# unirestore/UniRestore

Measured on AMD Instinct MI355X. Metric: restored 512x512 images/sec @ 20 denoise steps (whole job), higher is better.
Workload: dtype bf16; 1 GPU; PIR 512x512 batch=8/GPU, 20 DDIM steps, bf16, hipGraph replay (BASELINE.json configs[1]; configs[2] shape for N=8); global_batch=8, per_gpu_batch=8, image=512, denoise_steps=20, parallelism=image-parallel dp1, weights=seeded random init (no checkpoints reachable)

## Files before the change

### include/unirestore_hip.h

```cpp
#ifndef UNIRESTORE_HIP_H
#define UNIRESTORE_HIP_H

#include <stddef.h>
#include <stdint.h>

#ifdef __cplusplus
extern "C" {
#endif

typedef void* ur_stream_t;

enum { UR_OK = 0, UR_E_INVALID = -1, UR_E_UNSUPPORTED = -2, UR_E_LAUNCH = -3, UR_E_WORKSPACE = -4 };

enum { UR_DT_BF16 = 0, UR_DT_F16 = 1 };

enum {
  UR_ACT_NONE = 0,
  UR_ACT_SILU = 1,
  UR_ACT_GELU = 2,
  UR_ACT_GEGLU = 3,
  UR_ACT_GATE = 4,
  UR_ACT_TANH = 5,
  UR_ACT_RELU = 6
};

int ur_version(void);
const char* ur_last_error(void);

typedef struct ur_conv_desc {
  const void* x;
  const void* x2;
  const void* w;
  const float* bias;
  const void* residual;
  void* y;
  void* yt;
  float* gn_part;
  const float* gn_ab;
  int gn_silu;
  float* row_stats;
  const float* ln_stats;
  const float* ln_colsum;
  float ln_eps;
  int ln_dim;
  int ln_parts;
  float* workspace;
  size_t workspace_bytes;
  int N, H, W;
  int C1, ldx, C2, ldx2;
  int Cout, ldw, ldy, ldr;
  int KH, KW, stride, pad_t, pad_l;
  int OH, OW;
  int upsample2x;
  int act;
  int out_f32;
  int n_split, t_rows, t_ld;
  float out_scale;
  int nbatch;
  long long bs_x, bs_x2, bs_w, bs_bias, bs_y, bs_r;
  int k_chunk_major;
  long long bias_img_stride;
  int dtype;
  const void* w_frag;
} ur_conv_desc;

int ur_conv2d_nhwc(const ur_conv_desc* d, ur_stream_t stream);

typedef struct ur_conv_plan {
  int row_stat_parts;
  int gn_parts;
  int gn_fused;
  int prologue_ok;
} ur_conv_plan;
int ur_conv2d_plan(const ur_conv_desc* d, ur_conv_plan* plan);

typedef struct ur_conv_launch_info {
  int launcher;
  int splitk;
  int nk_per_split;
  int reduce;
  int reduce_ri;
  int gn_pass;
  int group_loop;
} ur_conv_launch_info;
int ur_conv2d_plan_launch(const ur_conv_desc* d, ur_conv_launch_info* info);
int ur_conv_launcher_count(void);
const char* ur_conv_launcher_name(int i);

int ur_gemm_bias_act(const void* x, const void* w, const float* bias, const void* residual, void* y, long long M, int N, int K,
                     int ldx, int ldw, int ldy, int ldr, int act, float* workspace, size_t workspace_bytes, int dtype,
                     ur_stream_t stream);
int ur_groupconv3x3_nhwc(const void* x, const void* w, const float* bias, void* y, int N, int H, int W, int Cg, int Cog,
                         int groups, int act, float* workspace, size_t workspace_bytes, int dtype, ur_stream_t stream);

int ur_groupnorm_stats_parts(int N, int HW, int C);
size_t ur_groupnorm_ws_bytes(int N, int HW, int C);
size_t ur_groupnorm_ab_bytes(int N, int C);
int ur_groupnorm_stats(const void* x, float* part, int N, int HW, int C, int dtype, ur_stream_t stream);
int ur_instnorm_stats(const void* x, float* part, int N, int HW, int C, int dtype, ur_stream_t stream);
int ur_groupnorm_finalize(const float* part1, int parts1, int C1, const float* part2, int parts2, int C2, const float* gamma,
                          const float* beta, int N, int HW, int G, float eps, float* ab, float* mean_out, ur_stream_t stream);
int ur_groupnorm_apply_act(const void* x, const void* x2, void* y, const float* ab, int N, int HW, int C1, int C2, int silu,
                           int dtype, ur_stream_t stream);
int ur_groupnorm_nhwc(const void* x, const void* x2, void* y, const float* gamma, const float* beta, int N, int HW,
                      int C1, int C2, int G, float eps, int silu, float* ws, float* ab, const float* pre1, int parts1,
                      const float* pre2, int parts2, int dtype, ur_stream_t stream);
int ur_layernorm_rows(const void* x, void* y, const float* gamma, const float* beta, long long rows, int C,
                      float eps, int dtype, ur_stream_t stream);
int ur_softmax_rows_f32(const float* s, void* p, long long rows, int cols, int ldp, int dtype, ur_stream_t stream);

int ur_attention_fwd(const void* q, const void* k, const void* vt, void* o, int B, int H, int Tq, int Tk,
                     int D, int ldq, int ldk, int ldvt, int ldo, long long bs_q, long long bs_k,
                     long long bs_vt, long long bs_o, float scale, int dtype, ur_stream_t stream);
size_t ur_attention_workspace_bytes(int B, int H, int Tq, int Tk, int D);
int ur_attention_fwd_ws(const void* q, const void* k, const void* vt, void* o, int B, int H, int Tq, int Tk,
                        int D, int ldq, int ldk, int ldvt, int ldo, long long bs_q, long long bs_k, long long bs_vt,
                        long long bs_o, float scale, void* ws, size_t ws_bytes, int dtype, ur_stream_t stream);
typedef struct ur_attention_plan {
  int kernel;
  int workgroups;
  int n_full;
  int n_split;
} ur_attention_plan;
int ur_attention_plan_launch(const void* q, const void* k, const void* vt, void* o, int B, int H, int Tq, int Tk,
                             int D, int ldq, int ldk, int ldvt, int ldo, long long bs_q, long long bs_k, long long bs_vt,
                             long long bs_o, void* ws, size_t ws_bytes, ur_attention_plan* plan);
int ur_attention_kernel_count(void);
const char* ur_attention_kernel_name(int i);

size_t ur_chain_tile_bytes(void);
int ur_ff_geglu_fused(const void* x, const void* stream_w, size_t stream_bytes, void* y, long long T, int C, int hidden, int ldx,
                      int ldy, float ln_eps, int dtype, ur_stream_t stream);

int ur_transformer_head_fused(const void* x, const float* gn_ab, const void* stream_w, size_t stream_bytes, void* h0, void* q, void* k,
                              void* vt, long long T, int tokens_per_image, int C, float ln_eps, int dtype, ur_stream_t stream);
int ur_transformer_tail_fused(const void* o1, const void* h0, const void* xres, const void* stream_w, size_t stream_bytes, void* y,
                              float* gn_part, long long T, int tokens_per_image, int C, int hidden, int heads, int tk, float ln_eps,
                              float attn_scale, int dtype, ur_stream_t stream);

int ur_csce_fused(const void* x, const void* cond, const void* stream_w, size_t stream_bytes, void* y, float* gn_part, long long T,
                  int tokens_per_image, int C, int Ccond, int dtype, ur_stream_t stream);

int ur_dwconv3x3_nhwc(const void* x, const float* w9c, const float* bias, void* y, int N, int H, int W, int C,
                      int gate, int dtype, ur_stream_t stream);
int ur_avgpool_hw(const void* x, float* out, int N, int HW, int C, float* ws, int dtype, ur_stream_t stream);
int ur_scale_channels(const void* x, const float* s, const void* residual, void* y, int N, int HW, int C,
                      int dtype, ur_stream_t stream);
int ur_axpy_channels(const void* a, const void* b, const float* s, void* y, long long rows, int C, int dtype, ur_stream_t stream);
int ur_spade_modulate(const void* n, const void* gb, int ldgb, const void* residual, void* y, long long rows, int C,
                      int dtype, ur_stream_t stream);
int ur_linear_f32(const float* x, const float* w, const float* bias, float* y, int M, int N, int K, int groups,
                  int act, ur_stream_t stream);
int ur_tfa_prompt_update(const float* pooled, const float* cond, float* upd, int B, int T, int D, ur_stream_t stream);
int ur_scale_channels_fanout(const void* x, const float* s, void* y, int B, int K, int HW, int C, int dtype, ur_stream_t stream);
int ur_tfa_prompt_update_fanout(const float* pooled, const float* cond, float* upd, int B, int K, int T, int D, int cond_per_row,
                                ur_stream_t stream);
int ur_vec_mul_group(const float* a, const float* b, float* out, int N, int C, int G, ur_stream_t stream);

int ur_image_to_nhwc(const float* img, void* y, int N, int C, int H, int W, int Cpad, int dtype, ur_stream_t stream);
int ur_nhwc_to_nchw_f32(const void* x, int x_is_f32, float* out, int N, int C, int H, int W, int ld, float mul,
                        float add, int dtype, ur_stream_t stream);
int ur_nchw_f32_to_nhwc(const float* x, void* y, int N, int C, int H, int W, int Cpad, int dtype, ur_stream_t stream);
int ur_image_resize_pad_nhwc(const float* img, void* y, int N, int C, int H, int W, int RH, int RW, int PH, int PW, int Cpad,
                             float mul, float add, int dtype, ur_stream_t stream);
int ur_image_unpad_resize_nchw(const void* x, int x_is_f32, float* out, int N, int C, int XH, int XW, int ld, int CH, int CW,
                               int OH, int OW, float mul, float add, int quantize, int dtype, ur_stream_t stream);
int ur_image_u8_ingest(const uint8_t* src, long long slot_bytes, const int* geom, void* y, int N, int CH, int CW, int Cpad, float mul,
                       float add, int dtype, ur_stream_t stream);
int ur_image_u8_egress(const void* x, int x_is_f32, uint8_t* dst, long long slot_bytes, const int* geom, int* nonfinite, int N, int C,
                       int XH, int XW, int ld, float mul, float add, int dtype, ur_stream_t stream);
int ur_vae_sample(const float* moments, int ld, const float* noise_nchw, float* z_nhwc, void* z_16, int N,
                  int HW, int Clat, int Cpad, float scale, int dtype, ur_stream_t stream);
int ur_add_noise(const float* z0, const float* noise_nchw, float* zt, void* zt_16, int N, int HW, int Clat,
                 int Cpad, float sa, float sb, int dtype, ur_stream_t stream);
int ur_ddim_step(float* zt, const float* eps, int ld_eps, void* zt_16, long long M, int Clat, int Cpad,
                 float c_x, float c_e, int dtype, ur_stream_t stream);
int ur_latent_tiles_gather(const float* z, void* tiles_16, int N, int LH, int LW, int Cpad, int T, int th, int tw,
                           const int* origins, int dtype, ur_stream_t stream);
int ur_latent_tiles_blend_ddim(float* zt, const float* eps_tiles, int ld_eps, void* zt_tiles_16, const float* wn, int N, int LH,
                               int LW, int Clat, int Cpad, int T, int th, int tw, const int* origins, float c_x, float c_e,
                               int dtype, ur_stream_t stream);
int ur_f32_to_bf16_scaled(const float* x, int ld, void* y, long long M, int C, int Cpad, float mul, int dtype, ur_stream_t stream);

int ur_image_metrics(const float* pred, const float* target, int N, int C, int H, int W, int win, double data_range,
                     double* psnr, double* ssim, void* ws, long long ws_bytes, ur_stream_t stream);
long long ur_image_metrics_ws_size(int N, int C, int H, int W, int win);

int ur_profile_enable(int on);
int ur_profile_report(char* buf, size_t buf_bytes);

#ifdef __cplusplus
}
#endif
#endif
```

### unirestore_amd/capi.py

```python
import ctypes as C
import os

import torch

_HERE = os.path.dirname(os.path.abspath(__file__))
LIB_PATH = os.environ.get("UR_LIB") or os.path.join(_HERE, "libunirestore_hip.so")

UR_ACT_NONE, UR_ACT_SILU, UR_ACT_GELU, UR_ACT_GEGLU, UR_ACT_GATE, UR_ACT_TANH, UR_ACT_RELU = range(7)
UR_DT_BF16, UR_DT_F16 = 0, 1
UR_E_INVALID, UR_E_UNSUPPORTED = -1, -2


class ConvDesc(C.Structure):
    _fields_ = [
        ("x", C.c_void_p), ("x2", C.c_void_p), ("w", C.c_void_p), ("bias", C.c_void_p), ("residual", C.c_void_p),
        ("y", C.c_void_p), ("yt", C.c_void_p), ("gn_part", C.c_void_p), ("gn_ab", C.c_void_p), ("gn_silu", C.c_int),
        ("row_stats", C.c_void_p), ("ln_stats", C.c_void_p), ("ln_colsum", C.c_void_p), ("ln_eps", C.c_float), ("ln_dim", C.c_int), ("ln_parts", C.c_int),
        ("workspace", C.c_void_p),
        ("workspace_bytes", C.c_size_t),
        ("N", C.c_int), ("H", C.c_int), ("W", C.c_int),
        ("C1", C.c_int), ("ldx", C.c_int), ("C2", C.c_int), ("ldx2", C.c_int),
        ("Cout", C.c_int), ("ldw", C.c_int), ("ldy", C.c_int), ("ldr", C.c_int),
        ("KH", C.c_int), ("KW", C.c_int), ("stride", C.c_int), ("pad_t", C.c_int), ("pad_l", C.c_int),
        ("OH", C.c_int), ("OW", C.c_int),
        ("upsample2x", C.c_int), ("act", C.c_int), ("out_f32", C.c_int),
        ("n_split", C.c_int), ("t_rows", C.c_int), ("t_ld", C.c_int),
        ("out_scale", C.c_float),
        ("nbatch", C.c_int),
        ("bs_x", C.c_longlong), ("bs_x2", C.c_longlong), ("bs_w", C.c_longlong), ("bs_bias", C.c_longlong),
        ("bs_y", C.c_longlong), ("bs_r", C.c_longlong), ("k_chunk_major", C.c_int), ("bias_img_stride", C.c_longlong),
        ("dtype", C.c_int), ("w_frag", C.c_void_p),
    ]


class ConvPlan(C.Structure):
    _fields_ = [("row_stat_parts", C.c_int), ("gn_parts", C.c_int), ("gn_fused", C.c_int), ("prologue_ok", C.c_int)]


class ConvLaunchInfo(C.Structure):
    _fields_ = [("launcher", C.c_int), ("splitk", C.c_int), ("nk_per_split", C.c_int), ("reduce", C.c_int), ("reduce_ri", C.c_int),
                ("gn_pass", C.c_int), ("group_loop", C.c_int)]


class AttentionPlan(C.Structure):
    _fields_ = [("kernel", C.c_int), ("workgroups", C.c_int), ("n_full", C.c_int), ("n_split", C.c_int)]


_P, _I, _F, _LL, _SZ = C.c_void_p, C.c_int, C.c_float, C.c_longlong, C.c_size_t

SIGNATURES = {
    "ur_version": (_I, []),
    "ur_last_error": (C.c_char_p, []),
    "ur_conv2d_nhwc": (_I, [C.POINTER(ConvDesc), _P]),
    "ur_conv2d_plan": (_I, [C.POINTER(ConvDesc), C.POINTER(ConvPlan)]),
    "ur_conv2d_plan_launch": (_I, [C.POINTER(ConvDesc), C.POINTER(ConvLaunchInfo)]),
    "ur_conv_launcher_count": (_I, []),
    "ur_conv_launcher_name": (C.c_char_p, [_I]),
    "ur_gemm_bias_act": (_I, [_P, _P, _P, _P, _P, _LL, _I, _I, _I, _I, _I, _I, _I, _P, _SZ, _I, _P]),
    "ur_groupconv3x3_nhwc": (_I, [_P, _P, _P, _P, _I, _I, _I, _I, _I, _I, _I, _P, _SZ, _I, _P]),
    "ur_groupnorm_stats_parts": (_I, [_I, _I, _I]),
    "ur_groupnorm_ws_bytes": (_SZ, [_I, _I, _I]),
    "ur_groupnorm_ab_bytes": (_SZ, [_I, _I]),
    "ur_groupnorm_stats": (_I, [_P, _P, _I, _I, _I, _I, _P]),
    "ur_instnorm_stats": (_I, [_P, _P, _I, _I, _I, _I, _P]),
    "ur_groupnorm_finalize": (_I, [_P, _I, _I, _P, _I, _I, _P, _P, _I, _I, _I, _F, _P, _P, _P]),
    "ur_groupnorm_apply_act": (_I, [_P, _P, _P, _P, _I, _I, _I, _I, _I, _I, _P]),
    "ur_groupnorm_nhwc": (_I, [_P, _P, _P, _P, _P, _I, _I, _I, _I, _I, _F, _I, _P, _P, _P, _I, _P, _I, _I, _P]),
    "ur_layernorm_rows": (_I, [_P, _P, _P, _P, _LL, _I, _F, _I, _P]),
    "ur_softmax_rows_f32": (_I, [_P, _P, _LL, _I, _I, _I, _P]),
    "ur_attention_fwd": (_I, [_P, _P, _P, _P, _I, _I, _I, _I, _I, _I, _I, _I, _I, _LL, _LL, _LL, _LL, _F, _I, _P]),
    "ur_attention_workspace_bytes": (_SZ, [_I, _I, _I, _I, _I]),
    "ur_attention_fwd_ws": (_I, [_P, _P, _P, _P, _I, _I, _I, _I, _I, _I, _I, _I, _I, _LL, _LL, _LL, _LL, _F, _P, _SZ, _I, _P]),
    "ur_attention_plan_launch": (_I, [_P, _P, _P, _P, _I, _I, _I, _I, _I, _I, _I, _I, _I, _LL, _LL, _LL, _LL, _P, _SZ, C.POINTER(AttentionPlan)]),
    "ur_attention_kernel_count": (_I, []),
    "ur_attention_kernel_name": (C.c_char_p, [_I]),
    "ur_chain_tile_bytes": (_SZ, []),
    "ur_ff_geglu_fused": (_I, [_P, _P, _SZ, _P, _LL, _I, _I, _I, _I, _F, _I, _P]),
    "ur_transformer_head_fused": (_I, [_P, _P, _P, _SZ, _P, _P, _P, _P, _LL, _I, _I, _F, _I, _P]),
    "ur_transformer_tail_fused": (_I, [_P, _P, _P, _P, _SZ, _P, _P, _LL, _I, _I, _I, _I, _I, _F, _F, _I, _P]),
    "ur_csce_fused": (_I, [_P, _P, _P, _SZ, _P, _P, _LL, _I, _I, _I, _I, _P]),
    "ur_dwconv3x3_nhwc": (_I, [_P, _P, _P, _P, _I, _I, _I, _I, _I, _I, _P]),
    "ur_avgpool_hw": (_I, [_P, _P, _I, _I, _I, _P, _I, _P]),
    "ur_scale_channels": (_I, [_P, _P, _P, _P, _I, _I, _I, _I, _P]),
    "ur_scale_channels_fanout": (_I, [_P, _P, _P, _I, _I, _I, _I, _I, _P]),
    "ur_axpy_channels": (_I, [_P, _P, _P, _P, _LL, _I, _I, _P]),
    "ur_spade_modulate": (_I, [_P, _P, _I, _P, _P, _LL, _I, _I, _P]),
    "ur_linear_f32": (_I, [_P, _P, _P, _P, _I, _I, _I, _I, _I, _P]),
    "ur_tfa_prompt_update": (_I, [_P, _P, _P, _I, _I, _I, _P]),
    "ur_tfa_prompt_update_fanout": (_I, [_P, _P, _P, _I, _I, _I, _I, _I, _P]),
    "ur_vec_mul_group": (_I, [_P, _P, _P, _I, _I, _I, _P]),
    "ur_image_to_nhwc": (_I, [_P, _P, _I, _I, _I, _I, _I, _I, _P]),
    "ur_nhwc_to_nchw_f32": (_I, [_P, _I, _P, _I, _I, _I, _I, _I, _F, _F, _I, _P]),
    "ur_nchw_f32_to_nhwc": (_I, [_P, _P, _I, _I, _I, _I, _I, _I, _P]),
    "ur_image_resize_pad_nhwc": (_I, [_P, _P] + [_I] * 9 + [_F, _F, _I, _P]),
    "ur_image_unpad_resize_nchw": (_I, [_P, _I, _P] + [_I] * 9 + [_F, _F, _I, _I, _P]),
    "ur_image_u8_ingest": (_I, [_P, _LL, _P, _P, _I, _I, _I, _I, _F, _F, _I, _P]),
    "ur_image_u8_egress": (_I, [_P, _I, _P, _LL, _P, _P, _I, _I, _I, _I, _I, _F, _F, _I, _P]),
    "ur_vae_sample": (_I, [_P, _I, _P, _P, _P, _I, _I, _I, _I, _F, _I, _P]),
    "ur_add_noise": (_I, [_P, _P, _P, _P, _I, _I, _I, _I, _F, _F, _I, _P]),
    "ur_ddim_step": (_I, [_P, _P, _I, _P, _LL, _I, _I, _F, _F, _I, _P]),
    "ur_latent_tiles_gather": (_I, [_P, _P, _I, _I, _I, _I, _I, _I, _I, _P, _I, _P]),
    "ur_latent_tiles_blend_ddim": (_I, [_P, _P, _I, _P, _P, _I, _I, _I, _I, _I, _I, _I, _I, _P, _F, _F, _I, _P]),
    "ur_f32_to_bf16_scaled": (_I, [_P, _I, _P, _LL, _I, _I, _F, _I, _P]),
    "ur_image_metrics": (_I, [_P, _P, _I, _I, _I, _I, _I, C.c_double, _P, _P, _P, _LL, _P]),
    "ur_image_metrics_ws_size": (_LL, [_I, _I, _I, _I, _I]),
    "ur_profile_enable": (_I, [_I]),
    "ur_profile_report": (_I, [C.c_char_p, _SZ]),
}


def _load():
    if not os.path.exists(LIB_PATH):
        raise ImportError(
            f"{LIB_PATH} not found: build it with `python -m unirestore_amd.build` (or __graft_entry__.build()). "
            "There is no CPU / eager fallback in the product path.")
    lib = C.CDLL(LIB_PATH)
    for name, (res, args) in SIGNATURES.items():
        fn = getattr(lib, name)
        fn.restype, fn.argtypes = res, args
    return lib


lib = _load()


def launcher_names() -> list:
    return [lib.ur_conv_launcher_name(i).decode() for i in range(lib.ur_conv_launcher_count())]


def plan_launch(d: ConvDesc) -> ConvLaunchInfo:
    info = ConvLaunchInfo()
    check(lib.ur_conv2d_plan_launch(d, info))
    return info


def attention_kernel_names() -> list:
    return [lib.ur_attention_kernel_name(i).decode() for i in range(lib.ur_attention_kernel_count())]


def attention_plan(q, k, vt, o, B, H, Tq, Tk, D, ldq, ldk, ldvt, ldo, bs_q, bs_k, bs_vt, bs_o, ws, ws_bytes) -> AttentionPlan:
    plan = AttentionPlan()
    check(lib.ur_attention_plan_launch(q, k, vt, o, B, H, Tq, Tk, D, ldq, ldk, ldvt, ldo, bs_q, bs_k, bs_vt, bs_o, ws, ws_bytes, plan))
    return plan


class URError(RuntimeError):
    pass


def check(rc: int):
    if rc != 0:
        msg = lib.ur_last_error().decode("utf-8", "replace")
        if rc == UR_E_INVALID:
            raise ValueError(f"unirestore_hip: {msg}")
        if rc == UR_E_UNSUPPORTED:
            raise NotImplementedError(f"unirestore_hip (UR_E_UNSUPPORTED): {msg}")
        raise URError(f"unirestore_hip error {rc}: {msg}")
```

### unirestore_amd/csrc/igemm.hip

```cpp
#include "igemm_impl.h"

namespace urk {
#define UR_DECLARE(name)                                                                                             \
  ConvLaunch name##_bf16(void* k, size_t ws_bytes);                                                                 \
  ConvLaunch name##_f16(void* k, size_t ws_bytes);                                                                  \
  static ConvLaunch name(ConvK& k, size_t ws_bytes) { return (k.f16 ? name##_f16 : name##_bf16)(&k, ws_bytes); }
UR_CONV_LAUNCHERS(UR_DECLARE)
#undef UR_DECLARE
}

namespace {

ConvLaunch dispatch_conv(ConvK& k, bool pair, size_t ws_bytes) {
  if (k.KH == 3 && k.stride == 1 && k.pad_t == 1 && k.pad_l == 1 && k.kcm && k.staged_ok_ && !pair && k.nbatch == 1 &&
      k.OW % 32 == 0 && k.OH % 8 == 0 && k.OH == (k.ups ? 2 * k.H : k.H) && k.OW == (k.ups ? 2 * k.W : k.W) && !k.yt) {
    const bool ok128 = k.Cout % 128 == 0, ok160 = k.Cout % 160 == 0;
    const long long tm8 = (long long)k.N * (k.OH / 8) * (k.OW / 32);
    auto eff = [](long long t) { return t <= 128 ? (double)(t * (256 / t)) / 256.0 : (double)t / (double)(((t + 255) / 256) * 256); };
    const bool use160 = ok160 && (!ok128 || eff(tm8 * (k.Cout / 160)) >= eff(tm8 * (k.Cout / 128)));
    const long long tiles8 = tm8 * (use160 ? k.Cout / 160 : k.Cout / 128);
    if ((ok128 || ok160) && tiles8 >= 64) {
      if (use160) return urk::halo_8x32_160(k, ws_bytes);
      return urk::halo_8x32_128(k, ws_bytes);
    }
  }
  if (k.KH == 3 && k.stride == 1 && k.pad_t == 1 && k.pad_l == 1 && k.kcm && !pair && k.nbatch == 1 && !k.ups && k.C2 == 0 &&
      k.Cout <= 32 && k.OW % 32 == 0 && k.OH % 8 == 0 && k.OH == k.H && k.OW == k.W && !k.yt && !k.gn_part && !k.gn_ab && !k.row_stats && !k.ln_stats &&
      !k.bias_img && (long long)k.N * (k.OH / 8) * (k.OW / 32) >= 128)
    return urk::halo_thin_32(k, ws_bytes);
  const bool himg_ups = k.ups && k.OH == 16 && k.OW == 16 && k.H == 8 && k.W == 8;
  if (k.KH == 3 && k.stride == 1 && k.pad_t == 1 && k.pad_l == 1 && k.kcm && k.staged_ok_ && !pair && k.nbatch == 1 &&
      ((!k.ups && k.OH == k.H && k.OW == k.W) || himg_ups) && !k.yt && k.Cout % 128 == 0 && k.nk >= 36) {
    if (k.wf && k.OH == 8 && k.OW == 8 && k.N <= 16 && k.Cin % 256 == 0 && k.nk >= 72 && k.y && k.ws && !k.gn_ab && !k.row_stats && !k.ln_stats &&
        (long long)(k.nk / 36) * k.M * k.Cout * 4 <= (long long)ws_bytes)
      return urk::wstream_8x8(k, ws_bytes);
    if (k.OH == 16 && k.OW == 16) return urk::himg_16x16(k, ws_bytes);
    if (k.OH == 8 && k.OW == 8 && k.N % 4 == 0) {
      return urk::himg_8x8x4(k, ws_bytes);
    }
  }
  if (k.KH == 1 && k.stride == 1 && !k.ups && k.C2 == 0 && k.staged_ok_ && k.Cout % 256 == 0 && !k.yt && (k.act == UR_ACT_GEGLU || k.act == UR_ACT_GATE) &&
      (long long)((k.M + 255) / 256) * (k.Cout / 256) * k.nbatch >= 200 && (long long)k.M * k.ldx < (1ll << 31) - 256)
  {
    auto fill = [](long long t) { return (double)t / (double)(((t + 255) / 256) * 256); };
    const long long tm = (k.M + 255) / 256;
    if (k.Cout % 320 == 0 && k.nbatch == 1 && !k.bias_img && fill(tm * (k.Cout / 320)) > fill(tm * (k.Cout / 256)))
      return urk::gemm_256x320_pair(k, ws_bytes);
    return urk::gemm_256x256(k, ws_bytes);
  }
  const bool use_v1 = k.KH == 1 && k.nk <= 10;
  const long long blocks128 = (long long)((k.M + 127) / 128) * ((k.Cout + 127) / 128) * k.nbatch;
  const bool g1 = k.KH == 1 && k.stride == 1 && !k.ups && k.C2 == 0 && k.pad_t == 0 && k.pad_l == 0 && k.OH == k.H && k.OW == k.W &&
                  (long long)k.M * k.ldx + k.Ktot < (1ll << 31) - 256;
  auto nosplit = [&](int bm, int bn) { return (long long)((k.M + bm - 1) / bm) * ((k.Cout + bn - 1) / bn) * k.nbatch >= 200 || k.nk < 8 || !k.ws; };
  if (k.KH == 1 && !pair && k.Cout > 64) {
    const long long blocks64 = (long long)((k.M + 63) / 64) * ((k.Cout + 63) / 64) * k.nbatch;
    if (blocks128 < 200 && g1 && blocks64 >= 128 && blocks64 <= 256 && k.nk >= 8 && k.nk <= 48) return urk::g1_64x64_deep(k, ws_bytes);
    if (g1 && blocks128 < 200 && k.nk > 24 && k.nk <= 96 && (long long)((k.M + 127) / 128) * ((k.Cout + 63) / 64) * k.nbatch >= 256)
      return urk::g1_128x64_deep(k, ws_bytes);
    if (blocks128 < 200 && g1 && ((blocks64 >= 128 && k.nk <= 24) || (blocks64 >= 256 && k.nk <= 48))) return urk::g1_64x64(k, ws_bytes);
    if (blocks128 < 200 && k.nk <= 24) return g1 && nosplit(64, 64) ? urk::g1_64x64(k, ws_bytes) : urk::v1_64x64(k, ws_bytes);
    if (use_v1 && blocks128 > 256 && blocks128 < 400 && k.Cout % 128 == 0) return g1 && nosplit(128, 64) ? urk::g1_128x64(k, ws_bytes) : urk::v1_128x64(k, ws_bytes);
  }
  if (use_v1) {
    if (pair) return urk::v1_128x128(k, ws_bytes);
    if (k.Cout <= 32) return urk::v1_256x32(k, ws_bytes);
    if (k.Cout <= 64) return urk::v1_128x64(k, ws_bytes);
    if (k.Cout % 160 == 0 && k.Cout % 128 != 0) return g1 && nosplit(128, 160) ? urk::g1_128x160(k, ws_bytes) : urk::v1_128x160(k, ws_bytes);
    return g1 && nosplit(128, 128) ? urk::g1_128x128(k, ws_bytes) : urk::v1_128x128(k, ws_bytes);
  }
  if (k.Cout <= 32) return urk::v2_256x32(k, ws_bytes);
  if (k.Cout <= 64 && !pair) return urk::v2_128x64(k, ws_bytes);
  const bool n160 = !pair && k.Cout % 160 == 0 && k.Cout % 128 != 0;
  const long long big_tiles = (long long)((k.M + 255) / 256) * ((k.Cout + (n160 ? 159 : 127)) / (n160 ? 160 : 128)) * k.nbatch;
  if (g1 && !pair && big_tiles < 256) {
    const long long t160 = k.Cout % 160 == 0 ? (long long)((k.M + 127) / 128) * (k.Cout / 160) : 0;
    const long long t128 = (long long)((k.M + 127) / 128) * ((k.Cout + 127) / 128);
    auto fill = [](long long t) { return t <= 0 ? 0.0 : (double)t / (double)(((t + 255) / 256) * 256); };
    if (t160 >= 200 && fill(t160) >= fill(t128)) return urk::g1_128x160(k, ws_bytes);
    if (t128 >= 200) return urk::g1_128x128(k, ws_bytes);
  }
  if (big_tiles >= 160) {
    if (n160 && g1) return urk::g1_128x160(k, ws_bytes);
    if (n160) return urk::v2_256x160(k, ws_bytes);
    return urk::v2_256x128(k, ws_bytes);
  }
  if (k.Cout % 160 == 0 && k.Cout % 128 != 0 && !pair) return urk::v1_128x160(k, ws_bytes);
  return urk::v1_128x128(k, ws_bytes);
}

}

static int conv_impl(const ur_conv_desc* d, ur_stream_t stream, ur_conv_plan* plan, ur_conv_launch_info* info = nullptr) {
  UR_REQUIRE(d && d->x && d->w, "null x/w");
  UR_REQUIRE(d->KH == d->KW && (d->KH == 1 || d->KH == 3), "only 1x1 and 3x3 kernels");
  UR_REQUIRE(d->C1 > 0 && d->C1 % 8 == 0 && d->C2 % 8 == 0 && d->ldx % 8 == 0, "Cin/ldx must be multiples of 8");
  UR_REQUIRE(d->C2 == 0 || (d->x2 && d->ldx2 % 8 == 0), "virtual concat needs x2");
  UR_REQUIRE(d->Cout > 0 && d->Cout % 4 == 0 && d->ldw % 8 == 0, "Cout%4, ldw%8");
  UR_REQUIRE(d->nbatch >= 1 && d->stride >= 1 && d->OH > 0 && d->OW > 0, "bad dims");
  UR_REQUIRE(d->y || d->yt || d->gn_part, "no output requested");
  UR_REQUIRE_DT(d->dtype);
  const bool pair = d->act == UR_ACT_GEGLU || d->act == UR_ACT_GATE;
  if (pair && d->Cout % 64 != 0)
    return ur::fail(UR_E_UNSUPPORTED, "ur_conv2d_nhwc: pair activations (GEGLU / SimpleGate) need Cout % 64 == 0 (32-row a|g interleave)");
  UR_REQUIRE(!d->y || (d->out_f32 ? d->ldy % 4 == 0 : d->ldy % 4 == 0), "ldy%4");
  UR_REQUIRE(!d->residual || d->ldr % 4 == 0, "ldr%4");
  UR_REQUIRE(!d->yt || (d->t_rows > 0 && d->n_split % 4 == 0 && !pair), "bad transposed-output spec");

  ConvK k;
  k.x = (const uint16_t*)d->x; k.x2 = (const uint16_t*)d->x2; k.w = (const uint16_t*)d->w; k.bias = d->bias;
  k.res = (const uint16_t*)d->residual; k.y = d->y; k.yt = (uint16_t*)d->yt;
  k.ws = d->workspace;
  k.N = d->N; k.H = d->H; k.W = d->W; k.C1 = d->C1; k.ldx = d->ldx; k.C2 = d->C2; k.ldx2 = d->ldx2;
  k.Cin = d->C1 + d->C2; k.Cout = d->Cout; k.ldw = d->ldw; k.ldy = d->ldy; k.ldr = d->ldr;
  k.KH = d->KH; k.KW = d->KW; k.stride = d->stride; k.pad_t = d->pad_t; k.pad_l = d->pad_l;
  k.OH = d->OH; k.OW = d->OW; k.OHW = d->OH * d->OW; k.ups = d->upsample2x; k.act = d->act; k.out_f32 = d->out_f32;
  k.n_split = d->yt ? d->n_split : d->Cout; k.t_rows = d->t_rows; k.t_ld = d->t_ld;
  k.out_scale = d->out_scale;
  k.M = d->N * d->OH * d->OW; k.Ktot = d->KH * d->KW * k.Cin; k.nk = (k.Ktot + 63) / 64; k.nbatch = d->nbatch;
  k.bs_x = d->bs_x; k.bs_x2 = d->bs_x2; k.bs_w = d->bs_w; k.bs_bias = d->bs_bias; k.bs_y = d->bs_y; k.bs_r = d->bs_r; k.bias_img = d->bias_img_stride;
  UR_REQUIRE(k.M > 0, "empty problem");
  UR_REQUIRE((long long)d->N * d->H * d->W * (long long)std::max(d->ldx, d->ldx2) < (1ll << 31) &&
                 (long long)d->Cout * d->ldw < (1ll << 31), "tensor too large for 32-bit element offsets");

  k.kcm = d->k_chunk_major; k.wf = (const uint16_t*)d->w_frag; k.wmajor = 0; k.xgm = 0; k.xbn = 0; k.patch_tw = 0;
  UR_REQUIRE(!k.kcm || (k.Cin % 64 == 0 && d->C1 % 64 == 0), "k_chunk_major needs C1 and C1+C2 to be multiples of 64");
  k.gn_part = d->gn_part; k.gn_ab = d->gn_ab; k.gn_silu = d->gn_silu; k.f16 = d->dtype == UR_DT_F16; k.gn_fused = 0; k.gn_parts = 0;
  k.ln_parts = d->ln_parts;
  k.row_stats = d->row_stats; k.ln_stats = d->ln_stats; k.ln_colsum = d->ln_colsum; k.ln_eps = d->ln_eps; k.ln_dim = d->ln_dim;
  UR_REQUIRE(!d->ln_stats || (d->ln_colsum && d->ln_dim > 0), "ln_stats needs ln_colsum / ln_dim");
  UR_REQUIRE(!(d->bias_img_stride && (pair || d->ln_stats || d->yt)), "per-image bias rows do not combine with pair activations / LayerNorm folding / transposed columns");
  k.staged_ok_ = (d->y ? (!d->out_f32 && ((d->ldy | d->bs_y) & 7) == 0) : d->gn_part != nullptr) &&
                 (!d->residual || ((d->ldr | d->bs_r) & 7) == 0);
  UR_REQUIRE(!d->gn_part || (!d->out_f32 && !d->yt), "gn_part needs a plain 16-bit output (or none)");
  hipStream_t s = (hipStream_t)stream;
  const double flops = 2.0 * k.M * (double)k.Cout * k.Ktot * k.nbatch;
  const double bytes = 2.0 * ((double)k.M * k.Cin + (double)k.Cout * k.Ktot + (double)k.M * k.Cout) * k.nbatch;
  const char* fam = d->KH == 3 ? "conv3x3_igemm" : "gemm1x1_igemm";
  static const bool prof_shapes = getenv("UR_PROF_SHAPES") != nullptr;
  if (prof_shapes) {
    static std::map<std::string, int> interned;
    char buf[128];
    snprintf(buf, sizeof buf, "%s M%d N%d K%d s%d u%d b%d a%d", d->KH == 3 ? "c3" : "g1", k.M, k.Cout, k.Ktot, d->stride, d->upsample2x,
             k.nbatch, d->act);
    fam = interned.emplace(buf, 0).first->first.c_str();
  }
  const ConvLaunch launch = dispatch_conv(k, pair, d->workspace_bytes);
  const bool group_loop = k.nbatch > 1 && d->KH == 3 && k.kcm && k.stride == 1 && !pair && !k.gn_part && !k.row_stats && !k.ln_stats &&
                          !k.yt && !k.gn_ab && !k.out_f32 && k.staged_ok_ && k.Cout % 128 == 0 && !k.bias_img && k.C2 == 0;
  auto group_k = [&](int b) {
    ConvK kb = k;
    kb.nbatch = 1;
    kb.x = k.x + b * k.bs_x; kb.w = k.w + b * k.bs_w; kb.bias = k.bias ? k.bias + b * k.bs_bias : nullptr;
    kb.res = k.res ? k.res + b * k.bs_r : nullptr;
    kb.y = reinterpret_cast<uint16_t*>(k.y) + b * k.bs_y;
    kb.bs_x = kb.bs_w = kb.bs_bias = kb.bs_y = kb.bs_r = 0;
    return kb;
  };
  if (plan) {
    plan->row_stat_parts = d->row_stats ? (k.splitk > 1 ? 1 : k.tiles_n) : 0;
    plan->gn_parts = k.gn_parts; plan->gn_fused = k.gn_fused; plan->prologue_ok = launch.prologue_ok;
  }
  if (info) {
    ConvK kb = group_loop ? group_k(0) : k;
    const ConvLaunch l = group_loop ? dispatch_conv(kb, pair, d->workspace_bytes) : launch;
    info->launcher = l.id; info->splitk = kb.splitk; info->nk_per_split = kb.nk_per_split;
    const ReducePlan r = kb.splitk > 1 ? plan_splitk_reduce(kb) : ReducePlan{-1, 0};
    info->reduce = r.kind; info->reduce_ri = r.ri;
    info->gn_pass = k.gn_part && !k.gn_fused && !group_loop;
    info->group_loop = group_loop;
  }
  if (plan || info) return UR_OK;
  if (!d->y && d->gn_part && (!k.gn_fused || k.splitk > 1))
    return ur::fail(UR_E_UNSUPPORTED, "ur_conv2d_nhwc: y == NULL needs a launch whose epilogue writes gn_part (see ur_conv2d_plan)");
  if (d->gn_ab && !launch.prologue_ok)
    return ur::fail(UR_E_UNSUPPORTED, "ur_conv2d_nhwc: gn_ab is not supported by this launch (see ur_conv2d_plan.prologue_ok)");
  ur::ProfScope prof(fam, flops, bytes, s);
  UR_REQUIRE(!(d->row_stats || d->ln_stats) || (k.staged_ok_ && k.nbatch == 1 && !d->yt == !d->yt), "row_stats / ln fusion need a bf16 staged output");
  if (group_loop) {
    for (int b = 0; b < d->nbatch; ++b) {
      ConvK kb = group_k(b);
      const int rcb = dispatch_conv(kb, pair, d->workspace_bytes).launch(&kb, s);
      if (rcb != UR_OK) return rcb;
    }
    return UR_OK;
  }
  const int rc = launch.launch(&k, s);
  if (rc != UR_OK) return rc;
  if (k.gn_part && !k.gn_fused) {
    const int ctot = (pair ? k.Cout / 2 : k.Cout) * k.nbatch;
    UR_REQUIRE(k.y && k.ldy == ctot, "gn_part fallback needs a dense output (ldy == channels)");
    return ur::gn_stats_launch(k.y, k.gn_part, k.N, k.OHW, ctot, d->dtype, s);
  }
  return UR_OK;
}

extern "C" int ur_conv2d_nhwc(const ur_conv_desc* d, ur_stream_t stream) { return conv_impl(d, stream, nullptr); }

extern "C" int ur_conv2d_plan(const ur_conv_desc* d, ur_conv_plan* plan) {
  UR_REQUIRE(d && plan, "null pointer");
  ur_conv_desc t = *d;
  if (!t.y && !t.yt && !t.gn_part) t.y = reinterpret_cast<void*>(16);
  return conv_impl(&t, nullptr, plan);
}

extern "C" int ur_conv2d_plan_launch(const ur_conv_desc* d, ur_conv_launch_info* info) {
  UR_REQUIRE(d && info, "null pointer");
  ur_conv_desc t = *d;
  if (!t.y && !t.yt && !t.gn_part) t.y = reinterpret_cast<void*>(16);
  return conv_impl(&t, nullptr, nullptr, info);
}

#define UR_LAUNCHER_NAME(name) #name,
static const char* const kLauncherNames[] = {UR_CONV_LAUNCHERS(UR_LAUNCHER_NAME)};
#undef UR_LAUNCHER_NAME
static_assert(sizeof(kLauncherNames) / sizeof(kLauncherNames[0]) == UR_CONV_LAUNCHER_COUNT, "one name per launcher");

extern "C" int ur_conv_launcher_count(void) { return UR_CONV_LAUNCHER_COUNT; }
extern "C" const char* ur_conv_launcher_name(int i) { return i >= 0 && i < UR_CONV_LAUNCHER_COUNT ? kLauncherNames[i] : nullptr; }

extern "C" int ur_gemm_bias_act(const void* x, const void* w, const float* bias, const void* residual, void* y, long long M, int N, int K,
                                int ldx, int ldw, int ldy, int ldr, int act, float* workspace, size_t workspace_bytes, int dtype,
                                ur_stream_t stream) {
  UR_REQUIRE(M > 0 && M < (1ll << 31), "M out of range");
  ur_conv_desc d = {};
  d.x = x; d.w = w; d.bias = bias; d.residual = residual; d.y = y;
  d.workspace = workspace; d.workspace_bytes = workspace_bytes;
  d.N = 1; d.H = 1; d.W = (int)M; d.C1 = K; d.ldx = ldx; d.Cout = N; d.ldw = ldw; d.ldy = ldy; d.ldr = ldr;
  d.KH = d.KW = 1; d.stride = 1; d.OH = 1; d.OW = (int)M; d.act = act; d.out_scale = 1.f; d.nbatch = 1; d.dtype = dtype;
  return conv_impl(&d, stream, nullptr);
}

extern "C" int ur_groupconv3x3_nhwc(const void* x, const void* w, const float* bias, void* y, int N, int H, int W, int Cg, int Cog,
                                    int groups, int act, float* workspace, size_t workspace_bytes, int dtype, ur_stream_t stream) {
  UR_REQUIRE(groups >= 1 && Cg % 8 == 0 && Cog % 4 == 0, "groups >= 1, Cg % 8 == 0, Cog % 4 == 0");
  ur_conv_desc d = {};
  d.x = x; d.w = w; d.bias = bias; d.y = y;
  d.workspace = workspace; d.workspace_bytes = workspace_bytes;
  d.N = N; d.H = H; d.W = W; d.C1 = Cg; d.ldx = Cg * groups; d.Cout = Cog; d.ldw = 9 * Cg; d.ldy = Cog * groups;
  d.KH = d.KW = 3; d.stride = 1; d.pad_t = d.pad_l = 1; d.OH = H; d.OW = W; d.act = act; d.out_scale = 1.f; d.nbatch = groups;
  d.bs_x = Cg; d.bs_w = (long long)Cog * 9 * Cg; d.bs_bias = Cog; d.bs_y = Cog; d.dtype = dtype;
  return conv_impl(&d, stream, nullptr);
}
```

### unirestore_amd/csrc/igemm_impl.h

```cpp
#pragma once
#include <cstdio>
#include <cstdlib>
#include <map>
#include <string>

#include "common.h"

static __device__ uint4 g_zero_page[8];
typedef uint32_t ig_u32x4 __attribute__((ext_vector_type(4)));

struct ConvLaunch {
  int (*launch)(void* k, hipStream_t s);
  int prologue_ok;
  int id;
};

namespace {

struct ConvK {
  const uint16_t* x; const uint16_t* x2; const uint16_t* w; const float* bias; const uint16_t* res;
  void* y; uint16_t* yt; float* ws; float* gn_part; const float* gn_ab;
  float* row_stats; const float* ln_stats; const float* ln_colsum; float ln_eps; int ln_dim, ln_parts;
  int N, H, W, C1, ldx, C2, ldx2, Cin, Cout, ldw, ldy, ldr, KH, KW, stride, pad_t, pad_l, OH, OW, OHW;
  int ups, act, out_f32, n_split, t_rows, t_ld;
  float out_scale;
  int M, Ktot, nk, tiles_m, tiles_n, splitk, nk_per_split, nbatch;
  long long bs_x, bs_x2, bs_w, bs_bias, bs_y, bs_r, bias_img;
  int gn_fused, gn_parts, gn_silu, f16, staged_ok_;
  int patch_tw;
  int kcm;
  const uint16_t* wf;
  int wmajor;
  int xgm, xbn;
};

__device__ __forceinline__ void xcd_tile_map(const ConvK& p, int id, int& tm, int& tn) {
  const int xcd = id & 7, idx = id >> 3;
  if (p.xgm) {
    const int lm = idx / p.xbn, ln = idx - lm * p.xbn;
    tm = (xcd % p.xgm) * (p.tiles_m / p.xgm) + lm;
    tn = (xcd / p.xgm) * p.xbn + ln;
    return;
  }
  const int nt = p.tiles_m * p.tiles_n, q = nt >> 3, r = nt & 7;
  id = (xcd < r ? xcd * (q + 1) : r * (q + 1) + (xcd - r) * q) + idx;
  if (p.wmajor) { tn = id / p.tiles_m; tm = id - tn * p.tiles_m; }
  else { tm = id / p.tiles_n; tn = id - tm * p.tiles_n; }
}

static inline void pick_xcd_grid(ConvK& k, double W, double A) {
  k.xgm = 0; k.xbn = 0; k.wmajor = 0;
  static const bool off = getenv("UR_NOXCDGRID") != nullptr;
  if (off || k.nbatch != 1) return;
  const long long nt = (long long)k.tiles_m * k.tiles_n;
  double best = 0.9 * (8.0 * W + A);
  if (nt % 8 == 0)
    for (int gm = 4; gm >= 1; gm >>= 1) {
      const int gn = 8 / gm;
      if (k.tiles_m % gm || k.tiles_n % gn) continue;
      const double c = gm * W + gn * A;
      if (c < best) { best = c; k.xgm = gm; k.xbn = k.tiles_n / gn; }
    }
  if (!k.xgm && k.tiles_n >= 8 && W + 8.0 * A < best) k.wmajor = 1;
}

__device__ __forceinline__ bool is_pair_act(int act) { return act == UR_ACT_GEGLU || act == UR_ACT_GATE; }

__device__ __forceinline__ int tile_row_to_m(const ConvK& p, int m0, int r) {
  return p.patch_tw ? m0 + (r / p.patch_tw) * p.OW + (r % p.patch_tw) : m0 + r;
}

template <bool F16>
__device__ __forceinline__ void epi_store(const ConvK& p, int gb, int m, int co, float v[4]) {
  if (p.res) {
    const uint16_t* r = p.res + gb * p.bs_r + (long long)m * p.ldr + co;
    uint2 rv = *reinterpret_cast<const uint2*>(r);
    v[0] += Act<F16>::lo(rv.x); v[1] += Act<F16>::hi(rv.x);
    v[2] += Act<F16>::lo(rv.y); v[3] += Act<F16>::hi(rv.y);
  }
  if (p.yt && co >= p.n_split) {
    int b = m / p.t_rows, t = m - b * p.t_rows;
    int cw = p.Cout - p.n_split;
    uint16_t* o = p.yt + ((long long)b * cw + (co - p.n_split)) * p.t_ld + t;
#pragma unroll
    for (int e = 0; e < 4; ++e) o[(long long)e * p.t_ld] = f2h16<F16>(v[e]);
    return;
  }
  if (!p.y) return;
  if (p.out_f32) {
    float* o = reinterpret_cast<float*>(p.y) + gb * p.bs_y + (long long)m * p.ldy + co;
    *reinterpret_cast<float4*>(o) = make_float4(v[0], v[1], v[2], v[3]);
  } else {
    uint16_t* o = reinterpret_cast<uint16_t*>(p.y) + gb * p.bs_y + (long long)m * p.ldy + co;
    *reinterpret_cast<uint2*>(o) = make_uint2(Act<F16>::pack2(v[0], v[1]), Act<F16>::pack2(v[2], v[3]));
  }
}

__device__ __forceinline__ int epi_act(const ConvK& p, int gb, int m, int co_in, float a[4], const float g[4]) {
  const long long boff = gb * p.bs_bias + (p.bias_img ? (long long)(m / p.OHW) * p.bias_img : 0);
  if (p.bias) {
    const float* b = p.bias + boff + co_in;
    float4 bv = *reinterpret_cast<const float4*>(b);
    a[0] += bv.x; a[1] += bv.y; a[2] += bv.z; a[3] += bv.w;
  }
  int co = co_in;
  if (is_pair_act(p.act)) {
    float gg[4] = {g[0], g[1], g[2], g[3]};
    if (p.bias) {
      float4 bv = *reinterpret_cast<const float4*>(p.bias + boff + co_in + 32);
      gg[0] += bv.x; gg[1] += bv.y; gg[2] += bv.z; gg[3] += bv.w;
    }
#pragma unroll
    for (int e = 0; e < 4; ++e) a[e] *= (p.act == UR_ACT_GEGLU) ? gelu_f(gg[e]) : gg[e];
    co = (co_in >> 6) * 32 + (co_in & 31);
  } else if (p.act != UR_ACT_NONE) {
#pragma unroll
    for (int e = 0; e < 4; ++e) a[e] = apply_act(a[e], p.act);
  }
#pragma unroll
  for (int e = 0; e < 4; ++e) a[e] *= p.out_scale;
  return co;
}

template <int BM, int NC, int NT, int SROW, bool LOAD>
__device__ __forceinline__ void tile_copy(const ConvK& p, uint16_t* g, long long ld, unsigned char* smem, int m0, int M, int c0,
                                          int cmax) {
  constexpr int Q = NC / 8;
  constexpr int TOT = BM * Q, U = 5;
  for (int i0 = threadIdx.x; i0 < TOT; i0 += NT * U) {
    uint4 v[U];
    uint16_t* gp[U];
    uint2* lp[U];
    bool ok[U];
#pragma unroll
    for (int u = 0; u < U; ++u) {
      const int i = i0 + u * NT;
      const int r = i / Q, c = (i - r * Q) * 8;
      const int m = tile_row_to_m(p, m0, i < TOT ? r : 0);
      ok[u] = i < TOT && m < M && c < cmax;
      gp[u] = g + (long long)(ok[u] ? m : m0) * ld + c0 + (ok[u] ? c : 0);
      lp[u] = reinterpret_cast<uint2*>(smem + (ok[u] ? r * SROW + c * 2 : 0));
      if (LOAD) v[u] = *reinterpret_cast<const uint4*>(gp[u]);
      else { const uint2 a = lp[u][0], b = lp[u][1]; v[u] = make_uint4(a.x, a.y, b.x, b.y); }
    }
#pragma unroll
    for (int u = 0; u < U; ++u) {
      if (!ok[u]) continue;
      if (LOAD) { lp[u][0] = make_uint2(v[u].x, v[u].y); lp[u][1] = make_uint2(v[u].z, v[u].w); }
      else {
store16_wt(gp[u], v[u]);
      }
    }
  }
}

template <int FM, int FN, int WTM, int WTN, bool F16>
__device__ __forceinline__ void igemm_epilogue_direct(const ConvK& p, f32x16 (&acc)[FN][FM], int m0, int n0, int wm, int wn,
                                                      int lane, int gb) {
  const int fhalf = lane >> 5, mrow = lane & 31;
  const bool pair = is_pair_act(p.act);
#pragma unroll
  for (int a = 0; a < FN; ++a) {
    if (pair && (a & 1)) continue;
#pragma unroll
    for (int b = 0; b < FM; ++b) {
      int m = tile_row_to_m(p, m0, wm * WTM + b * 32 + mrow);
#pragma unroll
      for (int rg = 0; rg < 4; ++rg) {
        int co_in = n0 + wn * WTN + a * 32 + rg * 8 + fhalf * 4;
        bool ok = m < p.M && co_in < p.Cout;
        float v[4], g[4] = {0.f, 0.f, 0.f, 0.f};
#pragma unroll
        for (int e = 0; e < 4; ++e) v[e] = acc[a][b][rg * 4 + e];
        if (pair) {
          constexpr int a1 = (FN > 1) ? 1 : 0;
#pragma unroll
          for (int e = 0; e < 4; ++e) g[e] = acc[(a + a1) % FN][b][rg * 4 + e];
        }
        int co = co_in;
        if (ok) co = epi_act(p, gb, m, co_in, v, g);
        if (ok) epi_store<F16>(p, gb, m, co, v);
      }
    }
  }
}

template <int FM, int FN, int WTM, int WTN, int BM, int BN, int SROW, int PAIR, int LN, int MULTI, int YT, int ACT, bool F16>
__device__ __forceinline__ void epi_frag_pass(const ConvK& p, f32x16 (&acc)[FN][FM], int m0, int n0, int c0, int wm, int wn, int lane,
                                              int gb, unsigned char* smem, const float* sbias, const float* scol, const float* srow) {
  const int fhalf = lane >> 5, mrow = lane & 31;
  const bool pair_ = PAIR == 2 ? is_pair_act(p.act) : PAIR != 0;
  const bool ln_ = LN == 2 ? p.ln_stats != nullptr : LN != 0;
  const bool multi_ = MULTI == 2 ? (p.bias_img && !p.patch_tw && p.OHW < BM) : MULTI != 0;
  const bool yt_ = YT == 2 ? p.yt != nullptr : YT != 0;
  const bool act_ = ACT == 2 ? p.act != UR_ACT_NONE : ACT != 0;
  const bool has_res = p.res != nullptr;
#pragma unroll
  for (int a = 0; a < FN; ++a) {
    if (pair_ && (a & 1)) continue;
#pragma unroll
    for (int rg = 0; rg < 4; ++rg) {
      const int ln = wn * WTN + a * 32 + rg * 8 + fhalf * 4;
      const int co_in = n0 + ln;
      float4 bv = *reinterpret_cast<const float4*>(sbias + ln);
      float4 gv = make_float4(0.f, 0.f, 0.f, 0.f);
      if (pair_) gv = *reinterpret_cast<const float4*>(sbias + ln + 32);
      const int lco = pair_ ? ((ln >> 6) * 32 + (ln & 31)) : ln;
      const int co = c0 + lco;
      const bool col_ok = co_in < p.Cout;
      float4 sv = make_float4(0.f, 0.f, 0.f, 0.f), sg = make_float4(0.f, 0.f, 0.f, 0.f);
      if (ln_) {
        sv = *reinterpret_cast<const float4*>(scol + ln);
        if (pair_) sg = *reinterpret_cast<const float4*>(scol + ln + 32);
      }
#pragma unroll
      for (int b = 0; b < FM; ++b) {
        const int lm = wm * WTM + b * 32 + mrow;
        if (multi_) {
          const int il = lm / p.OHW;
          bv = *reinterpret_cast<const float4*>(sbias + il * BN + ln);
          if (pair_) gv = *reinterpret_cast<const float4*>(sbias + il * BN + ln + 32);
        }
        float v[4], gq[4] = {0.f, 0.f, 0.f, 0.f};
        constexpr int a1 = (FN > 1) ? 1 : 0;
        if (ln_) {
          const float mean = srow[2 * lm], rstd = srow[2 * lm + 1];
          v[0] = rstd * (acc[a][b][rg * 4] - mean * sv.x) + bv.x;     v[1] = rstd * (acc[a][b][rg * 4 + 1] - mean * sv.y) + bv.y;
          v[2] = rstd * (acc[a][b][rg * 4 + 2] - mean * sv.z) + bv.z; v[3] = rstd * (acc[a][b][rg * 4 + 3] - mean * sv.w) + bv.w;
          if (pair_) {
            gq[0] = rstd * (acc[(a + a1) % FN][b][rg * 4] - mean * sg.x) + gv.x;     gq[1] = rstd * (acc[(a + a1) % FN][b][rg * 4 + 1] - mean * sg.y) + gv.y;
            gq[2] = rstd * (acc[(a + a1) % FN][b][rg * 4 + 2] - mean * sg.z) + gv.z; gq[3] = rstd * (acc[(a + a1) % FN][b][rg * 4 + 3] - mean * sg.w) + gv.w;
          }
        } else {
          v[0] = acc[a][b][rg * 4] + bv.x; v[1] = acc[a][b][rg * 4 + 1] + bv.y;
          v[2] = acc[a][b][rg * 4 + 2] + bv.z; v[3] = acc[a][b][rg * 4 + 3] + bv.w;
          if (pair_) {
            gq[0] = acc[(a + a1) % FN][b][rg * 4] + gv.x; gq[1] = acc[(a + a1) % FN][b][rg * 4 + 1] + gv.y;
            gq[2] = acc[(a + a1) % FN][b][rg * 4 + 2] + gv.z; gq[3] = acc[(a + a1) % FN][b][rg * 4 + 3] + gv.w;
          }
        }
        if (pair_) {
          const float g0 = gq[0], g1 = gq[1], g2 = gq[2], g3 = gq[3];
          if (p.act == UR_ACT_GEGLU) { v[0] *= gelu_f(g0); v[1] *= gelu_f(g1); v[2] *= gelu_f(g2); v[3] *= gelu_f(g3); }
          else { v[0] *= g0; v[1] *= g1; v[2] *= g2; v[3] *= g3; }
        } else if (act_) {
#pragma unroll
          for (int e = 0; e < 4; ++e) v[e] = apply_act(v[e], p.act);
        }
#pragma unroll
        for (int e = 0; e < 4; ++e) v[e] *= p.out_scale;
        const int mg = tile_row_to_m(p, m0, lm);
        const bool ok = col_ok && mg < p.M;
        if (yt_ && co >= p.n_split) {
          if (ok) epi_store<F16>(p, gb, mg, co, v);
          continue;
        }
        uint2* sp = reinterpret_cast<uint2*>(smem + lm * SROW + lco * 2);
        if (has_res) {
          const uint2 rv = *sp;
          v[0] += Act<F16>::lo(rv.x); v[1] += Act<F16>::hi(rv.x);
          v[2] += Act<F16>::lo(rv.y); v[3] += Act<F16>::hi(rv.y);
        }
        if (ok) *sp = make_uint2(Act<F16>::pack2(v[0], v[1]), Act<F16>::pack2(v[2], v[3]));
      }
    }
  }
}

template <int FM, int FN, int WTM, int WTN, int BM, int BN, int NT, int CLS, bool PAIRC, bool F16>
__device__ __forceinline__ void staged_epilogue(const ConvK& p, f32x16 (&acc)[FN][FM], int m0, int n0, int wm, int wn, int lane,
                                                int gb, unsigned char* smem, bool owner, int nimg_tile_in) {
  constexpr int SROW = (PAIRC ? BN : BN * 2) + 8;
  const bool pair = CLS ? is_pair_act(p.act) : false;
  const bool ln = CLS ? p.ln_stats != nullptr : false;
  const bool yt = CLS ? p.yt != nullptr : false;
  const int nimg_tile = CLS ? nimg_tile_in : 1;
  const int c0 = pair ? (n0 >> 1) : n0;
  const int ncols = pair ? BN / 2 : BN;
  const int cmax = min(yt ? p.n_split : (pair ? p.Cout / 2 : p.Cout), c0 + ncols) - c0;
  float* sbias = reinterpret_cast<float*>(smem + BM * SROW);
  float* scol = sbias + 4 * BN;
  float* srow = scol + BN;
  const int img0 = m0 / p.OHW;
  for (int i = threadIdx.x; i < BN * nimg_tile; i += NT) {
    const int il = i / BN, col = i - il * BN;
    const long long boff = gb * p.bs_bias + (p.bias_img ? (long long)min(img0 + il, p.N - 1) * p.bias_img : 0);
    sbias[i] = (p.bias && n0 + col < p.Cout) ? p.bias[boff + n0 + col] : 0.f;
  }
  if (ln) {
    for (int i = threadIdx.x; i < BN; i += NT) scol[i] = n0 + i < p.Cout ? p.ln_colsum[n0 + i] : 0.f;
    for (int r = threadIdx.x; r < BM; r += NT) {
      const int m = min(tile_row_to_m(p, m0, r), p.M - 1);
      float sx = 0.f, sq = 0.f;
      for (int q = 0; q < p.ln_parts; ++q) {
        const float2 t2 = *reinterpret_cast<const float2*>(p.ln_stats + 2 * ((long long)q * p.M + m));
        sx += t2.x; sq += t2.y;
      }
      const float mean = sx / p.ln_dim;
      const float var = fmaxf(sq / p.ln_dim - mean * mean, 0.f);
      srow[2 * r] = mean;
      srow[2 * r + 1] = rsqrtf(var + p.ln_eps);
    }
  }
  if (p.res) {
    uint16_t* rb = const_cast<uint16_t*>(p.res) + gb * p.bs_r;
    if (pair) tile_copy<BM, (BN >= 16 ? BN / 2 : 8), NT, SROW, true>(p, rb, p.ldr, smem, m0, p.M, c0, cmax);
    else tile_copy<BM, BN, NT, SROW, true>(p, rb, p.ldr, smem, m0, p.M, c0, cmax);
  }
  __syncthreads();
  if (owner) {
    const bool multi = nimg_tile > 1, hasact = p.act != UR_ACT_NONE;
#define UR_EPI_PASS(PAIR, LN, MULTI, YT, ACT) \
    epi_frag_pass<FM, FN, WTM, WTN, BM, BN, SROW, PAIR, LN, MULTI, YT, ACT, F16>(p, acc, m0, n0, c0, wm, wn, lane, gb, smem, sbias, scol, srow)
    if constexpr (CLS == 0) { if (hasact) UR_EPI_PASS(0, 0, 0, 0, 1); else UR_EPI_PASS(0, 0, 0, 0, 0); }
    else if constexpr (PAIRC) {
      if (ln) UR_EPI_PASS(1, 1, 0, 0, 0); else UR_EPI_PASS(1, 0, 0, 0, 0);
    } else {
      if (pair) { if (ln) UR_EPI_PASS(1, 1, 0, 0, 0); else UR_EPI_PASS(1, 0, 0, 0, 0); }
      else if (yt) {
        if (hasact) UR_EPI_PASS(0, 2, 0, 1, 2);
        else if (ln) UR_EPI_PASS(0, 1, 0, 1, 0);
        else UR_EPI_PASS(0, 0, 0, 1, 0);
      }
      else if (multi) { if (hasact) UR_EPI_PASS(0, 0, 1, 0, 2); else UR_EPI_PASS(0, 0, 1, 0, 0); }
      else if (hasact) UR_EPI_PASS(0, 1, 0, 0, 2);
      else UR_EPI_PASS(0, 1, 0, 0, 0);
    }
#undef UR_EPI_PASS
  }
  __syncthreads();
  if (p.gn_fused) {
    float* red = sbias;
    const int CP = ncols >> 1, NG = NT / CP, RGN = (BM + NG - 1) / NG;
    const int cp = threadIdx.x % CP, g = threadIdx.x / CP;
    if (g < NG) {
      float s0 = 0.f, s1 = 0.f, q0 = 0.f, q1 = 0.f;
      if (cp * 2 < cmax) {
        const int r0 = g * RGN, r1 = p.patch_tw ? min(BM, r0 + RGN) : min(min(BM, r0 + RGN), p.M - m0);
        for (int r = r0; r < r1; ++r) {
          const uint32_t w = *reinterpret_cast<const uint32_t*>(smem + r * SROW + cp * 4);
          const float a = Act<F16>::lo(w), b = Act<F16>::hi(w);
          s0 += a; q0 += a * a; s1 += b; q1 += b * b;
        }
      }
      red[(g * 4 + 0) * CP + cp] = s0; red[(g * 4 + 1) * CP + cp] = s1;
      red[(g * 4 + 2) * CP + cp] = q0; red[(g * 4 + 3) * CP + cp] = q1;
    }
    __syncthreads();
    const int ctot = pair ? p.Cout / 2 : p.Cout;
    const int img = m0 / p.OHW, rem = m0 - img * p.OHW;
    const int pm = p.patch_tw ? ((rem / p.OW) / (BM / p.patch_tw)) * (p.OW / p.patch_tw) + (rem % p.OW) / p.patch_tw : rem / BM;
    float* st = p.gn_part + ((((long long)img * p.gn_parts + pm) * p.nbatch + gb) * ctot + c0) * 2;
    for (int i = threadIdx.x; i < cmax; i += NT) {
      const int c2 = i >> 1, odd = i & 1;
      float a = 0.f, b = 0.f;
      for (int gg = 0; gg < NG; ++gg) { a += red[(gg * 4 + odd) * CP + c2]; b += red[(gg * 4 + 2 + odd) * CP + c2]; }
      *reinterpret_cast<float2*>(st + 2 * i) = make_float2(a, b);
    }
  }
  if (p.row_stats) {
    constexpr int TPR = NT / BM >= 1 ? NT / BM : 1;
    const int r = threadIdx.x / TPR, part = threadIdx.x % TPR;
    if (r < BM) {
      const int m = tile_row_to_m(p, m0, r);
      const int npair = cmax >> 1, per = (npair + TPR - 1) / TPR;
      float sx = 0.f, sq = 0.f;
      for (int j = part * per; j < min(npair, (part + 1) * per); ++j) {
        const uint32_t w = *reinterpret_cast<const uint32_t*>(smem + r * SROW + j * 4);
        const float a = Act<F16>::lo(w), b = Act<F16>::hi(w);
        sx += a + b; sq += a * a + b * b;
      }
      if (TPR >= 2) { sx += __shfl_xor(sx, 1, 64); sq += __shfl_xor(sq, 1, 64); }
      if (TPR >= 4) { sx += __shfl_xor(sx, 2, 64); sq += __shfl_xor(sq, 2, 64); }
      static_assert(TPR == 1 || TPR == 2 || TPR == 4, "row-stat reduction: 1, 2 or 4 threads per row (same wave)");
      const int tn_idx = n0 / BN;
      if (m < p.M && part == 0)
        *reinterpret_cast<float2*>(p.row_stats + 2 * ((long long)tn_idx * p.M + m)) = make_float2(sx, sq);
    }
  }
  if (!p.y) return;
  uint16_t* yb = reinterpret_cast<uint16_t*>(p.y) + gb * p.bs_y;
  if (pair) tile_copy<BM, (BN >= 16 ? BN / 2 : 8), NT, SROW, false>(p, yb, p.ldy, smem, m0, p.M, c0, cmax);
  else tile_copy<BM, BN, NT, SROW, false>(p, yb, p.ldy, smem, m0, p.M, c0, cmax);
}

template <int BM, int BN, int NT, bool PAIRC = false>
constexpr int epi_lds_bytes() {
  constexpr int tile = BM * ((PAIRC ? BN : BN * 2) + 8);
  constexpr int aux1 = 5 * BN * 4 + BM * 8, aux2 = 4 * NT * 4;
  return tile + (aux1 > aux2 ? aux1 : aux2);
}

template <int FM, int FN, int WTM, int WTN, int BM, int BN, int NT, bool F16, bool DIRECT_OK = true, bool PAIRC = false>
__device__ __forceinline__ void igemm_epilogue(const ConvK& p, f32x16 (&acc)[FN][FM], int m0, int n0, int wm, int wn, int lane,
                                               int gb, int sz, unsigned char* smem, bool owner = true) {
  const int fhalf = lane >> 5, mrow = lane & 31;
  if (p.splitk > 1) {
    if (!owner) return;
    float* ws = p.ws + ((long long)(sz * p.nbatch + gb) * p.M) * p.Cout;
#pragma unroll
    for (int a = 0; a < FN; ++a)
#pragma unroll
      for (int b = 0; b < FM; ++b) {
        int m = tile_row_to_m(p, m0, wm * WTM + b * 32 + mrow);
#pragma unroll
        for (int rg = 0; rg < 4; ++rg) {
          int co = n0 + wn * WTN + a * 32 + rg * 8 + fhalf * 4;
          if (m < p.M && co < p.Cout)
            *reinterpret_cast<float4*>(ws + (long long)m * p.Cout + co) =
                make_float4(acc[a][b][rg * 4], acc[a][b][rg * 4 + 1], acc[a][b][rg * 4 + 2], acc[a][b][rg * 4 + 3]);
        }
      }
    return;
  }
  const bool pair = is_pair_act(p.act);
  constexpr int SROW = BN * 2 + 8;
  const int nimg_tile = (p.bias_img && !p.patch_tw && p.OHW < BM) ? BM / p.OHW : 1;
  const bool bias_geom_ok = !p.bias_img || p.patch_tw || (p.OHW % BM) == 0 || ((BM % p.OHW) == 0 && nimg_tile <= 4);
  const bool staged = p.staged_ok_ && BN >= 32 && bias_geom_ok;
  if (!staged) {
    if (DIRECT_OK && owner) igemm_epilogue_direct<FM, FN, WTM, WTN, F16>(p, acc, m0, n0, wm, wn, lane, gb);
    return;
  }
  const bool plain = !pair && !p.ln_stats && nimg_tile == 1 && !p.yt;
  if (PAIRC) { if (!plain) staged_epilogue<FM, FN, WTM, WTN, BM, BN, NT, 1, true, F16>(p, acc, m0, n0, wm, wn, lane, gb, smem, owner, nimg_tile); }
  else if (plain) staged_epilogue<FM, FN, WTM, WTN, BM, BN, NT, 0, false, F16>(p, acc, m0, n0, wm, wn, lane, gb, smem, owner, nimg_tile);
  else staged_epilogue<FM, FN, WTM, WTN, BM, BN, NT, 1, false, F16>(p, acc, m0, n0, wm, wn, lane, gb, smem, owner, nimg_tile);
}

#include "igemm_asm.inc"
#define IG_MN(ASM, ...)                                                                      \
  do {                                                                                       \
    if constexpr (F16) asm volatile(ASM("v_mfma_f32_32x32x16_f16") __VA_ARGS__);             \
    else asm volatile(ASM("v_mfma_f32_32x32x16_bf16") __VA_ARGS__);                          \
  } while (0)
template <int FM, int FN, bool F16>
__device__ __forceinline__ void ktile_mma(f32x16 (&acc)[FN][FM], const unsigned (&ab)[FM], unsigned aw) {
  ig_u32x4 t0, t1, t2, t3, t4, t5, t6, t7, t8, t9;
  unsigned x0, x1, xw;
#define KT_POOL6 "=&v"(t0), "=&v"(t1), "=&v"(t2), "=&v"(t3), "=&v"(t4), "=&v"(t5)
#define KT_POOL8 KT_POOL6, "=&v"(t6), "=&v"(t7)
#define KT_POOL10 KT_POOL8, "=&v"(t8), "=&v"(t9)
  if constexpr (FM == 1 && FN == 5) {
    IG_MN(IG_ASM_KT_1x5, : "+v"(acc[0][0]), "+v"(acc[1][0]), "+v"(acc[2][0]), "+v"(acc[3][0]), "+v"(acc[4][0]), KT_POOL10, "=&v"(x0), "=&v"(xw)
          : "v"(ab[0]), "v"(aw) : "memory");
  } else if constexpr (FM == 2 && FN == 2) {
    IG_MN(IG_ASM_KT_2x2, : "+v"(acc[0][0]), "+v"(acc[0][1]), "+v"(acc[1][0]), "+v"(acc[1][1]), KT_POOL8, "=&v"(x0), "=&v"(x1), "=&v"(xw)
          : "v"(ab[0]), "v"(ab[1]), "v"(aw) : "memory");
  } else if constexpr (FM == 1 && FN == 1) {
    IG_MN(IG_ASM_KT_1x1, : "+v"(acc[0][0]), KT_POOL6, "=&v"(x0), "=&v"(xw) : "v"(ab[0]), "v"(aw) : "memory");
  } else if constexpr (FM == 2 && FN == 1) {
    IG_MN(IG_ASM_KT_2x1, : "+v"(acc[0][0]), "+v"(acc[0][1]), KT_POOL6, "=&v"(x0), "=&v"(x1), "=&v"(xw) : "v"(ab[0]), "v"(ab[1]), "v"(aw) : "memory");
  } else if constexpr (FM == 2 && FN == 4) {
    IG_MN(IG_ASM_KT_2x4, : "+v"(acc[0][0]), "+v"(acc[0][1]), "+v"(acc[1][0]), "+v"(acc[1][1]), "+v"(acc[2][0]), "+v"(acc[2][1]), "+v"(acc[3][0]), "+v"(acc[3][1]),
          KT_POOL6, "=&v"(x0), "=&v"(x1), "=&v"(xw) : "v"(ab[0]), "v"(ab[1]), "v"(aw) : "memory");
  } else if constexpr (FM == 1 && FN == 10) {
    IG_MN(IG_ASM_KT_1x10, : "+v"(acc[0][0]), "+v"(acc[1][0]), "+v"(acc[2][0]), "+v"(acc[3][0]), "+v"(acc[4][0]), "+v"(acc[5][0]), "+v"(acc[6][0]), "+v"(acc[7][0]),
          "+v"(acc[8][0]), "+v"(acc[9][0]), KT_POOL6, "=&v"(x0), "=&v"(xw) : "v"(ab[0]), "v"(aw) : "memory");
  } else {
    static_assert(FM == 0, "no hand-scheduled K tile for this fragment shape");
  }
#undef KT_POOL6
#undef KT_POOL8
#undef KT_POOL10
}
template <int FM, int FN> constexpr bool ktile_gemm_ok() {
#if defined(UR_IGEMM_NOASM) || defined(UR_GEMM_NOASM)
  return false;
#else
  return (FM == 1 && (FN == 1 || FN == 5 || FN == 10)) || (FM == 2 && (FN == 1 || FN == 2 || FN == 4));
#endif
}
template <int FM, int FN> constexpr bool ktile_asm_ok() {
#ifdef UR_IGEMM_NOASM
  return false;
#else
  return (FM == 1 && FN == 5) || (FM == 2 && FN == 2);
#endif
}


template <int BM, int BN, int WM, int WN, bool G1, bool F16>
__global__ __launch_bounds__(256) void igemm_kernel(const ConvK p) {
  constexpr int WTM = BM / WM, WTN = BN / WN, FM = WTM / 32, FN = WTN / 32, XP = BM / 32, WP = BN / 32;
  constexpr int STAGE = (BM + BN) * 128;
  static_assert(WM * WN == 4 && WTM % 32 == 0 && WTN % 32 == 0, "tile/wave shape");
  extern __shared__ __attribute__((aligned(16))) unsigned char smem[];

  const int tid = threadIdx.x, lane = tid & 63, wid = tid >> 6;
  const int wm = wid % WM, wn = wid / WM;
  const int gb = blockIdx.y, sz = blockIdx.z;

  int tm, tn;
  xcd_tile_map(p, blockIdx.x, tm, tn);
  const int m0 = tm * BM, n0 = tn * BN;

  const uint16_t* __restrict__ X1 = p.x + gb * p.bs_x;
  const uint16_t* __restrict__ X2 = p.x2 ? p.x2 + gb * p.bs_x2 : nullptr;
  const uint16_t* __restrict__ Wt = p.w + gb * p.bs_w;

  const int chunk = tid & 7, lrow = tid >> 3;
  int ih0[XP], iw0[XP], nb[XP];
  bool xok[XP];
#pragma unroll
  for (int i = 0; i < XP; ++i) {
    int m = m0 + i * 32 + lrow;
    xok[i] = m < p.M;
    if (G1) { nb[i] = xok[i] ? m * p.ldx : 0; ih0[i] = iw0[i] = 0; continue; }
    int mm = xok[i] ? m : 0;
    int n = mm / p.OHW, rem = mm - n * p.OHW;
    int oh = rem / p.OW, ow = rem - oh * p.OW;
    ih0[i] = oh * p.stride - p.pad_t;
    iw0[i] = ow * p.stride - p.pad_l;
    nb[i] = n * p.H;
  }
  long long woff[WP];
  bool wok[WP];
#pragma unroll
  for (int j = 0; j < WP; ++j) {
    int row = n0 + j * 32 + lrow;
    wok[j] = row < p.Cout;
    woff[j] = (long long)(wok[j] ? row : 0) * p.ldw;
  }
  const int Hlim = p.ups ? p.H * 2 : p.H, Wlim = p.ups ? p.W * 2 : p.W;

  const int kt_begin = sz * p.nk_per_split;
  const int kt_end = min(p.nk, kt_begin + p.nk_per_split);
  int kcur = kt_begin * 64 + chunk * 8;
  int tap = 0, cch = kcur;
  const int ntap = p.KH * p.KW;
  if (!G1) {
    tap = kcur / p.Cin; cch = kcur - tap * p.Cin;
    if (p.kcm) { tap = kt_begin % ntap; cch = (kt_begin / ntap) * 64 + chunk * 8; }
  }

  uint4 xr[XP], wr[WP];
  auto load_tile = [&]() {
    const bool kval = kcur < p.Ktot;
    if (G1) {
#pragma unroll
      for (int i = 0; i < XP; ++i) {
        const bool v = kval && xok[i];
        const uint4 val = *reinterpret_cast<const uint4*>(v ? X1 + nb[i] + kcur : X1);
        xr[i] = v ? val : make_uint4(0, 0, 0, 0);
      }
#pragma unroll
      for (int j = 0; j < WP; ++j) {
        const bool v = kval && wok[j];
        const uint4 val = *reinterpret_cast<const uint4*>(v ? Wt + woff[j] + kcur : Wt);
        wr[j] = v ? val : make_uint4(0, 0, 0, 0);
      }
      kcur += 64;
      return;
    }
    const int dy = (p.KW == 1) ? 0 : (tap * 11) >> 5;
    const int dx = tap - dy * p.KW;
    const uint16_t* src = X1;
    int ld = p.ldx, cc = cch;
    if (cch >= p.C1) { src = X2; ld = p.ldx2; cc = cch - p.C1; }
#pragma unroll
    for (int i = 0; i < XP; ++i) {
      int ih = ih0[i] + dy, iw = iw0[i] + dx;
      bool v = kval && xok[i] && (unsigned)ih < (unsigned)Hlim && (unsigned)iw < (unsigned)Wlim;
      if (p.ups) { ih >>= 1; iw >>= 1; }
      long long off = ((long long)(nb[i] + ih) * p.W + iw) * ld + cc;
      const uint4* ptr = reinterpret_cast<const uint4*>(v ? src + off : src);
      uint4 val = *ptr;
      xr[i] = v ? val : make_uint4(0, 0, 0, 0);
    }
#pragma unroll
    for (int j = 0; j < WP; ++j) {
      bool v = kval && wok[j];
      const uint4* ptr = reinterpret_cast<const uint4*>(v ? Wt + woff[j] + kcur : Wt);
      uint4 val = *ptr;
      wr[j] = v ? val : make_uint4(0, 0, 0, 0);
    }
    kcur += 64;
    if (p.kcm) { if (++tap == ntap) { tap = 0; cch += 64; } }
    else { cch += 64; while (cch >= p.Cin) { cch -= p.Cin; ++tap; } }
  };
  auto store_tile = [&](int stage) {
    unsigned char* xs = smem + stage * STAGE;
    unsigned char* wsm = xs + BM * 128;
#pragma unroll
    for (int i = 0; i < XP; ++i) {
      int row = i * 32 + lrow;
      *reinterpret_cast<uint4*>(xs + row * 128 + ((chunk ^ ((row >> 1) & 7)) << 4)) = xr[i];
    }
#pragma unroll
    for (int j = 0; j < WP; ++j) {
      int row = j * 32 + lrow;
      *reinterpret_cast<uint4*>(wsm + row * 128 + ((chunk ^ ((row >> 1) & 7)) << 4)) = wr[j];
    }
  };

  f32x16 acc[FN][FM];
#pragma unroll
  for (int a = 0; a < FN; ++a)
#pragma unroll
    for (int b = 0; b < FM; ++b)
#pragma unroll
      for (int e = 0; e < 16; ++e) acc[a][b][e] = 0.f;

  const int frow = lane & 31, fhalf = lane >> 5;
  typedef __attribute__((address_space(3))) void* lptr_t;
  const unsigned kt_x0 = (unsigned)(uintptr_t)(lptr_t)smem + (wm * WTM + frow) * 128 + ((fhalf ^ ((frow >> 1) & 7)) << 4);
  const unsigned kt_w0 = (unsigned)(uintptr_t)(lptr_t)smem + (BM + wn * WTN + frow) * 128 + ((fhalf ^ ((frow >> 1) & 7)) << 4);
  static_assert(WTM % 32 == 0 && ((WTN >> 1) & 7) == 0, "fragment rows must keep the swizzle phase of row 0");
  auto compute = [&](int stage) {
    if constexpr (ktile_gemm_ok<FM, FN>()) {
      unsigned ab[FM];
#pragma unroll
      for (int b = 0; b < FM; ++b) ab[b] = kt_x0 + stage * STAGE + b * 4096;
      ktile_mma<FM, FN, F16>(acc, ab, kt_w0 + stage * STAGE);
      return;
    }
    const unsigned char* xs = smem + stage * STAGE;
    const unsigned char* wsm = xs + BM * 128;
#pragma unroll
    for (int ks = 0; ks < 4; ++ks) {
      const int slot = ks * 2 + fhalf;
      typename Frag<F16>::type bfr[FM], afr[FN];
#pragma unroll
      for (int b = 0; b < FM; ++b) {
        int row = wm * WTM + b * 32 + frow;
        bfr[b] = *reinterpret_cast<const typename Frag<F16>::type*>(xs + row * 128 + ((slot ^ ((row >> 1) & 7)) << 4));
      }
#pragma unroll
      for (int a = 0; a < FN; ++a) {
        int row = wn * WTN + a * 32 + frow;
        afr[a] = *reinterpret_cast<const typename Frag<F16>::type*>(wsm + row * 128 + ((slot ^ ((row >> 1) & 7)) << 4));
      }
#pragma unroll
      for (int a = 0; a < FN; ++a)
#pragma unroll
        for (int b = 0; b < FM; ++b)
          acc[a][b] = mfma16t(afr[a], bfr[b], acc[a][b]);
    }
  };

  if (kt_begin < kt_end) {
    load_tile();
    store_tile(0);
    __syncthreads();
    int stage = 0;
    for (int kt = kt_begin; kt < kt_end; ++kt) {
      const bool more = kt + 1 < kt_end;
      if (more) load_tile();
      compute(stage);
      if (more) store_tile(stage ^ 1);
      __syncthreads();
      stage ^= 1;
    }
  }
// ... 611 lines not shown

struct GnAB { float4 a0, a1, b0, b1; };
__device__ __forceinline__ GnAB gn_load_ab(const unsigned char* abuf, int chunk) {
  GnAB r;
  r.a0 = *reinterpret_cast<const float4*>(abuf + chunk * 32); r.a1 = *reinterpret_cast<const float4*>(abuf + chunk * 32 + 16);
  r.b0 = *reinterpret_cast<const float4*>(abuf + 256 + chunk * 32); r.b1 = *reinterpret_cast<const float4*>(abuf + 256 + chunk * 32 + 16);
  return r;
}
template <bool F16>
__device__ __forceinline__ void gn_piece_inplace(unsigned char* piece, const GnAB& ab, bool silu) {
  const float4 a0 = ab.a0, a1 = ab.a1, b0 = ab.b0, b1 = ab.b1;
  const uint4 v = *reinterpret_cast<const uint4*>(piece);
  float f[8];
  unpack8t<F16>(v, f);
  f[0] = fmaf(f[0], a0.x, b0.x); f[1] = fmaf(f[1], a0.y, b0.y); f[2] = fmaf(f[2], a0.z, b0.z); f[3] = fmaf(f[3], a0.w, b0.w);
  f[4] = fmaf(f[4], a1.x, b1.x); f[5] = fmaf(f[5], a1.y, b1.y); f[6] = fmaf(f[6], a1.z, b1.z); f[7] = fmaf(f[7], a1.w, b1.w);
  if (silu) {
#pragma unroll
    for (int e = 0; e < 8; ++e) f[e] = silu_f(f[e]);
  }
  *reinterpret_cast<uint4*>(piece) = pack8t<F16>(f);
}

template <int FM, int FN> struct KPipeRings { ig_u32x4 ra[FN == 5 ? 10 : 4], rb[4]; };
template <int FM, int FN, bool F16, int PHASE>
__device__ __forceinline__ void kpipe(f32x16 (&acc)[FN][FM], KPipeRings<FM, FN>& r, const unsigned (&ab)[FM], unsigned aw, const unsigned (&abn)[FM],
                                      unsigned awn) {
  unsigned x0, x1, xw;
#define KP_OPS_1x5 : "+v"(acc[0][0]), "+v"(acc[1][0]), "+v"(acc[2][0]), "+v"(acc[3][0]), "+v"(acc[4][0]),                                        \
      "+v"(r.ra[0]), "+v"(r.ra[1]), "+v"(r.ra[2]), "+v"(r.ra[3]), "+v"(r.ra[4]), "+v"(r.ra[5]), "+v"(r.ra[6]), "+v"(r.ra[7]), "+v"(r.ra[8]), "+v"(r.ra[9]), \
      "+v"(r.rb[0]), "+v"(r.rb[1]), "+v"(r.rb[2]), "+v"(r.rb[3]), "=&v"(x0), "=&v"(xw) : "v"(ab[0]), "v"(aw), "v"(abn[0]), "v"(awn) : "memory"
#define KP_OPS_2x2 : "+v"(acc[0][0]), "+v"(acc[0][1]), "+v"(acc[1][0]), "+v"(acc[1][1]),                                                          \
      "+v"(r.ra[0]), "+v"(r.ra[1]), "+v"(r.ra[2]), "+v"(r.ra[3]),                                                                                 \
      "+v"(r.rb[0]), "+v"(r.rb[1]), "+v"(r.rb[2]), "+v"(r.rb[3]), "=&v"(x0), "=&v"(x1), "=&v"(xw)                                                   \
      : "v"(ab[0]), "v"(ab[1]), "v"(aw), "v"(abn[0]), "v"(abn[1]), "v"(awn) : "memory"
  if constexpr (FM == 1 && FN == 5) {
    if constexpr (PHASE == 0) IG_MN(IG_ASM_KP_1x5_PRE, KP_OPS_1x5);
    else if constexpr (PHASE == 1) IG_MN(IG_ASM_KP_1x5_H1, KP_OPS_1x5);
    else if constexpr (PHASE == 2) IG_MN(IG_ASM_KP_1x5_H2, KP_OPS_1x5);
    else IG_MN(IG_ASM_KP_1x5_H2L, KP_OPS_1x5);
  } else if constexpr (FM == 2 && FN == 2) {
    if constexpr (PHASE == 0) IG_MN(IG_ASM_KP_2x2_PRE, KP_OPS_2x2);
    else if constexpr (PHASE == 1) IG_MN(IG_ASM_KP_2x2_H1, KP_OPS_2x2);
    else if constexpr (PHASE == 2) IG_MN(IG_ASM_KP_2x2_H2, KP_OPS_2x2);
    else IG_MN(IG_ASM_KP_2x2_H2L, KP_OPS_2x2);
  } else {
    static_assert(FM == 0, "no pipelined K tile for this fragment shape");
  }
#undef KP_OPS_1x5
#undef KP_OPS_2x2
}
template <int FM, int FN> __device__ __forceinline__ void kpipe_drain(KPipeRings<FM, FN>& r) {
  if constexpr (FN == 5)
    asm volatile("s_waitcnt lgkmcnt(0)" : "+v"(r.ra[0]), "+v"(r.ra[1]), "+v"(r.ra[2]), "+v"(r.ra[3]), "+v"(r.ra[4]), "+v"(r.ra[5]), "+v"(r.ra[6]), "+v"(r.ra[7]),
                 "+v"(r.ra[8]), "+v"(r.ra[9]), "+v"(r.rb[0]), "+v"(r.rb[1]), "+v"(r.rb[2]), "+v"(r.rb[3]) : : "memory");
  else
    asm volatile("s_waitcnt lgkmcnt(0)" : "+v"(r.ra[0]), "+v"(r.ra[1]), "+v"(r.ra[2]), "+v"(r.ra[3]), "+v"(r.rb[0]), "+v"(r.rb[1]), "+v"(r.rb[2]), "+v"(r.rb[3]) : : "memory");
}
template <int FM, int FN> __device__ __forceinline__ void kpipe_init(KPipeRings<FM, FN>& r) {
#pragma unroll
  for (int i = 0; i < (FN == 5 ? 10 : 4); ++i) r.ra[i] = ig_u32x4{0u, 0u, 0u, 0u};
#pragma unroll
  for (int i = 0; i < 4; ++i) r.rb[i] = ig_u32x4{0u, 0u, 0u, 0u};
}

template <int TH, int BN, int WM, int WN, bool F16, bool GNP>
__global__ __launch_bounds__(WM* WN * 64) void igemm_halo_kernel(const ConvK p) {
  constexpr int NW = WM * WN, TW = 32, BM = TH * TW, PW = TW + 2, HPIX = (TH + 2) * PW;
  constexpr int HSLOTS = (HPIX + 8 * NW - 1) / (8 * NW);
  constexpr int HPIECES = HSLOTS * NW, HBYTES = HPIECES * 1024;
  constexpr int WBYTES = BN * 128 > NW * 1024 ? BN * 128 : NW * 1024, WPIECES = BN / 8, WPW = (WPIECES + NW - 1) / NW;
  constexpr int WTM = BM / WM, WTN = BN / WN, FM = WTM / 32, FN = WTN / 32, NT = NW * 64;
  static_assert((NW == 8 || NW == 4) && WTM % 32 == 0 && WTN % 32 == 0 && HSLOTS <= 8, "wave layout");
  extern __shared__ __attribute__((aligned(16))) unsigned char smem[];
  unsigned char* const hbuf = smem;
  unsigned char* const wring = smem + 2 * HBYTES;
  unsigned char* const abuf = wring + 3 * WBYTES;
  constexpr bool gnp = GNP;
  static_assert(HSLOTS <= 7, "the in-LDS GroupNorm pass needs taps 2 .. HSLOTS+1 <= 8");

  const int tid = threadIdx.x, lane = tid & 63, wid = tid >> 6;
  const int wm = wid % WM, wn = wid / WM;
  const int sz = blockIdx.y;
  int id = blockIdx.x;
  {
    const int nt = p.tiles_m * p.tiles_n, q = nt >> 3, r = nt & 7, xcd = id & 7, idx = id >> 3;
    id = (xcd < r ? xcd * (q + 1) : r * (q + 1) + (xcd - r) * q) + idx;
  }
  const int tn = id % p.tiles_n, tmi = id / p.tiles_n;
  const int tiles_x = p.OW / TW, tiles_y = p.OH / TH;
  const int tx = tmi % tiles_x, ty = (tmi / tiles_x) % tiles_y, img = tmi / (tiles_x * tiles_y);
  const int n0 = tn * BN;
  const int m0 = img * p.OHW + ty * TH * p.OW + tx * TW;

  typedef __attribute__((address_space(1))) const void* gptr_t;
  typedef __attribute__((address_space(3))) void* lptr_t;
  const uint16_t* __restrict__ X1 = p.x;
  const uint16_t* __restrict__ X2 = p.x2;
  const uint16_t* __restrict__ Wt = p.w;
  const uint16_t* zero = reinterpret_cast<const uint16_t*>(g_zero_page);
  const int lr = lane >> 3, ps = lane & 7;
  const int chunk = ps ^ ((((wid & 1) << 2) + (lr >> 1)) & 7);

  int hpix[HSLOTS];
#pragma unroll
  for (int t = 0; t < HSLOTS; ++t) {
    const int hr = (t * NW + wid) * 8 + lr;
    const int hy = hr / PW, hx = hr - hy * PW;
    int iy = ty * TH - 1 + hy, ix = tx * TW - 1 + hx;
    const bool v = hr < HPIX && (unsigned)iy < (unsigned)p.OH && (unsigned)ix < (unsigned)p.OW;
    if (p.ups) { iy >>= 1; ix >>= 1; }
    hpix[t] = v ? (img * p.H + iy) * p.W + ix : -1;
  }
  int woff[WPW];
#pragma unroll
  for (int i = 0; i < WPW; ++i) {
    const int qq = (wid + NW * i < WPIECES) ? wid + NW * i : wid;
    const int row = n0 + qq * 8 + lr;
    woff[i] = row < p.Cout ? row * p.ldw : -1;
  }
  const int cps = p.nk_per_split / 9, c_begin = sz * cps, nchunk = min(p.nk / 9, c_begin + cps) - c_begin;
  const int nk = nchunk * 9, kt0 = c_begin * 9;

#ifdef UR_HALO_DMA_BUILTIN
  auto issue_w = [&](int kt, int ring) {
    unsigned char* st = wring + ring * WBYTES;
#pragma unroll
    for (int i = 0; i < WPW; ++i) {
      const int qq = (wid + NW * i < WPIECES) ? wid + NW * i : wid;
      const uint16_t* g = woff[i] >= 0 ? Wt + woff[i] + (kt0 + kt) * 64 + chunk * 8 : zero;
      __builtin_amdgcn_global_load_lds((gptr_t)g, (lptr_t)(st + qq * 1024), 16, 0, 0);
    }
  };
  auto issue_h = [&](int c, int t) {
    const int q = t * NW + wid;
    int cc = (c_begin + c) * 64 + chunk * 8;
    const uint16_t* src = X1;
    int ld = p.ldx;
    if (cc >= p.C1) { src = X2; ld = p.ldx2; cc -= p.C1; }
    const uint16_t* g = hpix[t] >= 0 ? src + hpix[t] * ld + cc : zero;
    __builtin_amdgcn_global_load_lds((gptr_t)g, (lptr_t)(hbuf + (c & 1) * HBYTES + q * 1024), 16, 0, 0);
  };
#else
  const int wid_s = __builtin_amdgcn_readfirstlane(wid);
  const ig_u32x4 rs_w = ig_make_rsrc(Wt, (unsigned long long)p.Cout * p.ldw * 2);
  const ig_u32x4 rs_x1 = ig_make_rsrc(X1, (unsigned long long)p.N * p.H * p.W * p.ldx * 2);
  const ig_u32x4 rs_x2 = ig_make_rsrc(X2 ? X2 : X1, (unsigned long long)p.N * p.H * p.W * (X2 ? p.ldx2 : p.ldx) * 2);
  const unsigned wring_lds = (unsigned)(uintptr_t)(lptr_t)wring, hbuf_lds = (unsigned)(uintptr_t)(lptr_t)hbuf;
  unsigned wvo[WPW];
#pragma unroll
  for (int i = 0; i < WPW; ++i) wvo[i] = woff[i] >= 0 ? (unsigned)woff[i] * 2u + chunk * 16u : IG_OOB;
  auto issue_w = [&](int kt, int ring) {
#pragma unroll
    for (int i = 0; i < WPW; ++i) {
      const int qq = (wid_s + NW * i < WPIECES) ? wid_s + NW * i : wid_s;
      ig_lds_dma16(wring_lds + ring * WBYTES + qq * 1024, wvo[i], rs_w, (unsigned)(kt0 + kt) * 128u);
    }
  };
  auto issue_h = [&](int c, int t) {
    const int cb = (c_begin + c) * 64;
    const bool second = cb >= p.C1;
    const unsigned ld2 = (unsigned)(second ? p.ldx2 : p.ldx) * 2u;
    const unsigned vo = hpix[t] >= 0 ? (unsigned)hpix[t] * ld2 + chunk * 16u : IG_OOB;
    const unsigned m0v = hbuf_lds + (c & 1) * HBYTES + (t * NW + wid_s) * 1024;
    if (second) ig_lds_dma16(m0v, vo, rs_x2, (unsigned)(cb - p.C1) * 2u);
    else ig_lds_dma16(m0v, vo, rs_x1, (unsigned)cb * 2u);
  };
#endif
  auto issue_ab = [&](int c) {
    const float* t = p.gn_ab + ((long long)img * 2 + (lane >> 4 & 1)) * p.Cin + (c_begin + c) * 64 + (lane & 15) * 4;
    const void* g = lane < 32 ? (const void*)t : (const void*)zero;
    __builtin_amdgcn_global_load_lds((gptr_t)g, (lptr_t)(abuf + (c & 1) * 1024), 16, 0, 0);
  };
  auto gn_slot = [&](int c, int t) {
    if (hpix[t] >= 0)
      gn_piece_inplace<F16>(hbuf + (c & 1) * HBYTES + (t * NW + wid) * 1024 + lane * 16, gn_load_ab(abuf + (c & 1) * 1024, chunk), p.gn_silu != 0);
  };

  f32x16 acc[FN][FM];
#pragma unroll
  for (int a = 0; a < FN; ++a)
#pragma unroll
    for (int b = 0; b < FM; ++b)
#pragma unroll
      for (int e = 0; e < 16; ++e) acc[a][b][e] = 0.f;
  const int frow = lane & 31, fhalf = lane >> 5;
  const unsigned hb_lds = (unsigned)(uintptr_t)(lptr_t)hbuf;
  const unsigned aw_lds = (unsigned)(uintptr_t)(lptr_t)wring + (wn * WTN + frow) * 128 + ((fhalf ^ ((frow >> 1) & 7)) << 4);
  static_assert(((WTN >> 1) & 7) == 0, "the wave's weight rows must keep the swizzle phase of fragment row 0");

  if (gnp) issue_ab(0);
#pragma unroll
  for (int t = 0; t < HSLOTS; ++t) issue_h(0, t);
  issue_w(0, 0);
  if (nk > 1) {
    issue_w(1, 1);
    asm volatile("s_waitcnt vmcnt(%0)" ::"n"(WPW) : "memory");
  } else {
    asm volatile("s_waitcnt vmcnt(0)" ::: "memory");
  }
  if (gnp) {
#pragma unroll
    for (int t = 0; t < HSLOTS; ++t) gn_slot(0, t);
    asm volatile("s_waitcnt lgkmcnt(0)" ::: "memory");
  }
  __builtin_amdgcn_s_barrier();

  auto tap_addr = [&](int cc, int tp, unsigned (&ab)[FM]) -> unsigned {
    const int dy = tp / 3, dx = tp % 3;
#pragma unroll
    for (int b = 0; b < FM; ++b) {
      const int hrow = (wm * FM + b + dy) * PW + dx + frow;
      ab[b] = hb_lds + (cc & 1) * HBYTES + hrow * 128 + ((fhalf ^ ((hrow >> 1) & 7)) << 4);
    }
    return aw_lds + (tp % 3) * WBYTES;
  };
#if defined(UR_HALO_DMA_BUILTIN) || !defined(UR_HALO_STAGGER)
  constexpr bool stagger = false;
  const bool early_grp = true;
#else
  constexpr bool stagger = ktile_asm_ok<FM, FN>();
  const bool early_grp = wid_s < NW / 2;
#endif
  KPipeRings<FM, FN> rings;
  if constexpr (ktile_asm_ok<FM, FN>()) {
    kpipe_init(rings);
    unsigned ab0[FM];
    const unsigned aw0 = tap_addr(0, 0, ab0);
    kpipe<FM, FN, F16, 0>(acc, rings, ab0, aw0, ab0, aw0);
  }

  for (int c = 0; c < nchunk; ++c) {
    const unsigned char* hb = hbuf + (c & 1) * HBYTES;
    const bool next_chunk = c + 1 < nchunk;
#pragma unroll
    for (int tap = 0; tap < 9; ++tap) {
      const int kt = c * 9 + tap;
      const bool more_w = kt + 2 < nk;
      const bool more_h = tap < HSLOTS && next_chunk;
      auto issue_tap = [&]() {
        if (more_w) issue_w(kt + 2, (tap + 2) % 3);
        if (tap < HSLOTS) { if (next_chunk) issue_h(c + 1, tap < HSLOTS ? tap : 0); }
      };
      if (!stagger || early_grp) issue_tap();
      const bool ab_now = gnp && tap == 0 && next_chunk;
      if (ab_now) issue_ab(c + 1);
      if (gnp && tap >= 2 && tap - 2 < HSLOTS && next_chunk) gn_slot(c + 1, (tap >= 2 && tap - 2 < HSLOTS) ? tap - 2 : 0);
      auto dma_wait = [&]() {
        if (ab_now) {
          if (more_w) asm volatile("s_waitcnt vmcnt(%0)" ::"n"(WPW + 2) : "memory");
          else asm volatile("s_waitcnt vmcnt(2)" ::: "memory");
        } else if (more_w && more_h) asm volatile("s_waitcnt vmcnt(%0)" ::"n"(WPW + 1) : "memory");
        else if (more_w) asm volatile("s_waitcnt vmcnt(%0)" ::"n"(WPW) : "memory");
        else if (more_h) asm volatile("s_waitcnt vmcnt(1)" ::: "memory");
        else asm volatile("s_waitcnt vmcnt(0)" ::: "memory");
      };
      if constexpr (ktile_asm_ok<FM, FN>()) {
        unsigned ab[FM], abn[FM];
        const unsigned aw = tap_addr(c, tap, ab), awn = tap_addr(c + (tap == 8 ? 1 : 0), (tap + 1) % 9, abn);
        kpipe<FM, FN, F16, 1>(acc, rings, ab, aw, abn, awn);
        if (stagger && !early_grp) issue_tap();
        dma_wait();
        __builtin_amdgcn_s_barrier();
        kpipe<FM, FN, F16, 2>(acc, rings, ab, aw, abn, awn);
        __builtin_amdgcn_s_barrier();
      } else {
        const int dy = tap / 3, dx = tap % 3;
        const unsigned char* wsm = wring + (tap % 3) * WBYTES;
        typedef typename Frag<F16>::type frag_t;
        auto load_frags = [&](int ks, frag_t (&bfr)[FM], frag_t (&afr)[FN]) {
          const int slot = ks * 2 + fhalf;
#pragma unroll
          for (int b = 0; b < FM; ++b) {
            const int hrow = (wm * FM + b + dy) * PW + dx + frow;
            bfr[b] = *reinterpret_cast<const frag_t*>(hb + hrow * 128 + ((slot ^ ((hrow >> 1) & 7)) << 4));
          }
#pragma unroll
          for (int a = 0; a < FN; ++a) {
            const int row = wn * WTN + a * 32 + frow;
            afr[a] = *reinterpret_cast<const frag_t*>(wsm + row * 128 + ((slot ^ ((row >> 1) & 7)) << 4));
          }
        };
#pragma unroll
        for (int ks = 0; ks < 4; ++ks) {
          frag_t bfr[FM], afr[FN];
          load_frags(ks, bfr, afr);
#pragma unroll
          for (int a = 0; a < FN; ++a)
#pragma unroll
            for (int b = 0; b < FM; ++b)
              acc[a][b] = mfma16t(afr[a], bfr[b], acc[a][b]);
        }
        dma_wait();
        asm volatile("s_waitcnt lgkmcnt(0)" ::: "memory");
        __builtin_amdgcn_s_barrier();
      }
    }
  }
  if constexpr (ktile_asm_ok<FM, FN>()) kpipe_drain(rings);
  asm volatile("s_waitcnt vmcnt(0)\n\ts_nop 15\n\ts_nop 7" ::: "memory");
  igemm_epilogue<FM, FN, WTM, WTN, BM, BN, NT, F16, BN == 32>(p, acc, m0, n0, wm, wn, lane, 0, sz, smem);
}

template <int TH, int BN, int WM, int WN, bool F16, bool GNP>
__global__ __launch_bounds__((WM * WN + 2) * 64) void igemm_halo_ws_kernel(const ConvK p) {
  constexpr int NW = WM * WN, TW = 32, BM = TH * TW, PW = TW + 2, HPIX = (TH + 2) * PW;
  constexpr int HSLOTS = (HPIX + 8 * NW - 1) / (8 * NW), HNEED = (HPIX + 7) / 8;
  constexpr int HPIECES = HSLOTS * NW, HBYTES = HPIECES * 1024;
  constexpr int HPER = (HNEED + 15) / 16, HTAP = 2 * HPER;
  constexpr int WBYTES = BN * 128, WPIECES = BN / 8, WH = WPIECES / 2;
  constexpr int WTM = BM / WM, WTN = BN / WN, FM = WTM / 32, FN = WTN / 32, NT = NW * 64;
  static_assert(NW == 8 && WTM % 32 == 0 && WTN % 32 == 0 && HTAP <= NW && ktile_asm_ok<FM, FN>(), "wave layout");
  extern __shared__ __attribute__((aligned(16))) unsigned char smem[];
  unsigned char* const hbuf = smem;
  unsigned char* const wring = smem + 2 * HBYTES;
  unsigned char* const abuf = wring + 3 * WBYTES;
  constexpr bool gnp = GNP;
  typedef __attribute__((address_space(3))) void* lptr_t;

  const int tid = threadIdx.x, lane = tid & 63, wid = tid >> 6;
  const int wid_s = __builtin_amdgcn_readfirstlane(wid);
  const int sz = blockIdx.y;
  int id = blockIdx.x;
  {
    const int nt = p.tiles_m * p.tiles_n, q = nt >> 3, r = nt & 7, xcd = id & 7, idx = id >> 3;
    id = (xcd < r ? xcd * (q + 1) : r * (q + 1) + (xcd - r) * q) + idx;
  }
  const int tn = id % p.tiles_n, tmi = id / p.tiles_n;
  const int tiles_x = p.OW / TW, tiles_y = p.OH / TH;
  const int tx = tmi % tiles_x, ty = (tmi / tiles_x) % tiles_y, img = tmi / (tiles_x * tiles_y);
  const int n0 = tn * BN;
  const int m0 = img * p.OHW + ty * TH * p.OW + tx * TW;
  const int cps = p.nk_per_split / 9, c_begin = sz * cps, nchunk = min(p.nk / 9, c_begin + cps) - c_begin;
  const int nk = nchunk * 9, kt0 = c_begin * 9;
  const unsigned wring_lds = (unsigned)(uintptr_t)(lptr_t)wring, hbuf_lds = (unsigned)(uintptr_t)(lptr_t)hbuf;
  const unsigned abuf_lds = (unsigned)(uintptr_t)(lptr_t)abuf;
  const int lr = lane >> 3, ps = lane & 7;
  auto halo_pixel = [&](int hr) -> int {
    const int hy = hr / PW, hx = hr - hy * PW;
    int iy = ty * TH - 1 + hy, ix = tx * TW - 1 + hx;
    const bool v = hr < HPIX && (unsigned)iy < (unsigned)p.OH && (unsigned)ix < (unsigned)p.OW;
    if (p.ups) { iy >>= 1; ix >>= 1; }
    return v ? (img * p.H + iy) * p.W + ix : -1;
  };

  if (wid_s >= NW) {
    const bool two = blockDim.x > (NW + 1) * 64;
    const bool do_w = wid_s == NW, do_h = two ? wid_s == NW + 1 : true;
    const unsigned ck0 = (ps ^ ((lr >> 1) & 7)) * 16u, ck1 = (ps ^ ((4 + (lr >> 1)) & 7)) * 16u;
    const ig_u32x4 rs_w = ig_make_rsrc(p.w, (unsigned long long)p.Cout * p.ldw * 2);
    const ig_u32x4 rs_x1 = ig_make_rsrc(p.x, (unsigned long long)p.N * p.H * p.W * p.ldx * 2);
    const ig_u32x4 rs_x2 = ig_make_rsrc(p.x2 ? p.x2 : p.x, (unsigned long long)p.N * p.H * p.W * (p.x2 ? p.ldx2 : p.ldx) * 2);
    const ig_u32x4 rs_ab = ig_make_rsrc(gnp ? (const void*)p.gn_ab : (const void*)p.w, gnp ? (unsigned long long)p.N * 2 * p.Cin * 4 : 16ull);
    unsigned wvo[WPIECES];
#pragma unroll
    for (int q = 0; q < WPIECES; ++q) {
      const int row = n0 + q * 8 + lr;
      wvo[q] = row < p.Cout ? (unsigned)row * (unsigned)p.ldw * 2u + ((q & 1) ? ck1 : ck0) : IG_OOB;
    }
    int hpx[HNEED];
    auto dma_w = [&](int kt, int ring, int q0, int q1) {
      const unsigned so = (unsigned)(kt0 + min(kt, nk - 1)) * 128u;
#pragma unroll
      for (int q = q0; q < q1; ++q) ig_lds_dma16(wring_lds + ring * WBYTES + q * 1024, wvo[q], rs_w, so);
    };
    auto dma_h = [&](int c, int h) {
      const int cb = (c_begin + min(c, nchunk - 1)) * 64;
      const bool second = cb >= p.C1;
      const unsigned ld2 = (unsigned)(second ? p.ldx2 : p.ldx) * 2u;
      const unsigned so = (unsigned)(second ? cb - p.C1 : cb) * 2u;
#pragma unroll
      for (int j = 0; j < HPER; ++j) {
        const int q = h * HPER + j;
        if (h < 16 && q < HNEED) {
          const unsigned vo = hpx[q] >= 0 ? (unsigned)hpx[q] * ld2 + ((q & 1) ? ck1 : ck0) : IG_OOB;
          const unsigned m0v = hbuf_lds + (c & 1) * HBYTES + q * 1024;
          if (second) ig_lds_dma16(m0v, vo, rs_x2, so);
          else ig_lds_dma16(m0v, vo, rs_x1, so);
        }
      }
    };
    auto halo_count = [](int h) -> int { return (h >= 16 || h * HPER >= HNEED) ? 0 : (HNEED - h * HPER < HPER ? HNEED - h * HPER : HPER); };
    auto dma_ab = [&](int c) {
      const unsigned vo = lane < 32 ? (unsigned)((img * 2 + (lane >> 4 & 1)) * p.Cin + (lane & 15) * 4) * 4u : IG_OOB;
      ig_lds_dma16(abuf_lds + (c & 1) * 1024, vo, rs_ab, (unsigned)((c_begin + min(c, nchunk - 1)) * 64) * 4u);
    };
    if (gnp && do_h) dma_ab(0);
    if (do_w) dma_w(1, 1, 0, WPIECES);
    if (do_h) {
#pragma unroll
      for (int q = 0; q < HNEED; ++q) hpx[q] = halo_pixel(q * 8 + lr);
    }
    if (gnp && do_h) {
      if (do_w) asm volatile("s_waitcnt vmcnt(%0)" ::"n"(WPIECES) : "memory");
      else asm volatile("s_waitcnt vmcnt(0)" ::: "memory");
    }
    __builtin_amdgcn_s_barrier();
    if (gnp) __builtin_amdgcn_s_barrier();
    for (int c = 0; c < nchunk; ++c) {
#pragma unroll
      for (int tap = 0; tap < 9; ++tap) {
        const int kt = c * 9 + tap;
        if (do_w) dma_w(kt + 2, (tap + 2) % 3, 0, WH);
        if (do_h) {
          dma_h(c + 1, 2 * tap);
          if (gnp && tap == 0) dma_ab(c + 1);
        }
        if (kt + 1 == nk) asm volatile("s_waitcnt vmcnt(0)" ::: "memory");
        else if (do_w && do_h) asm volatile("s_waitcnt vmcnt(%0)" ::"n"(WH + halo_count(2 * tap) + ((gnp && tap == 0) ? 1 : 0)) : "memory");
        else if (do_w) asm volatile("s_waitcnt vmcnt(%0)" ::"n"(WH) : "memory");
        else asm volatile("s_waitcnt vmcnt(%0)" ::"n"(halo_count(2 * tap) + ((gnp && tap == 0) ? 1 : 0)) : "memory");
        __builtin_amdgcn_s_barrier();
        if (kt + 1 < nk) {
          if (do_w) dma_w(kt + 2, (tap + 2) % 3, WH, WPIECES);
          if (do_h) dma_h(c + 1, 2 * tap + 1);
        }
        __builtin_amdgcn_s_barrier();
      }
    }
    return;
  }

  const int wm = wid % WM, wn = wid / WM;
  const int chunk = ps ^ ((((wid & 1) << 2) + (lr >> 1)) & 7);
  static_assert(HTAP % 2 == 0, "piece parity");
  int hpix[8];
#pragma unroll
  for (int t = 0; t < 8; ++t) hpix[t] = (wid < HTAP && t * HTAP + wid < HNEED) ? halo_pixel((t * HTAP + wid) * 8 + lr) : -1;
  {
    const ig_u32x4 rs_w = ig_make_rsrc(p.w, (unsigned long long)p.Cout * p.ldw * 2);
    const int cb = c_begin * 64;
    const bool second = cb >= p.C1;
    const ig_u32x4 rs_x = second ? ig_make_rsrc(p.x2, (unsigned long long)p.N * p.H * p.W * p.ldx2 * 2) : ig_make_rsrc(p.x, (unsigned long long)p.N * p.H * p.W * p.ldx * 2);
    const unsigned ld2 = (unsigned)(second ? p.ldx2 : p.ldx) * 2u, so = (unsigned)(second ? cb - p.C1 : cb) * 2u;
    if (wid_s < HTAP) {
#pragma unroll
      for (int t = 0; t < 8; ++t)
        if (t * HTAP + wid_s < HNEED)
          ig_lds_dma16(hbuf_lds + (t * HTAP + wid_s) * 1024, hpix[t] >= 0 ? (unsigned)hpix[t] * ld2 + chunk * 16u : IG_OOB, rs_x, so);
    }
#pragma unroll
    for (int j = 0; j < (WPIECES + NW - 1) / NW; ++j) {
      const int q = wid_s + NW * j;
      if (q < WPIECES) {
        const int row = n0 + q * 8 + lr;
        ig_lds_dma16(wring_lds + q * 1024, row < p.Cout ? (unsigned)row * (unsigned)p.ldw * 2u + chunk * 16u : IG_OOB, rs_w, (unsigned)kt0 * 128u);
      }
    }
  }
  auto gn_slot = [&](int c, int t) {
    if (hpix[t] >= 0)
      gn_piece_inplace<F16>(hbuf + (c & 1) * HBYTES + (t * HTAP + wid) * 1024 + lane * 16, gn_load_ab(abuf + (c & 1) * 1024, chunk), p.gn_silu != 0);
  };
  f32x16 acc[FN][FM];
#pragma unroll
  for (int a = 0; a < FN; ++a)
#pragma unroll
    for (int b = 0; b < FM; ++b)
#pragma unroll
      for (int e = 0; e < 16; ++e) acc[a][b][e] = 0.f;
  const int frow = lane & 31, fhalf = lane >> 5;
  const unsigned aw_lds = wring_lds + (wn * WTN + frow) * 128 + ((fhalf ^ ((frow >> 1) & 7)) << 4);
  static_assert(((WTN >> 1) & 7) == 0, "the wave's weight rows must keep the swizzle phase of fragment row 0");
  auto tap_addr = [&](int cc, int tp, unsigned (&ab)[FM]) -> unsigned {
    const int dy = tp / 3, dx = tp % 3;
#pragma unroll
    for (int b = 0; b < FM; ++b) {
      const int hrow = (wm * FM + b + dy) * PW + dx + frow;
      ab[b] = hbuf_lds + (cc & 1) * HBYTES + hrow * 128 + ((fhalf ^ ((hrow >> 1) & 7)) << 4);
    }
    return aw_lds + (tp % 3) * WBYTES;
  };
  KPipeRings<FM, FN> rings;
  kpipe_init(rings);
  asm volatile("s_waitcnt vmcnt(0)" ::: "memory");
  __builtin_amdgcn_s_barrier();
  if (gnp) {
#pragma unroll
    for (int t = 0; t < 8; ++t) gn_slot(0, t);
    asm volatile("s_waitcnt lgkmcnt(0)" ::: "memory");
    __builtin_amdgcn_s_barrier();
  }
  {
    unsigned ab0[FM];
    const unsigned aw0 = tap_addr(0, 0, ab0);
    kpipe<FM, FN, F16, 0>(acc, rings, ab0, aw0, ab0, aw0);
  }
  for (int c = 0; c < nchunk; ++c) {
    const bool next_chunk = c + 1 < nchunk;
#pragma unroll
    for (int tap = 0; tap < 9; ++tap) {
      if (gnp && tap >= 2 && next_chunk) gn_slot(c + 1, tap >= 2 ? tap - 2 : 0);
      if (gnp && tap == 0 && c > 0) gn_slot(c, 7);
      unsigned ab[FM], abn[FM];
      const unsigned aw = tap_addr(c, tap, ab), awn = tap_addr(c + (tap == 8 ? 1 : 0), (tap + 1) % 9, abn);
      kpipe<FM, FN, F16, 1>(acc, rings, ab, aw, abn, awn);
      __builtin_amdgcn_s_barrier();
      kpipe<FM, FN, F16, 2>(acc, rings, ab, aw, abn, awn);
      __builtin_amdgcn_s_barrier();
    }
  }
  kpipe_drain(rings);
  asm volatile("s_nop 15\n\ts_nop 7" ::: "memory");
  igemm_epilogue<FM, FN, WTM, WTN, BM, BN, NT, F16, false>(p, acc, m0, n0, wm, wn, lane, 0, sz, smem);
}

template <int TH, int BN, int WM, int WN>
struct HaloThin {
  static constexpr int NW = WM * WN, HPIX = (TH + 2) * 34, HSLOTS = (HPIX + 8 * NW - 1) / (8 * NW);
  static constexpr int HBYTES = HSLOTS * NW * 1024;
  static constexpr int lds = 2 * HBYTES + 3 * (BN * 128 > NW * 1024 ? BN * 128 : NW * 1024) + 2048;
  static_assert(lds <= 160 * 1024, "LDS budget");
  static int plan(ConvK& k, size_t) {
    k.tiles_m = k.N * (k.OH / TH) * (k.OW / 32);
    k.tiles_n = (k.Cout + BN - 1) / BN;
    k.splitk = 1;
    k.nk_per_split = k.nk;
    set_gn_plan(k, false, 0);
    return 0;
  }
  static int launch(ConvK& k, hipStream_t s) {
    k.patch_tw = 32;
    static ur::DeviceOnce attr_once;
    if (auto once_guard = attr_once.first()) {
      hipFuncSetAttribute(reinterpret_cast<const void*>(&igemm_halo_kernel<TH, BN, WM, WN, UR_TU_F16 != 0, false>), hipFuncAttributeMaxDynamicSharedMemorySize, lds);
    }
    UR_F16_SWITCH(k, hipLaunchKernelGGL((igemm_halo_kernel<TH, BN, WM, WN, F16, false>), dim3(k.tiles_m * k.tiles_n, 1), dim3(NW * 64), lds, s, k));
    return ur::check_launch("ur_conv2d_nhwc");
  }
};

template <int TH, int BN, int WM, int WN>
struct Halo {
  static constexpr int NW = WM * WN, BM = TH * 32, HPIX = (TH + 2) * 34, HSLOTS = (HPIX + 8 * NW - 1) / (8 * NW);
  static constexpr int HBYTES = HSLOTS * NW * 1024;
  static constexpr int lds_loop = 2 * HBYTES + 3 * BN * 128 + 2048, lds_epi = epi_lds_bytes<BM, BN, NW * 64>();
  static constexpr int lds = lds_loop > lds_epi ? lds_loop : lds_epi;
  static_assert(lds <= 160 * 1024, "LDS budget");
  static constexpr bool GN_OK = BN <= 128;
  static int plan(ConvK& k, size_t ws_bytes) {
    k.tiles_m = k.N * (k.OH / TH) * (k.OW / 32);
    k.tiles_n = (k.Cout + BN - 1) / BN;
    const int nchunk = k.nk / 9;
    const long long tiles = (long long)k.tiles_m * k.tiles_n;
    plan_splitk(k, ws_bytes, tiles <= 128 && k.ws && k.y ? std::min<long long>(256 / tiles, std::max(1, nchunk / 2)) : 1, 9);
    set_gn_plan(k, true, (k.OH / TH) * (k.OW / 32));
    return GN_OK;
  }
  static int launch(ConvK& k, hipStream_t s) {
    k.patch_tw = 32;
    static ur::DeviceOnce attr_once;
    if (auto once_guard = attr_once.first()) {
      hipFuncSetAttribute(reinterpret_cast<const void*>(&igemm_halo_kernel<TH, BN, WM, WN, UR_TU_F16 != 0, false>), hipFuncAttributeMaxDynamicSharedMemorySize, lds);
      hipFuncSetAttribute(reinterpret_cast<const void*>(&igemm_halo_kernel<TH, BN, WM, WN, UR_TU_F16 != 0, GN_OK>), hipFuncAttributeMaxDynamicSharedMemorySize, lds);
      hipFuncSetAttribute(reinterpret_cast<const void*>(&igemm_halo_ws_kernel<TH, BN, WM, WN, UR_TU_F16 != 0, false>), hipFuncAttributeMaxDynamicSharedMemorySize, lds);
      hipFuncSetAttribute(reinterpret_cast<const void*>(&igemm_halo_ws_kernel<TH, BN, WM, WN, UR_TU_F16 != 0, GN_OK>), hipFuncAttributeMaxDynamicSharedMemorySize, lds);
    }
    static const bool no_ws = getenv("UR_HALO_NOWS") != nullptr;
    if (no_ws) {
      if (GN_OK && k.gn_ab) UR_F16_SWITCH(k, hipLaunchKernelGGL((igemm_halo_kernel<TH, BN, WM, WN, F16, GN_OK>), dim3(k.tiles_m * k.tiles_n, k.splitk), dim3(NW * 64), lds, s, k));
      else UR_F16_SWITCH(k, hipLaunchKernelGGL((igemm_halo_kernel<TH, BN, WM, WN, F16, false>), dim3(k.tiles_m * k.tiles_n, k.splitk), dim3(NW * 64), lds, s, k));
    } else {
      static const bool ld1 = getenv("UR_HALO_LD1") != nullptr;
      const dim3 blk((NW + (ld1 ? 1 : 2)) * 64);
      if (GN_OK && k.gn_ab) UR_F16_SWITCH(k, hipLaunchKernelGGL((igemm_halo_ws_kernel<TH, BN, WM, WN, F16, GN_OK>), dim3(k.tiles_m * k.tiles_n, k.splitk), blk, lds, s, k));
      else UR_F16_SWITCH(k, hipLaunchKernelGGL((igemm_halo_ws_kernel<TH, BN, WM, WN, F16, false>), dim3(k.tiles_m * k.tiles_n, k.splitk), blk, lds, s, k));
    }
    if (k.splitk > 1) {
      k.patch_tw = 0;
      launch_splitk_reduce(k, s);
    }
    return ur::check_launch("ur_conv2d_nhwc");
  }
};

template <int TH, int TW, int NIMG, int BN, int WM, int WN, bool F16, bool GNP>
__global__ __launch_bounds__(WM* WN * 64) void igemm_halo_img_kernel(const ConvK p) {
  constexpr int NW = WM * WN, BM = TH * TW * NIMG, PW = TW + 2, HP = (TH + 2) * PW, HPIX = HP * NIMG;
  constexpr int HSLOTS = (HPIX + 8 * NW - 1) / (8 * NW);
  constexpr int HPIECES = HSLOTS * NW, HBYTES = HPIECES * 1024;
  constexpr int WBYTES = BN * 128, WPIECES = BN / 8, WPW = (WPIECES + NW - 1) / NW;
  constexpr int WTM = BM / WM, WTN = BN / WN, FM = WTM / 32, FN = WTN / 32, NT = NW * 64;
  static_assert(BM == 256 && NW == 8 && WTM % 32 == 0 && WTN % 32 == 0 && HSLOTS <= 8, "tile shape");
  extern __shared__ __attribute__((aligned(16))) unsigned char smem[];
  unsigned char* const hbuf = smem;
  unsigned char* const wring = smem + 2 * HBYTES;
  unsigned char* const abuf = wring + 3 * WBYTES;
  constexpr bool GN_OK = NIMG == 1 && HSLOTS <= 7;
  constexpr bool gnp = GN_OK && GNP;

  const int tid = threadIdx.x, lane = tid & 63, wid = tid >> 6;
  const int wm = wid % WM, wn = wid / WM;
  int sz = blockIdx.y, tn, tmi;
  if (p.wmajor) {
    const int L = blockIdx.x, xcd = L & 7, j = L >> 3;
    const int g = (j / p.tiles_m) * 8 + xcd;
    if (g >= p.tiles_n * p.splitk) return;
    tn = g % p.tiles_n; sz = g / p.tiles_n; tmi = j % p.tiles_m;
  } else {
    int id = blockIdx.x;
    const int nt = p.tiles_m * p.tiles_n, q = nt >> 3, r = nt & 7, xcd = id & 7, idx = id >> 3;
    id = (xcd < r ? xcd * (q + 1) : r * (q + 1) + (xcd - r) * q) + idx;
    tn = id % p.tiles_n; tmi = id / p.tiles_n;
  }
  const int n0 = tn * BN, img0 = tmi * NIMG, m0 = tmi * BM;

  typedef __attribute__((address_space(1))) const void* gptr_t;
  typedef __attribute__((address_space(3))) void* lptr_t;
  const uint16_t* __restrict__ X1 = p.x;
  const uint16_t* __restrict__ X2 = p.x2;
  const uint16_t* __restrict__ Wt = p.w;
  const uint16_t* zero = reinterpret_cast<const uint16_t*>(g_zero_page);
  const int lr = lane >> 3, ps = lane & 7;

  int hpix[HSLOTS], hchk[HSLOTS];
#pragma unroll
  for (int t = 0; t < HSLOTS; ++t) {
    const int hr = (t * NW + wid) * 8 + lr;
    const int im = hr / HP, rin = hr - im * HP, hy = rin / PW, hx = rin - hy * PW;
    const int iy = hy - 1, ix = hx - 1;
    const bool v = hr < HPIX && img0 + im < p.N && (unsigned)iy < (unsigned)TH && (unsigned)ix < (unsigned)TW;
    const int sy = p.ups ? iy >> 1 : iy, sx = p.ups ? ix >> 1 : ix;
    hpix[t] = v ? ((img0 + im) * p.H + sy) * p.W + sx : -1;
    hchk[t] = ps ^ (((rin >> 1) - hy) & 7);
  }
  const int wchunk = ps ^ ((((wid & 1) << 2) + (lr >> 1)) & 7);
  int woff[WPW];
#pragma unroll
  for (int i = 0; i < WPW; ++i) {
    const int qq = (wid + NW * i < WPIECES) ? wid + NW * i : wid;
    const int row = n0 + qq * 8 + lr;
    woff[i] = row < p.Cout ? row * p.ldw : -1;
  }
  const int nchunk_all = p.nk / 9, cps = p.nk_per_split / 9;
  const int c_begin = sz * cps, c_end = min(nchunk_all, c_begin + cps);
  const int nchunk = c_end - c_begin, nk = nchunk * 9, kt0 = c_begin * 9;

  const int wid_s = __builtin_amdgcn_readfirstlane(wid);
  const ig_u32x4 rs_w = ig_make_rsrc(Wt, (unsigned long long)p.Cout * p.ldw * 2);
  const ig_u32x4 rs_x1 = ig_make_rsrc(X1, (unsigned long long)p.N * p.H * p.W * p.ldx * 2);
  const ig_u32x4 rs_x2 = ig_make_rsrc(X2 ? X2 : X1, (unsigned long long)p.N * p.H * p.W * (X2 ? p.ldx2 : p.ldx) * 2);
  const unsigned wring_lds = (unsigned)(uintptr_t)(lptr_t)wring, hbuf_lds = (unsigned)(uintptr_t)(lptr_t)hbuf;
  unsigned wvo[WPW];
#pragma unroll
  for (int i = 0; i < WPW; ++i) wvo[i] = woff[i] >= 0 ? (unsigned)woff[i] * 2u + wchunk * 16u : IG_OOB;
  auto issue_w = [&](int kt, int ring) {
#pragma unroll
    for (int i = 0; i < WPW; ++i) {
      const int qq = (wid_s + NW * i < WPIECES) ? wid_s + NW * i : wid_s;
      ig_lds_dma16(wring_lds + ring * WBYTES + qq * 1024, wvo[i], rs_w, (unsigned)(kt0 + kt) * 128u);
    }
  };
  auto issue_h = [&](int c, int t) {
    const int cb = (c_begin + c) * 64;
    const bool second = cb >= p.C1;
    const unsigned ld2 = (unsigned)(second ? p.ldx2 : p.ldx) * 2u;
    const unsigned vo = hpix[t] >= 0 ? (unsigned)hpix[t] * ld2 + hchk[t] * 16u : IG_OOB;
    const unsigned m0v = hbuf_lds + (c & 1) * HBYTES + (t * NW + wid_s) * 1024;
    if (second) ig_lds_dma16(m0v, vo, rs_x2, (unsigned)(cb - p.C1) * 2u);
    else ig_lds_dma16(m0v, vo, rs_x1, (unsigned)cb * 2u);
  };
  auto issue_ab = [&](int c) {
    const float* t = p.gn_ab + ((long long)img0 * 2 + (lane >> 4 & 1)) * p.Cin + (c_begin + c) * 64 + (lane & 15) * 4;
    const void* g = lane < 32 ? (const void*)t : (const void*)zero;
    __builtin_amdgcn_global_load_lds((gptr_t)g, (lptr_t)(abuf + (c & 1) * 1024), 16, 0, 0);
  };
  auto gn_slot = [&](int c, int t) {
    if (hpix[t] >= 0)
      gn_piece_inplace<F16>(hbuf + (c & 1) * HBYTES + (t * NW + wid) * 1024 + lane * 16, gn_load_ab(abuf + (c & 1) * 1024, hchk[t]), p.gn_silu != 0);
  };

  f32x16 acc[FN][FM];
#pragma unroll
  for (int a = 0; a < FN; ++a)
#pragma unroll
    for (int b = 0; b < FM; ++b)
#pragma unroll
      for (int e = 0; e < 16; ++e) acc[a][b][e] = 0.f;
  const int frow = lane & 31, fhalf = lane >> 5;
  int hrow0[FM], hin0[FM], hy0[FM];
#pragma unroll
  for (int b = 0; b < FM; ++b) {
    const int pix = wm * WTM + b * 32 + frow;
    const int im = pix / (TH * TW), r = pix - im * (TH * TW), y = r / TW, x = r - y * TW;
    hin0[b] = y * PW + x;
    hrow0[b] = im * HP + hin0[b];
    hy0[b] = y;
  }
  const unsigned hb_lds = (unsigned)(uintptr_t)(lptr_t)hbuf;
  const unsigned aw_lds = (unsigned)(uintptr_t)(lptr_t)wring + (wn * WTN + frow) * 128 + ((fhalf ^ ((frow >> 1) & 7)) << 4);
  static_assert(((WTN >> 1) & 7) == 0, "the wave's weight rows must keep the swizzle phase of fragment row 0");

  if (gnp) issue_ab(0);
#pragma unroll
  for (int t = 0; t < HSLOTS; ++t) issue_h(0, t);
  issue_w(0, 0);
  if (nk > 1) {
    issue_w(1, 1);
    asm volatile("s_waitcnt vmcnt(%0)" ::"n"(WPW) : "memory");
  } else {
    asm volatile("s_waitcnt vmcnt(0)" ::: "memory");
  }
  if (gnp) {
#pragma unroll
    for (int t = 0; t < HSLOTS; ++t) gn_slot(0, t);
    asm volatile("s_waitcnt lgkmcnt(0)" ::: "memory");
  }
  __builtin_amdgcn_s_barrier();

  for (int c = 0; c < nchunk; ++c) {
    const unsigned char* hb = hbuf + (c & 1) * HBYTES;
    const bool next_chunk = c + 1 < nchunk;
#pragma unroll
    for (int tap = 0; tap < 9; ++tap) {
      const int kt = c * 9 + tap;
      const bool more_w = kt + 2 < nk;
      const bool more_h = tap < HSLOTS && next_chunk;
      if (more_w) issue_w(kt + 2, (tap + 2) % 3);
      if (tap < HSLOTS) { if (next_chunk) issue_h(c + 1, tap < HSLOTS ? tap : 0); }
      const bool ab_now = gnp && tap == 0 && next_chunk;
      if (ab_now) issue_ab(c + 1);
      if (gnp && tap >= 2 && tap - 2 < HSLOTS && next_chunk) gn_slot(c + 1, (tap >= 2 && tap - 2 < HSLOTS) ? tap - 2 : 0);
      if constexpr (ktile_asm_ok<FM, FN>()) {
        const int dy = tap / 3, dx = tap % 3;
        unsigned ab[FM];
#pragma unroll
        for (int b = 0; b < FM; ++b) {
          const int hsw = (((hin0[b] + dy * PW + dx) >> 1) - (hy0[b] + dy)) & 7;
          ab[b] = hb_lds + (c & 1) * HBYTES + (hrow0[b] + dy * PW + dx) * 128 + ((fhalf ^ hsw) << 4);
        }
        ktile_mma<FM, FN, F16>(acc, ab, aw_lds + (tap % 3) * WBYTES);
      } else {
        const int dy = tap / 3, dx = tap % 3;
        const unsigned char* wsm = wring + (tap % 3) * WBYTES;
        int hro[FM], hsw[FM];
#pragma unroll
        for (int b = 0; b < FM; ++b) {
          hro[b] = (hrow0[b] + dy * PW + dx) * 128;
          hsw[b] = (((hin0[b] + dy * PW + dx) >> 1) - (hy0[b] + dy)) & 7;
        }
#pragma unroll
        for (int ks = 0; ks < 4; ++ks) {
          const int slot = ks * 2 + fhalf;
          typename Frag<F16>::type bfr[FM], afr[FN];
#pragma unroll
          for (int b = 0; b < FM; ++b) bfr[b] = *reinterpret_cast<const typename Frag<F16>::type*>(hb + hro[b] + ((slot ^ hsw[b]) << 4));
#pragma unroll
          for (int a = 0; a < FN; ++a) {
            const int row = wn * WTN + a * 32 + frow;
            afr[a] = *reinterpret_cast<const typename Frag<F16>::type*>(wsm + row * 128 + ((slot ^ ((row >> 1) & 7)) << 4));
          }
#pragma unroll
          for (int a = 0; a < FN; ++a)
#pragma unroll
            for (int b = 0; b < FM; ++b)
              acc[a][b] = mfma16t(afr[a], bfr[b], acc[a][b]);
        }
      }
      if (ab_now) {
        if (more_w) asm volatile("s_waitcnt vmcnt(%0)" ::"n"(WPW + 2) : "memory");
        else asm volatile("s_waitcnt vmcnt(2)" ::: "memory");
      } else if (more_w && more_h) asm volatile("s_waitcnt vmcnt(%0)" ::"n"(WPW + 1) : "memory");
      else if (more_w) asm volatile("s_waitcnt vmcnt(%0)" ::"n"(WPW) : "memory");
      else if (more_h) asm volatile("s_waitcnt vmcnt(1)" ::: "memory");
      else asm volatile("s_waitcnt vmcnt(0)" ::: "memory");
      asm volatile("s_waitcnt lgkmcnt(0)" ::: "memory");
      __builtin_amdgcn_s_barrier();
    }
  }
  asm volatile("s_nop 15\n\ts_nop 7" ::: "memory");
  igemm_epilogue<FM, FN, WTM, WTN, BM, BN, NT, F16, false>(p, acc, m0, n0, wm, wn, lane, 0, sz, smem);
}

template <int TH, int TW, int NIMG, int BN, int WM, int WN, bool F16>
__global__ __launch_bounds__((WM * WN + 2) * 64) void igemm_halo_img_ws_kernel(const ConvK p) {
  constexpr int NW = WM * WN, BM = TH * TW * NIMG, PW = TW + 2, HP = (TH + 2) * PW, HPIX = HP * NIMG;
  constexpr int HSLOTS = (HPIX + 8 * NW - 1) / (8 * NW);
  constexpr int HPIECES = HSLOTS * NW, HBYTES = HPIECES * 1024;
  constexpr int WBYTES = BN * 128, WPIECES = BN / 8;
  constexpr int WTM = BM / WM, WTN = BN / WN, FM = WTM / 32, FN = WTN / 32, NT = NW * 64;
  static_assert(BM == 256 && NW == 8 && WTM % 32 == 0 && WTN % 32 == 0 && HSLOTS <= 8 && ktile_asm_ok<FM, FN>() && WPIECES % NW == 0, "tile shape");
  extern __shared__ __attribute__((aligned(16))) unsigned char smem[];
  unsigned char* const hbuf = smem;
  unsigned char* const wring = smem + 2 * HBYTES;
  typedef __attribute__((address_space(3))) void* lptr_t;

  const int tid = threadIdx.x, lane = tid & 63, wid = tid >> 6;
  const int wid_s = __builtin_amdgcn_readfirstlane(wid);
  int sz = blockIdx.y, tn, tmi;
  if (p.wmajor) {
    const int L = blockIdx.x, xcd = L & 7, j = L >> 3;
    const int g = (j / p.tiles_m) * 8 + xcd;
    if (g >= p.tiles_n * p.splitk) return;
    tn = g % p.tiles_n; sz = g / p.tiles_n; tmi = j % p.tiles_m;
  } else {
    int id = blockIdx.x;
    const int nt = p.tiles_m * p.tiles_n, q = nt >> 3, r = nt & 7, xcd = id & 7, idx = id >> 3;
    id = (xcd < r ? xcd * (q + 1) : r * (q + 1) + (xcd - r) * q) + idx;
    tn = id % p.tiles_n; tmi = id / p.tiles_n;
  }
  const int n0 = tn * BN, img0 = tmi * NIMG, m0 = tmi * BM;
  const int lr = lane >> 3, ps = lane & 7;
  const int nchunk_all = p.nk / 9, cps = p.nk_per_split / 9;
  const int c_begin = sz * cps, c_end = min(nchunk_all, c_begin + cps);
  const int nchunk = c_end - c_begin, nk = nchunk * 9, kt0 = c_begin * 9;
  const ig_u32x4 rs_w = ig_make_rsrc(p.w, (unsigned long long)p.Cout * p.ldw * 2);
  const ig_u32x4 rs_x1 = ig_make_rsrc(p.x, (unsigned long long)p.N * p.H * p.W * p.ldx * 2);
  const ig_u32x4 rs_x2 = ig_make_rsrc(p.x2 ? p.x2 : p.x, (unsigned long long)p.N * p.H * p.W * (p.x2 ? p.ldx2 : p.ldx) * 2);
  const unsigned wring_lds = (unsigned)(uintptr_t)(lptr_t)wring, hbuf_lds = (unsigned)(uintptr_t)(lptr_t)hbuf;

  auto piece_of = [&](int q, int& pix, int& chk) {
    const int hr = q * 8 + lr;
    const int im = hr / HP, rin = hr - im * HP, hy = rin / PW, hx = rin - hy * PW;
    const int iy = hy - 1, ix = hx - 1;
    const bool v = hr < HPIX && img0 + im < p.N && (unsigned)iy < (unsigned)TH && (unsigned)ix < (unsigned)TW;
    const int sy = p.ups ? iy >> 1 : iy, sx = p.ups ? ix >> 1 : ix;
    pix = v ? ((img0 + im) * p.H + sy) * p.W + sx : -1;
    chk = ps ^ (((rin >> 1) - hy) & 7);
  };
  auto dma_piece = [&](int c, int q, int pix, int chk) {
    const int cb = (c_begin + c) * 64;
    const bool second = cb >= p.C1;
    const unsigned ld2 = (unsigned)(second ? p.ldx2 : p.ldx) * 2u;
    const unsigned vo = pix >= 0 ? (unsigned)pix * ld2 + chk * 16u : IG_OOB;
    const unsigned m0v = hbuf_lds + (c & 1) * HBYTES + q * 1024;
    if (second) ig_lds_dma16(m0v, vo, rs_x2, (unsigned)(cb - p.C1) * 2u);
    else ig_lds_dma16(m0v, vo, rs_x1, (unsigned)cb * 2u);
  };
  auto wvo_of = [&](int q) -> unsigned {
    const int row = n0 + q * 8 + lr;
    const int wchunk = ps ^ ((((q & 1) << 2) + (lr >> 1)) & 7);
    return row < p.Cout ? (unsigned)row * (unsigned)p.ldw * 2u + wchunk * 16u : IG_OOB;
  };

  if (wid_s == NW) {
    unsigned wvo[WPIECES];
#pragma unroll
    for (int q = 0; q < WPIECES; ++q) wvo[q] = wvo_of(q);
    auto dma_w = [&](int kt, int ring) {
      const unsigned so = (unsigned)(kt0 + kt) * 128u;
#pragma unroll
      for (int q = 0; q < WPIECES; ++q) ig_lds_dma16(wring_lds + ring * WBYTES + q * 1024, wvo[q], rs_w, so);
    };
    if (nk > 1) dma_w(1, 1);
    asm volatile("s_waitcnt vmcnt(0)" ::: "memory");
    __builtin_amdgcn_s_barrier();
    for (int kt = 0; kt < nk; ++kt) {
      if (kt + 2 < nk) {
        dma_w(kt + 2, (kt + 2) % 3);
        asm volatile("s_waitcnt vmcnt(%0)" ::"n"(WPIECES) : "memory");
      } else {
        asm volatile("s_waitcnt vmcnt(0)" ::: "memory");
      }
      __builtin_amdgcn_s_barrier();
    }
    return;
  }
  if (wid_s == NW + 1) {
    int hpx[HPIECES];
#pragma unroll
    for (int q = 0; q < HPIECES; ++q) { int pix, chk; piece_of(q, pix, chk); hpx[q] = pix >= 0 ? pix * 8 + chk : -1; }
    __builtin_amdgcn_s_barrier();
// ... 109 lines not shown
```

### unirestore_amd/csrc/runtime.hip

```cpp
#include <cstring>
#include <mutex>
#include <sstream>
#include <vector>
#include <map>

#include "common.h"

namespace {
__global__ void zero_kernel(uint32_t* p, size_t n) {
  for (size_t i = blockIdx.x * (size_t)blockDim.x + threadIdx.x; i < n; i += (size_t)gridDim.x * blockDim.x) p[i] = 0u;
}
}

namespace ur {

void zero_async(void* ptr, size_t bytes, hipStream_t s) {
  const size_t n = bytes / 4;
  if (n == 0) return;
  const unsigned blocks = (unsigned)std::min<size_t>((n + 255) / 256, 1024);
  hipLaunchKernelGGL(zero_kernel, dim3(blocks), dim3(256), 0, s, (uint32_t*)ptr, n);
}

static thread_local std::string g_err;

void set_error(const std::string& msg) { g_err = msg; }
int fail(int code, const std::string& msg) {
  g_err = msg;
  return code;
}
int check_launch(const char* what) {
  hipError_t e = hipGetLastError();
  if (e != hipSuccess) return fail(UR_E_LAUNCH, std::string(what) + ": " + hipGetErrorString(e));
  return UR_OK;
}

struct ProfRec {
  const char* family;
  double flops, bytes;
  hipEvent_t a, b;
};
static std::mutex g_mu;
static bool g_prof_on = false;
static std::vector<ProfRec> g_recs;
static std::vector<hipEvent_t> g_pool;

static hipEvent_t get_event() {
  if (!g_pool.empty()) {
    hipEvent_t e = g_pool.back();
    g_pool.pop_back();
    return e;
  }
  hipEvent_t e;
  hipEventCreate(&e);
  return e;
}

ProfScope::ProfScope(const char* family, double flops, double bytes, hipStream_t s) : slot(-1), stream(s) {
  if (!g_prof_on) return;
  hipStreamCaptureStatus st = hipStreamCaptureStatusNone;
  if (hipStreamIsCapturing(s, &st) != hipSuccess || st != hipStreamCaptureStatusNone) return;
  std::lock_guard<std::mutex> lk(g_mu);
  ProfRec r{family, flops, bytes, get_event(), get_event()};
  hipEventRecord(r.a, s);
  g_recs.push_back(r);
  slot = (int)g_recs.size() - 1;
}
ProfScope::~ProfScope() {
  if (slot < 0) return;
  std::lock_guard<std::mutex> lk(g_mu);
  hipEventRecord(g_recs[slot].b, stream);
}

}

extern "C" {

int ur_version(void) { return 101; }
const char* ur_last_error(void) { return ur::g_err.c_str(); }

int ur_profile_enable(int on) {
  std::lock_guard<std::mutex> lk(ur::g_mu);
  ur::g_prof_on = on != 0;
  if (on) {
    for (auto& r : ur::g_recs) {
      ur::g_pool.push_back(r.a);
      ur::g_pool.push_back(r.b);
    }
    ur::g_recs.clear();
  }
  return UR_OK;
}

int ur_profile_report(char* buf, size_t buf_bytes) {
  std::lock_guard<std::mutex> lk(ur::g_mu);
  struct Agg { long n = 0; double ms = 0, flops = 0, bytes = 0; };
  std::map<std::string, Agg> agg;
  for (auto& r : ur::g_recs) {
    hipEventSynchronize(r.b);
    float ms = 0.f;
    hipEventElapsedTime(&ms, r.a, r.b);
    Agg& a = agg[r.family];
    a.n++; a.ms += ms; a.flops += r.flops; a.bytes += r.bytes;
  }
  std::ostringstream os;
  os << "{";
  bool first = true;
  for (auto& kv : agg) {
    if (!first) os << ", ";
    first = false;
    os << "\"" << kv.first << "\": {\"launches\": " << kv.second.n << ", \"ms\": " << kv.second.ms
       << ", \"flops\": " << kv.second.flops << ", \"bytes\": " << kv.second.bytes << "}";
  }
  os << "}";
  std::string s = os.str();
  if (s.size() + 1 > buf_bytes) return ur::fail(UR_E_INVALID, "ur_profile_report: buffer too small");
  memcpy(buf, s.c_str(), s.size() + 1);
  return UR_OK;
}

}
```

### unirestore_amd/modules/nn.py

```python
import math
from typing import Optional

import os

import torch
import torch.nn as nn

from .. import chain, ops
from ..ops import UR_ACT_GEGLU, UR_ACT_GELU, UR_ACT_NONE, UR_ACT_SILU

DEV = "cuda"
CHAIN = os.environ.get("UR_CHAIN", "1") == "1"


class _NoEager:
    def forward(self, *a, **k):
        raise RuntimeError(f"{type(self).__name__}: no eager/PyTorch path exists; use the HIP-backed graph")


class Conv2d(_NoEager, nn.Conv2d):
    def packed(self, pair=False, scale: Optional[torch.Tensor] = None) -> ops.PackedConv:
        key = ("pk", pair, ops.act_dtype())
        if key not in self.__dict__:
            w, b = self.weight, self.bias
            if scale is not None:
                s = scale.detach().reshape(-1)
                w = w * s[:, None, None, None]
                b = None if b is None else b * s
            self.__dict__[key] = ops.pack_conv(w, b, DEV, pair=pair, groups=self.groups)
        return self.__dict__[key]


class Linear(_NoEager, nn.Linear):
    def packed(self, pair=False) -> ops.PackedConv:
        key = ("pk", pair, ops.act_dtype())
        if key not in self.__dict__:
            self.__dict__[key] = ops.pack_conv(self.weight, self.bias, DEV, pair=pair)
        return self.__dict__[key]

    def dev_f32(self):
        if "f32" not in self.__dict__:
            self.__dict__["f32"] = (self.weight.detach().float().to(DEV).contiguous(),
                                    None if self.bias is None else self.bias.detach().float().to(DEV).contiguous())
        return self.__dict__["f32"]


class _Affine:
    def dev(self):
        if "aff" not in self.__dict__:
            self.__dict__["aff"] = (self.weight.detach().float().to(DEV).contiguous(),
                                    self.bias.detach().float().to(DEV).contiguous())
        return self.__dict__["aff"]


class GroupNorm(_NoEager, _Affine, nn.GroupNorm):
    def run(self, x, silu=False, x2=None):
        g, b = self.dev()
        return ops.group_norm(x, g, b, self.num_groups, self.eps, silu, x2=x2)

    def coeffs(self, x, x2=None):
        g, b = self.dev()
        return ops.gn_finalize(x, g, b, self.num_groups, self.eps, x2=x2)


class LayerNorm(_NoEager, _Affine, nn.LayerNorm):
    def run(self, x):
        g, b = self.dev()
        return ops.layer_norm(x, g, b, self.eps)


def invalidate_packed(model: nn.Module):
    for m in model.modules():
        for k in [k for k in m.__dict__ if k in ("aff", "f32", "dw", "vecs") or
                  (isinstance(k, tuple) and k[0] in ("pk", "cache", "fused", "ctx", "gb"))]:
            del m.__dict__[k]


def sinusoid_table(timesteps, dim: int) -> torch.Tensor:
    half = dim // 2
    freqs = torch.exp(-math.log(10000.0) * torch.arange(half, dtype=torch.float32) / half)
    ang = torch.as_tensor(list(timesteps), dtype=torch.float32).reshape(-1, 1) * freqs.reshape(1, -1)
    return torch.cat([torch.cos(ang), torch.sin(ang)], dim=-1)


class TimestepEmbedding(nn.Module):
    def __init__(self, in_dim, time_dim):
        super().__init__()
        self.linear_1 = Linear(in_dim, time_dim)
        self.linear_2 = Linear(time_dim, time_dim)

    def silu_emb(self, sin_table: torch.Tensor) -> torch.Tensor:
        w1, b1 = self.linear_1.dev_f32()
        w2, b2 = self.linear_2.dev_f32()
        h = ops.linear_f32(sin_table.to(DEV), w1, b1, UR_ACT_SILU)
        return ops.linear_f32(h, w2, b2, UR_ACT_SILU)


class ResnetBlock2D(nn.Module):
    def __init__(self, cin, cout, temb_channels=None, groups=32, eps=1e-5):
        super().__init__()
        self.norm1 = GroupNorm(groups, cin, eps=eps)
        self.conv1 = Conv2d(cin, cout, 3, padding=1)
        self.time_emb_proj = Linear(temb_channels, cout) if temb_channels else None
        self.norm2 = GroupNorm(groups, cout, eps=eps)
        self.conv2 = Conv2d(cout, cout, 3, padding=1)
        self.conv_shortcut = Conv2d(cin, cout, 1) if cin != cout else None
        self.tbias = None

    def set_time_table(self, silu_emb: torch.Tensor):
        for k in [k for k in self.__dict__ if isinstance(k, tuple) and k[:2] == ("cache", "tb_all")]:
            del self.__dict__[k]
        w, b = self.time_emb_proj.dev_f32()
        cb = self.conv1.bias.detach().float().to(DEV)
        self.tbias = ops.linear_f32(silu_emb, w, b + cb)

    def _tbias_all(self, b, steps=None):
        key = ("cache", "tb_all", b) if steps is None else ("cache", "tb_all", b, steps.start, steps.stop)
        if key not in self.__dict__:
            rows = self.tbias if steps is None else self.tbias[steps]
            self.__dict__[key] = rows.repeat_interleave(b, dim=0).contiguous()
        return self.__dict__[key]

    def run(self, x, x2=None, step=None, sample_bias=None, control=None):
        bias = None
        if self.time_emb_proj is not None:
            if sample_bias is not None:
                bias = sample_bias
            elif isinstance(step, str):
                bias = self._tbias_all(x.shape[0] // self.tbias.shape[0])
            elif isinstance(step, slice):
                bias = self._tbias_all(x.shape[0] // (step.stop - step.start), step)
            else:
                bias = self.tbias[step]
        h = gn_silu_conv(self.norm1, x, self.conv1.packed(), x2=x2, bias=bias, gn=True)
        pc2 = self.conv2.packed()
        if self.conv_shortcut is not None:
            sc = ops.conv(x, self.conv_shortcut.packed(), x2=x2)
        else:
            sc = x
        if control is not None and "spade" in self._modules:
            if x2 is not None and self.conv_shortcut is None:
                raise ValueError("identity shortcut cannot take a virtual concat")
            h = gn_silu_conv(self.norm2, h, pc2, gn=True)
            return self.spade.run(h, control[h.shape[2]], residual=sc)
        return gn_silu_conv(self.norm2, h, pc2, residual=sc, gn=True)


FUSE_GN_MIN_PIXELS = 256 * 256
FUSE_GN_MAX_COUT = 256


def gn_silu_conv(norm: "GroupNorm", x, pc, x2=None, **kw):
    ab = norm.coeffs(x, x2=x2)
    if x.shape[1] * x.shape[2] >= FUSE_GN_MIN_PIXELS and pc.cout_out <= FUSE_GN_MAX_COUT and \
            ops.conv_plan(x, pc, x2=x2, gn=kw.get("gn", False), gn_ab=True, residual=kw.get("residual") is not None).prologue_ok:
        return ops.conv(x, pc, x2=x2, gn_ab=ab, gn_silu=True, **kw)
    return ops.conv(ops.gn_apply(x, ab, silu=True, x2=x2), pc, **kw)


class Downsample2D(nn.Module):
    def __init__(self, c, padding):
        super().__init__()
        self.padding = padding
        self.conv = Conv2d(c, c, 3, stride=2, padding=padding)

    def run(self, x):
        n, h, w, _ = x.shape
        if self.padding == 0:
            return ops.conv(x, self.conv.packed(), stride=2, pad=(0, 0), out_hw=(h // 2, w // 2), gn=True)
        return ops.conv(x, self.conv.packed(), stride=2, pad=(1, 1), gn=True)


class Upsample2D(nn.Module):
    def __init__(self, c):
        super().__init__()
        self.conv = Conv2d(c, c, 3, padding=1)

    def run(self, x):
        return ops.conv(x, self.conv.packed(), upsample=True, gn=True)


class _ToOut(nn.ModuleList):
    def __init__(self, c):
        super().__init__([Linear(c, c), nn.Identity()])


Q_FOLD = math.log2(math.e)
LN2 = math.log(2.0)


def _scaled_first(ts, q_scale):
    ts = [None if t is None else t.detach().float() for t in ts]
    if q_scale != 1.0 and ts[0] is not None:
        ts[0] = ts[0] * q_scale
    return ts


def _fused_qkv(mod, names, q_scale=1.0):
    ck = ("cache", "qkv", ops.act_dtype(), q_scale)
    if ck not in mod.__dict__:
        ws = _scaled_first([getattr(mod, n).weight for n in names], q_scale)
        bs = _scaled_first([getattr(mod, n).bias for n in names], q_scale)
        mod.__dict__[ck] = ops.pack_conv(torch.cat(ws, 0), None if bs[0] is None else torch.cat(bs, 0), DEV)
    return mod.__dict__[ck]


def _fused_ln(mod, key, names, norm, pair=False, q_scale=1.0):
    ck = ("cache", "ln", key, ops.act_dtype(), q_scale)
    if ck not in mod.__dict__:
        ws = _scaled_first([getattr(mod, n).weight for n in names], q_scale)
        bs = _scaled_first([getattr(mod, n).bias for n in names], q_scale)
        mod.__dict__[ck] = ops.pack_linear_ln(torch.cat(ws, 0), None if bs[0] is None else torch.cat(bs, 0), norm.weight, norm.bias, norm.eps,
                                               DEV, pair=pair)
    return mod.__dict__[ck]


def self_attention(mod, h, heads, residual, gn_kw={}, ln=None, rows=False):
    b, t, c = h.shape
    d = c // heads
    ldvt = ops.round_up(t, 8)
    vt = torch.zeros((b, c, ldvt), dtype=h.dtype, device=h.device) if ldvt != t else \
        torch.empty((b, c, ldvt), dtype=h.dtype, device=h.device)
    scale = 1.0 / math.sqrt(d)
    qs = scale * Q_FOLD if d == 64 else 1.0
    if ln is not None:
        qk = ops.linear(h, _fused_ln(mod, "qkv", ("to_q", "to_k", "to_v"), ln[0], q_scale=qs), ln_stats=ln[1], yt=vt, n_split=2 * c, t_rows=t)
    else:
        qk = ops.linear(h, _fused_qkv(mod, ("to_q", "to_k", "to_v"), q_scale=qs), yt=vt, n_split=2 * c, t_rows=t)
    if d in (64, 128, 512):
        o = ops.attention(qk, qk[:, :, c:], vt, heads, d, t, t, LN2 if d == 64 else scale, ldq=3 * c, ldk=3 * c,
                          bs_q=t * 3 * c, bs_k=t * 3 * c, bs_vt=c * ldvt, batch=b)
    else:
        o = attention_gemm(qk[:, :, :c], qk[:, :, c:2 * c], vt, heads, d, t)
    return ops.linear(o, mod.to_out[0].packed(), residual=residual, rows=rows, **gn_kw)


def attention_gemm(q, k, vt, heads, d, t, s_bytes=256 << 20):
    b = q.shape[0]
    rows = max(256, min(t, (s_bytes // (4 * b * t)) // 256 * 256))
    out = torch.empty((b, t, heads * d), dtype=q.dtype, device=q.device)
    for hh in range(heads):
        qh, kh, vh = q[:, :, hh * d:(hh + 1) * d], k[:, :, hh * d:(hh + 1) * d], vt[:, hh * d:(hh + 1) * d, :]
        for r0 in range(0, t, rows):
            r1 = min(t, r0 + rows)
            s = ops.bmm_nt(qh[:, r0:r1], kh, out_f32=True, out_scale=1.0 / math.sqrt(d))
            p = ops.softmax_rows(s, ldp=vt.shape[-1])
            out[:, r0:r1, hh * d:(hh + 1) * d] = ops.bmm_nt(p, vh)
    return out


class AttentionBlock(nn.Module):

    def __init__(self, c, head_dim, groups=32, eps=1e-5):
        super().__init__()
        self.heads = c // head_dim
        self.group_norm = GroupNorm(groups, c, eps=eps)
        self.to_q, self.to_k, self.to_v = Linear(c, c), Linear(c, c), Linear(c, c)
        self.to_out = _ToOut(c)

    def run(self, x):
        n, hh, ww, c = x.shape
        h = self.group_norm.run(x).view(n, hh * ww, c)
        o = self_attention(self, h, self.heads, x.view(n, hh * ww, c), gn_kw=dict(gn=True, gn_hw=(n, hh * ww)))
        return ops.carry(o, o.view(n, hh, ww, c))


class CrossAttention(nn.Module):
    def __init__(self, c, heads, kv_dim=None):
        super().__init__()
        self.heads = heads
        kv_dim = kv_dim or c
        self.to_q = Linear(c, c, bias=False)
        self.to_k = Linear(kv_dim, c, bias=False)
        self.to_v = Linear(kv_dim, c, bias=False)
        self.to_out = _ToOut(c)

    def context_kv(self, ctx: torch.Tensor):
        key = ("cache", "ctx", ops.act_dtype())
        if key not in self.__dict__:
            tk = ctx.shape[1]
            c = self.to_q.out_features
            kv = _fused_qkv(self, ("to_k", "to_v"))
            vt = torch.zeros((1, c, ops.round_up(tk, 8)), dtype=ctx.dtype, device=DEV)
            k = ops.linear(ctx, kv, yt=vt, n_split=c, t_rows=tk)
            self.__dict__[key] = (k, vt, tk)
        return self.__dict__[key]

    def run_cross(self, h, ctx, residual, ln=None, rows=False):
        b, t, c = h.shape
        d = c // self.heads
        k, vt, tk = self.context_kv(ctx)
        if ln is not None:
            q = ops.linear(h, _fused_ln(self, "q", ("to_q",), ln[0]), ln_stats=ln[1])
        else:
            q = ops.linear(h, self.to_q.packed())
        o = ops.attention(q, k, vt, self.heads, d, t, tk, 1.0 / math.sqrt(d), ldq=c, ldk=2 * c, bs_q=t * c, bs_k=0,
                          bs_vt=0, batch=b)
        return ops.linear(o, self.to_out[0].packed(), residual=residual, rows=rows)


class GEGLU(nn.Module):
    def __init__(self, c, inner):
        super().__init__()
        self.proj = Linear(c, inner * 2)


class FeedForward(nn.Module):
    def __init__(self, c):
        super().__init__()
        self.net = nn.ModuleList([GEGLU(c, 4 * c), nn.Identity(), Linear(4 * c, c)])

    def run(self, h, residual, ln=None):
        if ln is not None:
            a = ops.linear(h, _fused_ln(self.net[0], "proj", ("proj",), ln[0], pair=True), ln_stats=ln[1], act=UR_ACT_GEGLU)
        else:
            a = ops.linear(h, self.net[0].proj.packed(pair=True), act=UR_ACT_GEGLU)
        return ops.linear(a, self.net[2].packed(), residual=residual)


class BasicTransformerBlock(nn.Module):
    def __init__(self, c, heads, cross_dim):
        super().__init__()
        self.norm1, self.attn1 = LayerNorm(c), CrossAttention(c, heads)
        self.norm2, self.attn2 = LayerNorm(c), CrossAttention(c, heads, cross_dim)
        self.norm3, self.ff = LayerNorm(c), FeedForward(c)

    def run(self, h, ctx):
        st = ops.ln_of(h)
        if st is None:
            h = self_attention(self.attn1, self.norm1.run(h), self.attn1.heads, h)
            h = self.attn2.run_cross(self.norm2.run(h), ctx, h)
            return self.ff.run(self.norm3.run(h), h)
        h = self_attention(self.attn1, h, self.attn1.heads, h, ln=(self.norm1, st), rows=True)
        h = self.attn2.run_cross(h, ctx, h, ln=(self.norm2, ops.ln_of(h)), rows=True)
        return self.ff.run(h, h, ln=(self.norm3, ops.ln_of(h)))


class Transformer2DModel(nn.Module):
    def __init__(self, c, heads, cross_dim, groups=32):
        super().__init__()
        self.norm = GroupNorm(groups, c, eps=1e-6)
        self.proj_in = Linear(c, c)
        self.transformer_blocks = nn.ModuleList([BasicTransformerBlock(c, heads, cross_dim)])
        self.proj_out = Linear(c, c)

    def _chain_streams(self, ctx):
        key = ("cache", "chain", ops.act_dtype())
        if key not in self.__dict__:
            b = self.transformer_blocks[0]
            ff1, ff2 = b.ff.net[0].proj, b.ff.net[2]
            qs = Q_FOLD / math.sqrt(self.proj_in.weight.shape[0] // b.attn1.heads)
            head = chain.pack_head(self.proj_in.weight, self.proj_in.bias, b.attn1.to_q.weight.detach().float() * qs, b.attn1.to_k.weight,
                                   b.attn1.to_v.weight, b.norm1.weight, b.norm1.bias, DEV)
            tail = chain.pack_tail(b.attn1.to_out[0].weight, b.attn1.to_out[0].bias, b.attn2.to_q.weight, b.norm2.weight, b.norm2.bias,
                                   b.attn2.to_k.weight, b.attn2.to_v.weight, ctx[0].float(), b.attn2.to_out[0].weight, b.attn2.to_out[0].bias,
                                   ff1.weight, ff1.bias, ff2.weight, ff2.bias, b.norm3.weight, b.norm3.bias,
                                   self.proj_out.weight, self.proj_out.bias, b.attn2.heads, DEV)
            self.__dict__[key] = (head, tail)
        return self.__dict__[key]

    def _chain_ok(self, x, ctx):
        b = self.transformer_blocks[0]
        n, hh, ww, c = x.shape
        return (CHAIN and c == chain.CHAIN_C and (hh * ww) % chain.CHAIN_TOK == 0 and b.attn1.heads == 5 and b.attn2.heads == 5 and
                ctx.shape[0] == 1 and ctx.shape[1] <= 80 and b.attn1.to_q.bias is None and b.attn2.to_q.bias is None and
                b.norm1.eps == b.norm2.eps == b.norm3.eps and ff_hidden(b) == 4 * c and x.is_contiguous())

    def run(self, x, ctx):
        n, hh, ww, c = x.shape
        if self._chain_ok(x, ctx):
            b = self.transformer_blocks[0]
            head, tail = self._chain_streams(ctx)
            t, heads = hh * ww, b.attn1.heads
            d = c // heads
            h0, q, k, vt = chain.transformer_head_fused(x, self.norm.coeffs(x), head, n, b.norm1.eps)
            o1 = ops.attention(q, k, vt, heads, d, t, t, LN2, ldq=c, ldk=c, bs_q=t * c, bs_k=t * c, bs_vt=c * t, batch=n)
            y = chain.transformer_tail_fused(o1, h0, x, tail, n, 4 * c, heads, ctx.shape[1], b.norm1.eps, 1.0 / math.sqrt(d))
            return ops.carry(y, y.view(n, hh, ww, c))
        h = ops.linear(self.norm.run(x).view(n, hh * ww, c), self.proj_in.packed(), rows=True)
        h = self.transformer_blocks[0].run(h, ctx)
        o = ops.linear(h, self.proj_out.packed(), residual=x.view(n, hh * ww, c), gn=True, gn_hw=(n, hh * ww))
        return ops.carry(o, o.view(n, hh, ww, c))


def ff_hidden(block) -> int:
    return block.ff.net[2].in_features


class DownBlock(nn.Module):
    def __init__(self, cin, cout, temb, attn=None, heads=None, head_dim=None, cross_dim=None,
                 add_downsample=True, layers=2, groups=32, eps=1e-5):
        super().__init__()
        self.resnets = nn.ModuleList(
            [ResnetBlock2D(cin if i == 0 else cout, cout, temb, groups, eps) for i in range(layers)])
        self.attn_kind = attn
        if attn == "cross":
            self.attentions = nn.ModuleList([Transformer2DModel(cout, heads, cross_dim, groups) for _ in range(layers)])
        elif attn == "self":
            self.attentions = nn.ModuleList([AttentionBlock(cout, head_dim, groups, eps) for _ in range(layers)])
        self.downsamplers = nn.ModuleList([Downsample2D(cout, 1)]) if add_downsample else None


class MidBlock(nn.Module):
    def __init__(self, c, temb, attn, heads=None, head_dim=None, cross_dim=None, groups=32, eps=1e-5):
        super().__init__()
        self.resnets = nn.ModuleList([ResnetBlock2D(c, c, temb, groups, eps) for _ in range(2)])
        self.attn_kind = attn
        if attn == "cross":
            self.attentions = nn.ModuleList([Transformer2DModel(c, heads, cross_dim, groups)])
        else:
            self.attentions = nn.ModuleList([AttentionBlock(c, head_dim, groups, eps)])

    def run(self, h, step=None, ctx=None, sample_bias=None, control=None):
        sb = sample_bias or (None, None)
        h = self.resnets[0].run(h, step=step, sample_bias=sb[0], control=control)
        h = self.attentions[0].run(h, ctx) if self.attn_kind == "cross" else self.attentions[0].run(h)
        return self.resnets[1].run(h, step=step, sample_bias=sb[1], control=control)


class UpBlock(nn.Module):
    def __init__(self, cin, cout, prev, temb, attn=None, heads=None, cross_dim=None,
                 add_upsample=True, layers=3, groups=32, eps=1e-5):
        super().__init__()
        res = []
        for i in range(layers):
            skip = cin if i == layers - 1 else cout
            rin = prev if i == 0 else cout
            res.append(ResnetBlock2D(rin + skip, cout, temb, groups, eps))
        self.resnets = nn.ModuleList(res)
        self.attn_kind = attn
        if attn == "cross":
            self.attentions = nn.ModuleList([Transformer2DModel(cout, heads, cross_dim, groups) for _ in range(layers)])
        self.upsamplers = nn.ModuleList([Upsample2D(cout)]) if add_upsample else None


class UNet2DConditionModel(nn.Module):

    def __init__(self, in_channels=4, out_channels=4, block_out_channels=(320, 640, 1280, 1280),
                 heads=(5, 10, 20, 20), cross_dim=1024, groups=32, layers=2):
        super().__init__()
        ch = list(block_out_channels)
        self.time_proj_dim = ch[0]
        temb = ch[0] * 4
        self.time_embedding = TimestepEmbedding(ch[0], temb)
        self.conv_in = Conv2d(in_channels, ch[0], 3, padding=1)
        nb = len(ch)
        self.down_blocks = nn.ModuleList()
        out = ch[0]
        for i in range(nb):
            cin, out = out, ch[i]
            last = i == nb - 1
            self.down_blocks.append(DownBlock(cin, out, temb, attn=None if last else "cross", heads=heads[i],
                                              cross_dim=cross_dim, add_downsample=not last, layers=layers, groups=groups))
        self.mid_block = MidBlock(ch[-1], temb, "cross", heads=heads[-1], cross_dim=cross_dim, groups=groups)
        rev, rheads = ch[::-1], list(heads)[::-1]
        self.up_blocks = nn.ModuleList()
        out = rev[0]
        for i in range(nb):
            prev, out = out, rev[i]
            cin = rev[min(i + 1, nb - 1)]
            self.up_blocks.append(UpBlock(cin, out, prev, temb, attn=None if i == 0 else "cross", heads=rheads[i],
                                          cross_dim=cross_dim, add_upsample=i < nb - 1, layers=layers + 1, groups=groups))
        self.conv_norm_out = GroupNorm(groups, ch[0], eps=1e-5)
        self.conv_out = Conv2d(ch[0], out_channels, 3, padding=1)


class EncDownBlock(nn.Module):
    def __init__(self, cin, cout, add_downsample, groups, layers=2):
        super().__init__()
        self.resnets = nn.ModuleList(
            [ResnetBlock2D(cin if i == 0 else cout, cout, None, groups, 1e-6) for i in range(layers)])
        self.downsamplers = nn.ModuleList([Downsample2D(cout, 0)]) if add_downsample else None

    def run(self, h):
        for r in self.resnets:
            h = r.run(h)
        return self.downsamplers[0].run(h) if self.downsamplers is not None else h


class DecUpBlock(nn.Module):
    def __init__(self, cin, cout, add_upsample, groups, layers=3):
        super().__init__()
# ... 54 lines not shown
```

### unirestore_amd/ops.py

```python
from dataclasses import dataclass
from typing import Optional

import torch

from . import capi
from .capi import (UR_ACT_GATE, UR_ACT_GEGLU, UR_ACT_GELU, UR_ACT_NONE, UR_ACT_RELU, UR_ACT_SILU, UR_ACT_TANH, UR_DT_BF16,
                   UR_DT_F16, ConvDesc, ConvPlan, check, lib)

BF16 = torch.bfloat16
F16 = torch.float16
_ws = {}

_DTYPES = {"bf16": BF16, "bfloat16": BF16, BF16: BF16, "fp16": F16, "float16": F16, "f16": F16, "16": F16, F16: F16}
_act = BF16


def set_dtype(dt) -> torch.dtype:
    global _act
    if dt not in _DTYPES:
        raise ValueError(f"unsupported compute dtype {dt!r}: choose 'bf16' or 'fp16'")
    _act = _DTYPES[dt]
    return _act


def act_dtype() -> torch.dtype:
    return _act


def _dt(t: Optional[torch.Tensor] = None) -> int:
    d = _act if t is None else t.dtype
    if d == BF16:
        return UR_DT_BF16
    if d == F16:
        return UR_DT_F16
    raise TypeError(f"expected a bf16 / fp16 tensor, got {d}")


def _stream():
    return torch.cuda.current_stream().cuda_stream


def _ptr(t: Optional[torch.Tensor]):
    return None if t is None else t.data_ptr()


def workspace(dev, nbytes=192 << 20) -> torch.Tensor:
    key = (dev, "splitk")
    if key not in _ws:
        _ws[key] = torch.empty(nbytes // 4, dtype=torch.float32, device=dev)
    return _ws[key]


def ln_of(t):
    return getattr(t, "_ln", None)


def gn_of(t):
    return getattr(t, "_gn", None)


def carry(src, dst):
    g = getattr(src, "_gn", None)
    if g is not None:
        dst._gn = g
    r = getattr(src, "_ln", None)
    if r is not None:
        dst._ln = r
    return dst


def round_up(v, m):
    return (v + m - 1) // m * m


@dataclass
class PackedConv:
    w: torch.Tensor
    bias: Optional[torch.Tensor]
    cin: int
    cout: int
    cout_out: int
    k: int
    groups: int = 1
    pair: bool = False
    ln_colsum: Optional[torch.Tensor] = None
    ln_eps: float = 0.0
    kcm: bool = False
    w_frag: Optional[torch.Tensor] = None

    def frag(self) -> torch.Tensor:
        if self.w_frag is None:
            nt, nc = self.cout // 128, self.cin // 64
            w = self.w.view(nt, 4, 32, nc, 9, 4, 2, 8)
            self.w_frag = w.permute(0, 3, 4, 5, 1, 6, 2, 7).contiguous()
        return self.w_frag


def wants_frag(pc: "PackedConv", n, h, w_, c1, c2, stride, upsample, groups) -> bool:
    return (pc.k == 3 and pc.kcm and groups == 1 and stride == 1 and not upsample and h == 8 and w_ == 8 and n <= 16 and not pc.pair
            and pc.cout % 128 == 0 and (c1 + c2) % 256 == 0 and (c1 + c2) >= 512 and (c2 == 0 or c1 % 64 == 0))


def pack_conv(weight: torch.Tensor, bias: Optional[torch.Tensor], dev, *, pair=False, groups=1, cin_pad=None, c1=None, group_halo=False) -> PackedConv:
    w = weight.detach().to(dev, torch.float32)
    if w.dim() == 2:
        w = w[:, :, None, None]
    cout, cin_g, kh, kw = w.shape
    assert kh == kw and kh in (1, 3)
    cin_p = cin_pad or round_up(cin_g, 8)
    cout_p = round_up(cout, 8)
    if groups > 1:
        assert cin_g % 8 == 0 and (cout // groups) % 4 == 0
    if cin_p == cin_g and cout_p == cout:
        wp = w.permute(0, 2, 3, 1).contiguous()
    else:
        wp = torch.zeros(cout_p, kh, kw, cin_p, dtype=torch.float32, device=dev)
        wp[:cout, :, :, :cin_g] = w.permute(0, 2, 3, 1)
    b = None
    if bias is not None:
        b = torch.zeros(cout_p, dtype=torch.float32, device=dev)
        b[:cout] = bias.detach().to(dev, torch.float32)
    cout_out = cout_p
    if pair:
        half = cout // 2
        if cout % 2 or half % 32:
            raise NotImplementedError(f"UR_E_UNSUPPORTED: pair activations (GEGLU / SimpleGate) need (Cout/2) % 32 == 0, got {half}")
        idx = torch.arange(cout, device=dev).view(2, half // 32, 32).permute(1, 0, 2).reshape(-1)
        wp = wp[idx]
        b = b[idx] if b is not None else None
        cout_out = half
    kcm = kh == 3 and (groups == 1 or (group_halo and cout_p == cout)) and cin_p % 64 == 0 and (c1 is None or c1 % 64 == 0)
    if kcm:
        wp = wp.reshape(cout_p, kh * kw, cin_p // 64, 64).permute(0, 2, 1, 3)
    return PackedConv(wp.reshape(cout_p, kh * kw * cin_p).to(_act).contiguous(),
                      None if b is None else b.contiguous(), cin_p, cout_p, cout_out, kh, groups, pair, kcm=kcm)


def _conv_desc(x, pc: PackedConv, x2, stride, pad, upsample, out_hw, plan_only) -> ConvDesc:
    n, h, w_, c1 = x.shape
    c2 = 0 if x2 is None else x2.shape[-1]
    k, g = pc.k, pc.groups
    if pad is None:
        pad = (k // 2, k // 2)
    if out_hw is None:
        hin, win = (h * 2, w_ * 2) if upsample else (h, w_)
        out_hw = ((hin + 2 * pad[0] - k) // stride + 1, (win + 2 * pad[1] - k) // stride + 1)
    d = ConvDesc()
    d.dtype = _dt(x)
    if plan_only:
        d.x, d.x2, d.w = 16, (16 if c2 else None), 16
    else:
        d.x, d.x2, d.w = _ptr(x), _ptr(x2), _ptr(pc.w)
    ws = workspace(x.device)
    d.workspace, d.workspace_bytes = ws.data_ptr(), ws.numel() * 4
    d.N, d.H, d.W = n, h, w_
    d.C1, d.ldx, d.C2, d.ldx2 = (c1 // g if g > 1 else c1), c1, c2, c2
    d.Cout, d.ldw, d.ldy = pc.cout // g, pc.w.shape[1], pc.cout_out
    d.KH = d.KW = k
    d.stride, d.pad_t, d.pad_l = stride, pad[0], pad[1]
    d.OH, d.OW = out_hw
    d.upsample2x, d.out_scale = int(upsample), 1.0
    d.k_chunk_major = int(pc.kcm and (c2 == 0 or c1 % 64 == 0))
    if wants_frag(pc, n, h, w_, c1, c2, stride, upsample, g) and pad == (1, 1):
        d.w_frag = 16 if plan_only else pc.frag().data_ptr()
    d.nbatch = g
    if g > 1:
        d.bs_x, d.bs_w, d.bs_bias, d.bs_y, d.bs_r = c1 // g, (pc.cout // g) * pc.w.shape[1], pc.cout // g, pc.cout_out // g, pc.cout_out // g
    return d


def conv(x: torch.Tensor, pc: PackedConv, *, x2=None, residual=None, bias=None, act=UR_ACT_NONE, stride=1, pad=None,
         out_hw=None, upsample=False, out_f32=False, out_scale=1.0, out=None, yt=None, n_split=0, t_rows=0,
         gn=False, store=True, rows=False, ln_stats=None, gn_ab=None, gn_silu=False):
    if x.dtype not in (BF16, F16) or x.dtype != pc.w.dtype or not x.is_contiguous() or x.dim() != 4:
        raise ValueError(f"conv: x must be a contiguous 4-d {pc.w.dtype} tensor, got {x.dtype} {tuple(x.shape)}")
    n, h, w_, c1 = x.shape
    c2 = 0 if x2 is None else x2.shape[-1]
    if (c1 + c2) != pc.cin * pc.groups:
        raise ValueError(f"conv: Cin mismatch: {c1}+{c2} vs {pc.cin}*{pc.groups}")
    d = _conv_desc(x, pc, x2, stride, pad, upsample, out_hw, plan_only=False)
    assert not pc.kcm or d.k_chunk_major, "chunk-major weights need a 64-aligned concat boundary"
    oh, ow = d.OH, d.OW
    co_total = pc.cout_out
    if out is None and store:
        out = torch.empty((n, oh, ow, co_total), dtype=torch.float32 if out_f32 else x.dtype, device=x.device)
    bias_t = pc.bias if bias is None else bias
    d.bias = _ptr(bias_t)
    if bias is not None and bias.dim() == 2 and bias.shape[0] > 1:
        d.bias_img_stride = bias.shape[1]
    d.residual, d.y, d.yt = _ptr(residual), _ptr(out), _ptr(yt)
    if ln_stats is not None:
        assert pc.ln_colsum is not None, "weights were not packed with pack_linear_ln"
        st, parts = ln_stats
        d.ln_stats, d.ln_colsum, d.ln_eps, d.ln_dim, d.ln_parts = st.data_ptr(), pc.ln_colsum.data_ptr(), pc.ln_eps, pc.cin, parts
    if gn_ab is not None:
        d.gn_ab, d.gn_silu = gn_ab.data_ptr(), int(gn_silu)
    if out is not None:
        d.ldy = out.shape[-1]
    d.ldr = residual.shape[-1] if residual is not None else 0
    d.act, d.out_f32, d.out_scale = act, int(out_f32), out_scale
    d.n_split, d.t_rows = n_split, t_rows
    d.t_ld = yt.shape[-1] if yt is not None else 0
    stats = rstats = None
    if gn or rows:
        if gn:
            d.gn_part = 16
        if rows:
            d.row_stats = 16
        plan = ConvPlan()
        check(lib.ur_conv2d_plan(d, plan))
        if gn:
            if not store and not plan.gn_fused:
                raise NotImplementedError("store=False needs a launch whose epilogue writes the statistics (conv_plan().gn_fused)")
            stats = (torch.empty((n, plan.gn_parts, co_total, 2), dtype=torch.float32, device=x.device), plan.gn_parts)
            d.gn_part = stats[0].data_ptr()
        if rows:
            rstats = (torch.empty((plan.row_stat_parts, n * oh * ow, 2), dtype=torch.float32, device=x.device), plan.row_stat_parts)
            d.row_stats = rstats[0].data_ptr()
    check(lib.ur_conv2d_nhwc(d, _stream()))
    if not store:
        return stats
    if stats is not None:
        out._gn = stats
    if rstats is not None:
        out._ln = rstats
    return out


def conv_plan(x: torch.Tensor, pc: PackedConv, *, x2=None, stride=1, pad=None, upsample=False, gn=False, gn_ab=False,
              act=UR_ACT_NONE, residual=False, store=True) -> ConvPlan:
    d = _conv_desc(x, pc, x2, stride, pad, upsample, None, plan_only=True)
    d.y = 16 if store else None
    d.residual = 16 if residual else None
    d.gn_part = 16 if gn else None
    d.gn_ab = 16 if gn_ab else None
    d.ldr = pc.cout_out if residual else 0
    d.act = act
    plan = ConvPlan()
    check(lib.ur_conv2d_plan(d, plan))
    return plan


def conv_launch(x: torch.Tensor, pc: PackedConv, *, x2=None, stride=1, pad=None, upsample=False, gn=False, gn_ab=False,
                act=UR_ACT_NONE, residual=False, store=True):
    d = _conv_desc(x, pc, x2, stride, pad, upsample, None, plan_only=True)
    d.y = 16 if store else None
    d.residual = 16 if residual else None
    d.gn_part = 16 if gn else None
    d.gn_ab = 16 if gn_ab else None
    d.ldr = pc.cout_out if residual else 0
    d.act = act
    return capi.plan_launch(d)


def pack_linear_ln(weight, bias, gamma, beta, eps, dev, *, pair=False) -> PackedConv:
    w = weight.detach().to(dev, torch.float32)
    g, b0 = gamma.detach().to(dev, torch.float32), beta.detach().to(dev, torch.float32)
    wf = w * g[None, :]
    t = w @ b0 + (bias.detach().to(dev, torch.float32) if bias is not None else 0.0)
    pc = pack_conv(wf, t, dev, pair=pair)
    pc.ln_colsum = pc.w.float().sum(dim=1).contiguous()
    pc.ln_eps = float(eps)
    return pc


def linear(x: torch.Tensor, pc: PackedConv, **kw):
    shp = x.shape
    rows = x.numel() // shp[-1]
    res = kw.pop("residual", None)
    if res is not None:
        res = res.reshape(1, 1, rows, res.shape[-1])
    gn = kw.pop("gn", False)
    gn_hw = kw.pop("gn_hw", None)
    if kw.get("ln_stats") is None and getattr(pc, "ln_colsum", None) is not None:
        raise ValueError("LayerNorm-folded weights need ln_stats")
    if gn:
        n_img, hw = gn_hw
        y = conv(x.reshape(n_img, 1, hw, shp[-1]), pc, residual=None if res is None else res.reshape(n_img, 1, hw, -1), gn=True, **kw)
    else:
        y = conv(x.reshape(1, 1, rows, shp[-1]), pc, residual=res, **kw)
    return None if y is None else carry(y, y.reshape(*shp[:-1], y.shape[-1]))


def bmm_nt(a: torch.Tensor, bmat: torch.Tensor, *, out_f32=False, out_scale=1.0):
    B, M, K = a.shape
    N = bmat.shape[1]
    if a.dtype != bmat.dtype or a.dtype not in (BF16, F16):
        raise ValueError(f"bmm_nt: both operands must share one 16-bit type, got {a.dtype} and {bmat.dtype}")
    assert a.stride(2) == 1 and bmat.stride(2) == 1 and K % 8 == 0 and N % 4 == 0
    out = torch.empty((B, M, N), dtype=torch.float32 if out_f32 else a.dtype, device=a.device)
    d = ConvDesc()
    d.dtype = _dt(a)
    d.x, d.w, d.y = a.data_ptr(), bmat.data_ptr(), out.data_ptr()
    ws = workspace(a.device)
    d.workspace, d.workspace_bytes = ws.data_ptr(), ws.numel() * 4
    d.N, d.H, d.W, d.C1, d.ldx, d.Cout, d.ldw, d.ldy = 1, 1, M, K, a.stride(1), N, bmat.stride(1), N
    d.KH = d.KW = 1
    d.stride, d.OH, d.OW, d.out_f32, d.out_scale, d.nbatch = 1, 1, M, int(out_f32), out_scale, B
    d.bs_x, d.bs_w, d.bs_y = a.stride(0), bmat.stride(0), M * N
    check(lib.ur_conv2d_nhwc(d, _stream()))
    return out


def gn_partials(x: torch.Tensor):
    pre = gn_of(x)
    if pre is not None:
        return pre
    n, c = x.shape[0], x.shape[-1]
    hw = x.numel() // (n * c)
    parts = lib.ur_groupnorm_stats_parts(n, hw, c)
    if parts <= 0:
        check(parts if parts < 0 else -1)
    plane = torch.empty((n, parts, c, 2), dtype=torch.float32, device=x.device)
    check(lib.ur_groupnorm_stats(x.data_ptr(), plane.data_ptr(), n, hw, c, _dt(x), _stream()))
    return plane, parts


def gn_finalize(x: torch.Tensor, gamma, beta, groups: int, eps: float, x2=None, use_pre=True, want_mean=False):
    n, c1 = x.shape[0], x.shape[-1]
    c2 = 0 if x2 is None else x2.shape[-1]
    hw = x.numel() // (n * c1)
    if not use_pre:
        x = x.view(x.shape)
        x2 = None if x2 is None else x2.view(x2.shape)
    p1, n1 = gn_partials(x)
    p2, n2 = gn_partials(x2) if x2 is not None else (None, 0)
    out = torch.empty((n, groups) if want_mean else (n, 2, c1 + c2), dtype=torch.float32, device=x.device)
    check(lib.ur_groupnorm_finalize(p1.data_ptr(), n1, c1, _ptr(p2), n2, c2, _ptr(gamma), _ptr(beta), n, hw, groups, eps,
                                    None if want_mean else out.data_ptr(), out.data_ptr() if want_mean else None, _stream()))
    return out


def gn_finalize_planes(plane: torch.Tensor, parts: int, hw: int):
    n, c = plane.shape[0], plane.shape[2]
    out = torch.empty((n, c), dtype=torch.float32, device=plane.device)
    check(lib.ur_groupnorm_finalize(plane.data_ptr(), parts, c, None, 0, 0, None, None, n, hw, c, 0.0, None, out.data_ptr(), _stream()))
    return out


def gn_apply(x: torch.Tensor, ab: torch.Tensor, silu=False, x2=None):
    n, c1 = x.shape[0], x.shape[-1]
    c2 = 0 if x2 is None else x2.shape[-1]
    hw = x.numel() // (n * c1)
    out = torch.empty((*x.shape[:-1], c1 + c2), dtype=x.dtype, device=x.device)
    check(lib.ur_groupnorm_apply_act(x.data_ptr(), _ptr(x2), out.data_ptr(), ab.data_ptr(), n, hw, c1, c2, int(silu), _dt(x), _stream()))
    return out


def group_norm(x: torch.Tensor, gamma, beta, groups: int, eps: float, silu=False, x2=None, use_pre=True):
    assert x.dtype in (BF16, F16) and x.is_contiguous()
    return gn_apply(x, gn_finalize(x, gamma, beta, groups, eps, x2=x2, use_pre=use_pre), silu, x2=x2)


def layer_norm(x: torch.Tensor, gamma, beta, eps: float):
    assert x.dtype in (BF16, F16) and x.is_contiguous()
    c = x.shape[-1]
    out = torch.empty_like(x)
    check(lib.ur_layernorm_rows(x.data_ptr(), out.data_ptr(), _ptr(gamma), _ptr(beta), x.numel() // c, c, eps, _dt(x), _stream()))
    return out


def softmax_rows(s: torch.Tensor, ldp=None):
    cols = s.shape[-1]
    ldp = ldp or round_up(cols, 8)
    p = torch.empty((*s.shape[:-1], ldp), dtype=_act, device=s.device)
    check(lib.ur_softmax_rows_f32(s.data_ptr(), p.data_ptr(), s.numel() // cols, cols, ldp, _dt(), _stream()))
    return p


def attention(q, k, vt, heads: int, head_dim: int, tq: int, tk: int, scale: float, *, ldq, ldk, bs_q, bs_k, bs_vt,
              batch: int, out=None):
    c = heads * head_dim
    if not (q.dtype == k.dtype == vt.dtype) or q.dtype not in (BF16, F16):
        raise ValueError(f"attention: q, k, v^T must share one 16-bit type, got {q.dtype}, {k.dtype}, {vt.dtype}")
    out = torch.empty((batch, tq, c), dtype=q.dtype, device=q.device) if out is None else out
    nws = lib.ur_attention_workspace_bytes(batch, heads, tq, tk, head_dim)
    ws = torch.empty(nws, dtype=torch.uint8, device=q.device) if nws else None
    check(lib.ur_attention_fwd_ws(q.data_ptr(), k.data_ptr(), vt.data_ptr(), out.data_ptr(), batch, heads, tq, tk, head_dim,
                                  ldq, ldk, vt.shape[-1], c, bs_q, bs_k, bs_vt, tq * c, scale, _ptr(ws), nws, _dt(q), _stream()))
    return out


def dwconv3x3(x, w9c, bias, gate=False):
    n, h, w_, c = x.shape
    out = torch.empty((n, h, w_, c // 2 if gate else c), dtype=x.dtype, device=x.device)
    check(lib.ur_dwconv3x3_nhwc(x.data_ptr(), w9c.data_ptr(), bias.data_ptr(), out.data_ptr(), n, h, w_, c, int(gate), _dt(x), _stream()))
    return out


def avgpool(x):
    return gn_finalize(x, None, None, x.shape[-1], 0.0, want_mean=True)


def scale_channels(x, s, residual=None):
    n, c = x.shape[0], x.shape[-1]
    out = torch.empty_like(x)
    check(lib.ur_scale_channels(x.data_ptr(), s.data_ptr(), _ptr(residual), out.data_ptr(), n, x.numel() // (n * c), c, _dt(x), _stream()))
    return out


FANOUT_MAX_K = 8


def scale_channels_fanout(x, s, k):
    b, c = x.shape[0], x.shape[-1]
    if s is not None and (s.dtype != torch.float32 or tuple(s.shape) != (k * b, c) or not s.is_contiguous()):
        raise ValueError(f"scale_channels_fanout: s must be a contiguous fp32 [{k * b}, {c}] tensor, got {s.dtype} {tuple(s.shape)}")
    if not x.is_contiguous():
        raise ValueError("scale_channels_fanout: x must be contiguous")
    out = torch.empty((k * b, *x.shape[1:]), dtype=x.dtype, device=x.device)
    for k0 in range(0, k, FANOUT_MAX_K):
        check(lib.ur_scale_channels_fanout(x.data_ptr(), None if s is None else s[k0 * b:].data_ptr(), out[k0 * b:].data_ptr(), b,
                                           min(FANOUT_MAX_K, k - k0), x.numel() // (b * c), c, _dt(x), _stream()))
    return out


def spade_modulate(n, gb, residual=None):
    c = n.shape[-1]
    out = torch.empty_like(n)
    check(lib.ur_spade_modulate(n.data_ptr(), gb.data_ptr(), gb.shape[-1], _ptr(residual), out.data_ptr(), n.numel() // c, c, _dt(n), _stream()))
    return out


def axpy_channels(a, b, s):
    c = a.shape[-1]
    out = torch.empty_like(a)
    check(lib.ur_axpy_channels(a.data_ptr(), b.data_ptr(), s.data_ptr(), out.data_ptr(), a.numel() // c, c, _dt(a), _stream()))
    return out


def linear_f32(x, w, bias, act=UR_ACT_NONE, groups=1):
    m, k = x.shape
    n = w.shape[0]
    out = torch.empty((m, n), dtype=torch.float32, device=x.device)
    check(lib.ur_linear_f32(x.data_ptr(), w.data_ptr(), _ptr(bias), out.data_ptr(), m, n, k, groups, act, _stream()))
    return out


def tfa_prompt_update(pooled, cond):
    b, t, d = cond.shape
    upd = torch.empty_like(cond)
    check(lib.ur_tfa_prompt_update(pooled.data_ptr(), cond.data_ptr(), upd.data_ptr(), b, t, d, _stream()))
    return upd


def tfa_prompt_update_fanout(pooled, cond, b, k, cond_per_row):
    rows, t, d = cond.shape
    if rows != (k * b if cond_per_row else k) or pooled.shape[0] != b or pooled.numel() != b * 3 * t * d:
        raise ValueError(f"tfa_prompt_update_fanout: pooled {tuple(pooled.shape)} / cond {tuple(cond.shape)} do not fit b={b}, k={k}")
    if not (pooled.is_contiguous() and cond.is_contiguous() and pooled.dtype == cond.dtype == torch.float32):
        raise ValueError("tfa_prompt_update_fanout: pooled and cond must be contiguous fp32 tensors")
    upd = torch.empty((k * b, t, d), dtype=torch.float32, device=cond.device)
    check(lib.ur_tfa_prompt_update_fanout(pooled.data_ptr(), cond.data_ptr(), upd.data_ptr(), b, k, t, d, int(bool(cond_per_row)), _stream()))
    return upd


def vec_mul_group(a, b, groups):
    out = torch.empty_like(a)
    check(lib.ur_vec_mul_group(a.data_ptr(), b.data_ptr(), out.data_ptr(), a.shape[0], a.shape[1], groups, _stream()))
    return out


def nchw_to_nhwc(x: torch.Tensor, cpad=None, image=False):
    x = x.contiguous().float()
    n, c, h, w_ = x.shape
    cpad = cpad or round_up(c, 8)
    out = torch.empty((n, h, w_, cpad), dtype=_act, device=x.device)
# ... 173 lines not shown
```

Baseline: 30.12 images/s.

## Fold nearest-upsample into 3x3 conv as four 2x2 sub-pixel kernels

Adds a folded path for upsample-by-2 followed by a 3x3 conv. The weights are precomputed into four parity-specific 2x2 kernels, and the halo implicit-GEMM kernel runs 4 taps instead of 9 on the low-resolution input. This removes over half the MACs and the halo loads in decoder upsample convs. In exchange it needs an extra folded weight buffer, changes the tile-to-output mapping and the GN partial-stat indexing, and adds forced-launcher entry points. The fold is packed in bf16 from summed fp32 weights, so rounding differs slightly from the unfolded path.

```diff
diff --git a/include/unirestore_hip.h b/include/unirestore_hip.h
--- a/include/unirestore_hip.h
+++ b/include/unirestore_hip.h
@@ -62,6 +62,7 @@
   long long bias_img_stride;
   int dtype;
   const void* w_frag;
+  const void* w_fold;
 } ur_conv_desc;
 
 int ur_conv2d_nhwc(const ur_conv_desc* d, ur_stream_t stream);
@@ -82,8 +83,12 @@
   int reduce_ri;
   int gn_pass;
   int group_loop;
+  int workgroups;
+  int folded;
 } ur_conv_launch_info;
 int ur_conv2d_plan_launch(const ur_conv_desc* d, ur_conv_launch_info* info);
+int ur_conv2d_nhwc_as(const ur_conv_desc* d, int launcher, ur_stream_t stream);
+int ur_conv2d_plan_as(const ur_conv_desc* d, int launcher, ur_conv_plan* plan, ur_conv_launch_info* info);
 int ur_conv_launcher_count(void);
 const char* ur_conv_launcher_name(int i);
 
diff --git a/unirestore_amd/capi.py b/unirestore_amd/capi.py
--- a/unirestore_amd/capi.py
+++ b/unirestore_amd/capi.py
@@ -29,7 +29,7 @@
         ("nbatch", C.c_int),
         ("bs_x", C.c_longlong), ("bs_x2", C.c_longlong), ("bs_w", C.c_longlong), ("bs_bias", C.c_longlong),
         ("bs_y", C.c_longlong), ("bs_r", C.c_longlong), ("k_chunk_major", C.c_int), ("bias_img_stride", C.c_longlong),
-        ("dtype", C.c_int), ("w_frag", C.c_void_p),
+        ("dtype", C.c_int), ("w_frag", C.c_void_p), ("w_fold", C.c_void_p),
     ]
 
 
@@ -39,7 +39,7 @@
 
 class ConvLaunchInfo(C.Structure):
     _fields_ = [("launcher", C.c_int), ("splitk", C.c_int), ("nk_per_split", C.c_int), ("reduce", C.c_int), ("reduce_ri", C.c_int),
-                ("gn_pass", C.c_int), ("group_loop", C.c_int)]
+                ("gn_pass", C.c_int), ("group_loop", C.c_int), ("workgroups", C.c_int), ("folded", C.c_int)]
 
 
 class AttentionPlan(C.Structure):
@@ -54,6 +54,8 @@
     "ur_conv2d_nhwc": (_I, [C.POINTER(ConvDesc), _P]),
     "ur_conv2d_plan": (_I, [C.POINTER(ConvDesc), C.POINTER(ConvPlan)]),
     "ur_conv2d_plan_launch": (_I, [C.POINTER(ConvDesc), C.POINTER(ConvLaunchInfo)]),
+    "ur_conv2d_nhwc_as": (_I, [C.POINTER(ConvDesc), _I, _P]),
+    "ur_conv2d_plan_as": (_I, [C.POINTER(ConvDesc), _I, C.POINTER(ConvPlan), C.POINTER(ConvLaunchInfo)]),
     "ur_conv_launcher_count": (_I, []),
     "ur_conv_launcher_name": (C.c_char_p, [_I]),
     "ur_gemm_bias_act": (_I, [_P, _P, _P, _P, _P, _LL, _I, _I, _I, _I, _I, _I, _I, _P, _SZ, _I, _P]),
diff --git a/unirestore_amd/csrc/igemm.hip b/unirestore_amd/csrc/igemm.hip
--- a/unirestore_amd/csrc/igemm.hip
+++ b/unirestore_amd/csrc/igemm.hip
@@ -11,7 +11,14 @@
 
 namespace {
 
-ConvLaunch dispatch_conv(ConvK& k, bool pair, size_t ws_bytes) {
+ConvLaunch dispatch_conv(ConvK& k, bool pair, size_t ws_bytes, int force = -1) {
+  if (force >= 0) {
+    const bool halo_ok = k.KH == 3 && k.stride == 1 && k.pad_t == 1 && k.pad_l == 1 && k.kcm && k.staged_ok_ && !pair && k.nbatch == 1 &&
+                         k.OW % 32 == 0 && k.OH % 8 == 0 && k.OH == (k.ups ? 2 * k.H : k.H) && k.OW == (k.ups ? 2 * k.W : k.W) && !k.yt;
+    if (halo_ok && force == UR_LAUNCHER_halo_8x32_160) return urk::halo_8x32_160(k, ws_bytes);
+    if (halo_ok && force == UR_LAUNCHER_halo_8x32_128) return urk::halo_8x32_128(k, ws_bytes);
+    return ConvLaunch{nullptr, 0, -1};
+  }
   if (k.KH == 3 && k.stride == 1 && k.pad_t == 1 && k.pad_l == 1 && k.kcm && k.staged_ok_ && !pair && k.nbatch == 1 &&
       k.OW % 32 == 0 && k.OH % 8 == 0 && k.OH == (k.ups ? 2 * k.H : k.H) && k.OW == (k.ups ? 2 * k.W : k.W) && !k.yt) {
     const bool ok128 = k.Cout % 128 == 0, ok160 = k.Cout % 160 == 0;
@@ -91,7 +98,7 @@
 
 }
 
-static int conv_impl(const ur_conv_desc* d, ur_stream_t stream, ur_conv_plan* plan, ur_conv_launch_info* info = nullptr) {
+static int conv_impl(const ur_conv_desc* d, ur_stream_t stream, ur_conv_plan* plan, ur_conv_launch_info* info = nullptr, int force = -1) {
   UR_REQUIRE(d && d->x && d->w, "null x/w");
   UR_REQUIRE(d->KH == d->KW && (d->KH == 1 || d->KH == 3), "only 1x1 and 3x3 kernels");
   UR_REQUIRE(d->C1 > 0 && d->C1 % 8 == 0 && d->C2 % 8 == 0 && d->ldx % 8 == 0, "Cin/ldx must be multiples of 8");
@@ -124,6 +131,10 @@
                  (long long)d->Cout * d->ldw < (1ll << 31), "tensor too large for 32-bit element offsets");
 
   k.kcm = d->k_chunk_major; k.wf = (const uint16_t*)d->w_frag; k.wmajor = 0; k.xgm = 0; k.xbn = 0; k.patch_tw = 0;
+  k.tiles_m = k.tiles_n = 0; k.splitk = 1;
+  k.wfold = d->upsample2x && d->KH == 3 ? (const uint16_t*)d->w_fold : nullptr; k.fold = 0;
+  UR_REQUIRE(!(k.wfold && d->gn_ab), "w_fold does not combine with gn_ab (the folded loader has no GroupNorm pass)");
+  UR_REQUIRE(!k.wfold || (d->k_chunk_major && d->C2 == 0), "w_fold needs chunk-major weights and a single source");
   UR_REQUIRE(!k.kcm || (k.Cin % 64 == 0 && d->C1 % 64 == 0), "k_chunk_major needs C1 and C1+C2 to be multiples of 64");
   k.gn_part = d->gn_part; k.gn_ab = d->gn_ab; k.gn_silu = d->gn_silu; k.f16 = d->dtype == UR_DT_F16; k.gn_fused = 0; k.gn_parts = 0;
   k.ln_parts = d->ln_parts;
@@ -145,8 +156,9 @@
              k.nbatch, d->act);
     fam = interned.emplace(buf, 0).first->first.c_str();
   }
-  const ConvLaunch launch = dispatch_conv(k, pair, d->workspace_bytes);
-  const bool group_loop = k.nbatch > 1 && d->KH == 3 && k.kcm && k.stride == 1 && !pair && !k.gn_part && !k.row_stats && !k.ln_stats &&
+  const ConvLaunch launch = dispatch_conv(k, pair, d->workspace_bytes, force);
+  if (!launch.launch) return ur::fail(UR_E_UNSUPPORTED, "ur_conv2d_nhwc_as: this launcher cannot be forced, or does not cover the descriptor");
+  const bool group_loop = force < 0 && k.nbatch > 1 && d->KH == 3 && k.kcm && k.stride == 1 && !pair && !k.gn_part && !k.row_stats && !k.ln_stats &&
                           !k.yt && !k.gn_ab && !k.out_f32 && k.staged_ok_ && k.Cout % 128 == 0 && !k.bias_img && k.C2 == 0;
   auto group_k = [&](int b) {
     ConvK kb = k;
@@ -169,6 +181,7 @@
     info->reduce = r.kind; info->reduce_ri = r.ri;
     info->gn_pass = k.gn_part && !k.gn_fused && !group_loop;
     info->group_loop = group_loop;
+    info->workgroups = kb.tiles_m * kb.tiles_n * kb.splitk * kb.nbatch; info->folded = kb.fold;
   }
   if (plan || info) return UR_OK;
   if (!d->y && d->gn_part && (!k.gn_fused || k.splitk > 1))
@@ -204,6 +217,18 @@
   return conv_impl(&t, nullptr, plan);
 }
 
+extern "C" int ur_conv2d_nhwc_as(const ur_conv_desc* d, int launcher, ur_stream_t stream) {
+  UR_REQUIRE(launcher >= 0 && launcher < UR_CONV_LAUNCHER_COUNT, "no such launcher");
+  return conv_impl(d, stream, nullptr, nullptr, launcher);
+}
+extern "C" int ur_conv2d_plan_as(const ur_conv_desc* d, int launcher, ur_conv_plan* plan, ur_conv_launch_info* info) {
+  UR_REQUIRE(d && (plan || info) && launcher >= 0 && launcher < UR_CONV_LAUNCHER_COUNT, "null pointer / no such launcher");
+  ur_conv_desc t = *d;
+  if (!t.y && !t.yt && !t.gn_part) t.y = reinterpret_cast<void*>(16);
+  if (plan) { const int rc = conv_impl(&t, nullptr, plan, nullptr, launcher); if (rc != UR_OK) return rc; }
+  return info ? conv_impl(&t, nullptr, nullptr, info, launcher) : UR_OK;
+}
+
 extern "C" int ur_conv2d_plan_launch(const ur_conv_desc* d, ur_conv_launch_info* info) {
   UR_REQUIRE(d && info, "null pointer");
   ur_conv_desc t = *d;
diff --git a/unirestore_amd/csrc/igemm_impl.h b/unirestore_amd/csrc/igemm_impl.h
--- a/unirestore_amd/csrc/igemm_impl.h
+++ b/unirestore_amd/csrc/igemm_impl.h
@@ -32,6 +32,8 @@
   const uint16_t* wf;
   int wmajor;
   int xgm, xbn;
+  const uint16_t* wfold;
+  int fold;
 };
 
 __device__ __forceinline__ void xcd_tile_map(const ConvK& p, int id, int& tm, int& tn) {
@@ -67,7 +69,7 @@
 __device__ __forceinline__ bool is_pair_act(int act) { return act == UR_ACT_GEGLU || act == UR_ACT_GATE; }
 
 __device__ __forceinline__ int tile_row_to_m(const ConvK& p, int m0, int r) {
-  return p.patch_tw ? m0 + (r / p.patch_tw) * p.OW + (r % p.patch_tw) : m0 + r;
+  return p.patch_tw ? m0 + (((r / p.patch_tw) * p.OW + (r % p.patch_tw)) << p.fold) : m0 + r;
 }
 
 template <bool F16>
@@ -349,7 +351,11 @@
     __syncthreads();
     const int ctot = pair ? p.Cout / 2 : p.Cout;
     const int img = m0 / p.OHW, rem = m0 - img * p.OHW;
-    const int pm = p.patch_tw ? ((rem / p.OW) / (BM / p.patch_tw)) * (p.OW / p.patch_tw) + (rem % p.OW) / p.patch_tw : rem / BM;
+    int pm = p.patch_tw ? ((rem / p.OW) / (BM / p.patch_tw)) * (p.OW / p.patch_tw) + (rem % p.OW) / p.patch_tw : rem / BM;
+    if (p.fold) {
+      const int orow = rem / p.OW, ocol = rem - orow * p.OW;
+      pm = ((((orow >> 1) / (BM / p.patch_tw)) * (p.W / p.patch_tw) + (ocol >> 1) / p.patch_tw) << 2) + ((orow & 1) << 1) + (ocol & 1);
+    }
     float* st = p.gn_part + ((((long long)img * p.gn_parts + pm) * p.nbatch + gb) * ctot + c0) * 2;
     for (int i = threadIdx.x; i < cmax; i += NT) {
       const int c2 = i >> 1, odd = i & 1;
@@ -1567,15 +1573,18 @@
   igemm_epilogue<FM, FN, WTM, WTN, BM, BN, NT, F16, BN == 32>(p, acc, m0, n0, wm, wn, lane, 0, sz, smem);
 }
 
-template <int TH, int BN, int WM, int WN, bool F16, bool GNP>
+template <int TH, int BN, int WM, int WN, bool F16, bool GNP, bool FOLD = false>
 __global__ __launch_bounds__((WM * WN + 2) * 64) void igemm_halo_ws_kernel(const ConvK p) {
   constexpr int NW = WM * WN, TW = 32, BM = TH * TW, PW = TW + 2, HPIX = (TH + 2) * PW;
   constexpr int HSLOTS = (HPIX + 8 * NW - 1) / (8 * NW), HNEED = (HPIX + 7) / 8;
   constexpr int HPIECES = HSLOTS * NW, HBYTES = HPIECES * 1024;
-  constexpr int HPER = (HNEED + 15) / 16, HTAP = 2 * HPER;
+  constexpr int NTAP = FOLD ? 4 : 9, NHT = 2 * (NTAP - 1);
+  constexpr int HPER = (HNEED + NHT - 1) / NHT, HTAP = 2 * HPER;
+  constexpr int PSTR = FOLD ? NW : HTAP;
+  static_assert(!(FOLD && GNP), "the folded form has no in-LDS GroupNorm pass");
   constexpr int WBYTES = BN * 128, WPIECES = BN / 8, WH = WPIECES / 2;
   constexpr int WTM = BM / WM, WTN = BN / WN, FM = WTM / 32, FN = WTN / 32, NT = NW * 64;
-  static_assert(NW == 8 && WTM % 32 == 0 && WTN % 32 == 0 && HTAP <= NW && ktile_asm_ok<FM, FN>(), "wave layout");
+  static_assert(NW == 8 && WTM % 32 == 0 && WTN % 32 == 0 && PSTR <= NW && PSTR % 2 == 0 && 8 * PSTR >= HNEED && ktile_asm_ok<FM, FN>(), "wave layout");
   extern __shared__ __attribute__((aligned(16))) unsigned char smem[];
   unsigned char* const hbuf = smem;
   unsigned char* const wring = smem + 2 * HBYTES;
@@ -1591,21 +1600,26 @@
     const int nt = p.tiles_m * p.tiles_n, q = nt >> 3, r = nt & 7, xcd = id & 7, idx = id >> 3;
     id = (xcd < r ? xcd * (q + 1) : r * (q + 1) + (xcd - r) * q) + idx;
   }
-  const int tn = id % p.tiles_n, tmi = id / p.tiles_n;
-  const int tiles_x = p.OW / TW, tiles_y = p.OH / TH;
+  const int tn = id % p.tiles_n, tmf = id / p.tiles_n;
+  const int par = FOLD ? tmf & 3 : 0, py = par >> 1, px = par & 1, tmi = FOLD ? tmf >> 2 : tmf;
+  const int gh = FOLD ? p.H : p.OH, gw = FOLD ? p.W : p.OW;
+  const int tiles_x = gw / TW, tiles_y = gh / TH;
   const int tx = tmi % tiles_x, ty = (tmi / tiles_x) % tiles_y, img = tmi / (tiles_x * tiles_y);
   const int n0 = tn * BN;
-  const int m0 = img * p.OHW + ty * TH * p.OW + tx * TW;
-  const int cps = p.nk_per_split / 9, c_begin = sz * cps, nchunk = min(p.nk / 9, c_begin + cps) - c_begin;
-  const int nk = nchunk * 9, kt0 = c_begin * 9;
+  const int m0 = FOLD ? img * p.OHW + (2 * ty * TH + py) * p.OW + 2 * tx * TW + px : img * p.OHW + ty * TH * p.OW + tx * TW;
+  const int cps = p.nk_per_split / NTAP, c_begin = sz * cps, nchunk = min(p.nk / NTAP, c_begin + cps) - c_begin;
+  const int nk = nchunk * NTAP, kt0 = c_begin * NTAP;
+  const uint16_t* const wbase = FOLD ? p.wfold + par * 4 * p.Cin : p.w;
+  const unsigned wld = FOLD ? 16u * (unsigned)p.Cin : (unsigned)p.ldw;
+  const unsigned long long wbytes = (unsigned long long)p.Cout * wld * 2 - (FOLD ? (unsigned long long)par * 8 * p.Cin : 0ull);
   const unsigned wring_lds = (unsigned)(uintptr_t)(lptr_t)wring, hbuf_lds = (unsigned)(uintptr_t)(lptr_t)hbuf;
   const unsigned abuf_lds = (unsigned)(uintptr_t)(lptr_t)abuf;
   const int lr = lane >> 3, ps = lane & 7;
   auto halo_pixel = [&](int hr) -> int {
     const int hy = hr / PW, hx = hr - hy * PW;
     int iy = ty * TH - 1 + hy, ix = tx * TW - 1 + hx;
-    const bool v = hr < HPIX && (unsigned)iy < (unsigned)p.OH && (unsigned)ix < (unsigned)p.OW;
-    if (p.ups) { iy >>= 1; ix >>= 1; }
+    const bool v = hr < HPIX && (unsigned)iy < (unsigned)gh && (unsigned)ix < (unsigned)gw;
+    if (!FOLD && p.ups) { iy >>= 1; ix >>= 1; }
     return v ? (img * p.H + iy) * p.W + ix : -1;
   };
 
@@ -1613,7 +1627,7 @@
     const bool two = blockDim.x > (NW + 1) * 64;
     const bool do_w = wid_s == NW, do_h = two ? wid_s == NW + 1 : true;
     const unsigned ck0 = (ps ^ ((lr >> 1) & 7)) * 16u, ck1 = (ps ^ ((4 + (lr >> 1)) & 7)) * 16u;
-    const ig_u32x4 rs_w = ig_make_rsrc(p.w, (unsigned long long)p.Cout * p.ldw * 2);
+    const ig_u32x4 rs_w = ig_make_rsrc(wbase, wbytes);
     const ig_u32x4 rs_x1 = ig_make_rsrc(p.x, (unsigned long long)p.N * p.H * p.W * p.ldx * 2);
     const ig_u32x4 rs_x2 = ig_make_rsrc(p.x2 ? p.x2 : p.x, (unsigned long long)p.N * p.H * p.W * (p.x2 ? p.ldx2 : p.ldx) * 2);
     const ig_u32x4 rs_ab = ig_make_rsrc(gnp ? (const void*)p.gn_ab : (const void*)p.w, gnp ? (unsigned long long)p.N * 2 * p.Cin * 4 : 16ull);
@@ -1621,7 +1635,7 @@
 #pragma unroll
     for (int q = 0; q < WPIECES; ++q) {
       const int row = n0 + q * 8 + lr;
-      wvo[q] = row < p.Cout ? (unsigned)row * (unsigned)p.ldw * 2u + ((q & 1) ? ck1 : ck0) : IG_OOB;
+      wvo[q] = row < p.Cout ? (unsigned)row * wld * 2u + ((q & 1) ? ck1 : ck0) : IG_OOB;
     }
     int hpx[HNEED];
     auto dma_w = [&](int kt, int ring, int q0, int q1) {
@@ -1637,7 +1651,7 @@
 #pragma unroll
       for (int j = 0; j < HPER; ++j) {
         const int q = h * HPER + j;
-        if (h < 16 && q < HNEED) {
+        if (h < NHT && q < HNEED) {
           const unsigned vo = hpx[q] >= 0 ? (unsigned)hpx[q] * ld2 + ((q & 1) ? ck1 : ck0) : IG_OOB;
           const unsigned m0v = hbuf_lds + (c & 1) * HBYTES + q * 1024;
           if (second) ig_lds_dma16(m0v, vo, rs_x2, so);
@@ -1645,7 +1659,7 @@
         }
       }
     };
-    auto halo_count = [](int h) -> int { return (h >= 16 || h * HPER >= HNEED) ? 0 : (HNEED - h * HPER < HPER ? HNEED - h * HPER : HPER); };
+    auto halo_count = [](int h) -> int { return (h >= NHT || h * HPER >= HNEED) ? 0 : (HNEED - h * HPER < HPER ? HNEED - h * HPER : HPER); };
     auto dma_ab = [&](int c) {
       const unsigned vo = lane < 32 ? (unsigned)((img * 2 + (lane >> 4 & 1)) * p.Cin + (lane & 15) * 4) * 4u : IG_OOB;
       ig_lds_dma16(abuf_lds + (c & 1) * 1024, vo, rs_ab, (unsigned)((c_begin + min(c, nchunk - 1)) * 64) * 4u);
@@ -1662,11 +1676,13 @@
     }
     __builtin_amdgcn_s_barrier();
     if (gnp) __builtin_amdgcn_s_barrier();
+    int cm = 0;
     for (int c = 0; c < nchunk; ++c) {
 #pragma unroll
-      for (int tap = 0; tap < 9; ++tap) {
-        const int kt = c * 9 + tap;
-        if (do_w) dma_w(kt + 2, (tap + 2) % 3, 0, WH);
+      for (int tap = 0; tap < NTAP; ++tap) {
+        const int kt = c * NTAP + tap;
+        const int ring2 = FOLD ? (cm + tap + 2) % 3 : (tap + 2) % 3;
+        if (do_w) dma_w(kt + 2, ring2, 0, WH);
         if (do_h) {
           dma_h(c + 1, 2 * tap);
           if (gnp && tap == 0) dma_ab(c + 1);
@@ -1677,39 +1693,39 @@
         else asm volatile("s_waitcnt vmcnt(%0)" ::"n"(halo_count(2 * tap) + ((gnp && tap == 0) ? 1 : 0)) : "memory");
         __builtin_amdgcn_s_barrier();
         if (kt + 1 < nk) {
-          if (do_w) dma_w(kt + 2, (tap + 2) % 3, WH, WPIECES);
+          if (do_w) dma_w(kt + 2, ring2, WH, WPIECES);
           if (do_h) dma_h(c + 1, 2 * tap + 1);
         }
         __builtin_amdgcn_s_barrier();
       }
+      cm = cm == 2 ? 0 : cm + 1;
     }
     return;
   }
 
   const int wm = wid % WM, wn = wid / WM;
   const int chunk = ps ^ ((((wid & 1) << 2) + (lr >> 1)) & 7);
-  static_assert(HTAP % 2 == 0, "piece parity");
   int hpix[8];
 #pragma unroll
-  for (int t = 0; t < 8; ++t) hpix[t] = (wid < HTAP && t * HTAP + wid < HNEED) ? halo_pixel((t * HTAP + wid) * 8 + lr) : -1;
+  for (int t = 0; t < 8; ++t) hpix[t] = (wid < PSTR && t * PSTR + wid < HNEED) ? halo_pixel((t * PSTR + wid) * 8 + lr) : -1;
   {
-    const ig_u32x4 rs_w = ig_make_rsrc(p.w, (unsigned long long)p.Cout * p.ldw * 2);
+    const ig_u32x4 rs_w = ig_make_rsrc(wbase, wbytes);
     const int cb = c_begin * 64;
     const bool second = cb >= p.C1;
     const ig_u32x4 rs_x = second ? ig_make_rsrc(p.x2, (unsigned long long)p.N * p.H * p.W * p.ldx2 * 2) : ig_make_rsrc(p.x, (unsigned long long)p.N * p.H * p.W * p.ldx * 2);
     const unsigned ld2 = (unsigned)(second ? p.ldx2 : p.ldx) * 2u, so = (unsigned)(second ? cb - p.C1 : cb) * 2u;
-    if (wid_s < HTAP) {
+    if (wid_s < PSTR) {
 #pragma unroll
       for (int t = 0; t < 8; ++t)
-        if (t * HTAP + wid_s < HNEED)
-          ig_lds_dma16(hbuf_lds + (t * HTAP + wid_s) * 1024, hpix[t] >= 0 ? (unsigned)hpix[t] * ld2 + chunk * 16u : IG_OOB, rs_x, so);
+        if (t * PSTR + wid_s < HNEED)
+          ig_lds_dma16(hbuf_lds + (t * PSTR + wid_s) * 1024, hpix[t] >= 0 ? (unsigned)hpix[t] * ld2 + chunk * 16u : IG_OOB, rs_x, so);
     }
 #pragma unroll
     for (int j = 0; j < (WPIECES + NW - 1) / NW; ++j) {
       const int q = wid_s + NW * j;
       if (q < WPIECES) {
         const int row = n0 + q * 8 + lr;
-        ig_lds_dma16(wring_lds + q * 1024, row < p.Cout ? (unsigned)row * (unsigned)p.ldw * 2u + chunk * 16u : IG_OOB, rs_w, (unsigned)kt0 * 128u);
+        ig_lds_dma16(wring_lds + q * 1024, row < p.Cout ? (unsigned)row * wld * 2u + chunk * 16u : IG_OOB, rs_w, (unsigned)kt0 * 128u);
       }
     }
   }
@@ -1727,14 +1743,14 @@
   const int frow = lane & 31, fhalf = lane >> 5;
   const unsigned aw_lds = wring_lds + (wn * WTN + frow) * 128 + ((fhalf ^ ((frow >> 1) & 7)) << 4);
   static_assert(((WTN >> 1) & 7) == 0, "the wave's weight rows must keep the swizzle phase of fragment row 0");
-  auto tap_addr = [&](int cc, int tp, unsigned (&ab)[FM]) -> unsigned {
-    const int dy = tp / 3, dx = tp % 3;
+  auto tap_addr = [&](int cc, int tp, unsigned (&ab)[FM], int ring = 0) -> unsigned {
+    const int dy = FOLD ? py + (tp >> 1) : tp / 3, dx = FOLD ? px + (tp & 1) : tp % 3;
 #pragma unroll
     for (int b = 0; b < FM; ++b) {
       const int hrow = (wm * FM + b + dy) * PW + dx + frow;
       ab[b] = hbuf_lds + (cc & 1) * HBYTES + hrow * 128 + ((fhalf ^ ((hrow >> 1) & 7)) << 4);
     }
-    return aw_lds + (tp % 3) * WBYTES;
+    return aw_lds + (FOLD ? ring : tp % 3) * WBYTES;
   };
   KPipeRings<FM, FN> rings;
   kpipe_init(rings);
@@ -1751,19 +1767,22 @@
     const unsigned aw0 = tap_addr(0, 0, ab0);
     kpipe<FM, FN, F16, 0>(acc, rings, ab0, aw0, ab0, aw0);
   }
+  int cm = 0;
   for (int c = 0; c < nchunk; ++c) {
     const bool next_chunk = c + 1 < nchunk;
 #pragma unroll
-    for (int tap = 0; tap < 9; ++tap) {
+    for (int tap = 0; tap < NTAP; ++tap) {
       if (gnp && tap >= 2 && next_chunk) gn_slot(c + 1, tap >= 2 ? tap - 2 : 0);
       if (gnp && tap == 0 && c > 0) gn_slot(c, 7);
       unsigned ab[FM], abn[FM];
-      const unsigned aw = tap_addr(c, tap, ab), awn = tap_addr(c + (tap == 8 ? 1 : 0), (tap + 1) % 9, abn);
+      const unsigned aw = tap_addr(c, tap, ab, (cm + tap) % 3);
+      const unsigned awn = tap_addr(c + (tap == NTAP - 1 ? 1 : 0), (tap + 1) % NTAP, abn, (cm + tap + 1) % 3);
       kpipe<FM, FN, F16, 1>(acc, rings, ab, aw, abn, awn);
       __builtin_amdgcn_s_barrier();
       kpipe<FM, FN, F16, 2>(acc, rings, ab, aw, abn, awn);
       __builtin_amdgcn_s_barrier();
     }
+    cm = cm == 2 ? 0 : cm + 1;
   }
   kpipe_drain(rings);
   asm volatile("s_nop 15\n\ts_nop 7" ::: "memory");
@@ -1803,14 +1822,18 @@
   static constexpr int lds = lds_loop > lds_epi ? lds_loop : lds_epi;
   static_assert(lds <= 160 * 1024, "LDS budget");
   static constexpr bool GN_OK = BN <= 128;
+  static bool folds(const ConvK& k) { return k.wfold && k.ups && k.C2 == 0 && !k.gn_ab && k.H % TH == 0 && k.W % 32 == 0; }
   static int plan(ConvK& k, size_t ws_bytes) {
-    k.tiles_m = k.N * (k.OH / TH) * (k.OW / 32);
+    k.fold = folds(k);
+    const int ntap = k.fold ? 4 : 9;
+    if (k.fold) k.nk = (k.Cin / 64) * 4;
+    k.tiles_m = k.fold ? k.N * (k.H / TH) * (k.W / 32) * 4 : k.N * (k.OH / TH) * (k.OW / 32);
     k.tiles_n = (k.Cout + BN - 1) / BN;
-    const int nchunk = k.nk / 9;
+    const int nchunk = k.nk / ntap;
     const long long tiles = (long long)k.tiles_m * k.tiles_n;
-    plan_splitk(k, ws_bytes, tiles <= 128 && k.ws && k.y ? std::min<long long>(256 / tiles, std::max(1, nchunk / 2)) : 1, 9);
-    set_gn_plan(k, true, (k.OH / TH) * (k.OW / 32));
-    return GN_OK;
+    plan_splitk(k, ws_bytes, tiles <= 128 && k.ws && k.y ? std::min<long long>(256 / tiles, std::max(1, nchunk / 2)) : 1, ntap);
+    set_gn_plan(k, true, k.fold ? (k.H / TH) * (k.W / 32) * 4 : (k.OH / TH) * (k.OW / 32));
+    return GN_OK && !k.fold;
   }
   static int launch(ConvK& k, hipStream_t s) {
     k.patch_tw = 32;
@@ -1820,9 +1843,12 @@
       hipFuncSetAttribute(reinterpret_cast<const void*>(&igemm_halo_kernel<TH, BN, WM, WN, UR_TU_F16 != 0, GN_OK>), hipFuncAttributeMaxDynamicSharedMemorySize, lds);
       hipFuncSetAttribute(reinterpret_cast<const void*>(&igemm_halo_ws_kernel<TH, BN, WM, WN, UR_TU_F16 != 0, false>), hipFuncAttributeMaxDynamicSharedMemorySize, lds);
       hipFuncSetAttribute(reinterpret_cast<const void*>(&igemm_halo_ws_kernel<TH, BN, WM, WN, UR_TU_F16 != 0, GN_OK>), hipFuncAttributeMaxDynamicSharedMemorySize, lds);
+      hipFuncSetAttribute(reinterpret_cast<const void*>(&igemm_halo_ws_kernel<TH, BN, WM, WN, UR_TU_F16 != 0, false, true>), hipFuncAttributeMaxDynamicSharedMemorySize, lds);
     }
     static const bool no_ws = getenv("UR_HALO_NOWS") != nullptr;
-    if (no_ws) {
+    if (k.fold) {
+      UR_F16_SWITCH(k, hipLaunchKernelGGL((igemm_halo_ws_kernel<TH, BN, WM, WN, F16, false, true>), dim3(k.tiles_m * k.tiles_n, k.splitk), dim3((NW + 2) * 64), lds, s, k));
+    } else if (no_ws) {
       if (GN_OK && k.gn_ab) UR_F16_SWITCH(k, hipLaunchKernelGGL((igemm_halo_kernel<TH, BN, WM, WN, F16, GN_OK>), dim3(k.tiles_m * k.tiles_n, k.splitk), dim3(NW * 64), lds, s, k));
       else UR_F16_SWITCH(k, hipLaunchKernelGGL((igemm_halo_kernel<TH, BN, WM, WN, F16, false>), dim3(k.tiles_m * k.tiles_n, k.splitk), dim3(NW * 64), lds, s, k));
     } else {
diff --git a/unirestore_amd/csrc/runtime.hip b/unirestore_amd/csrc/runtime.hip
--- a/unirestore_amd/csrc/runtime.hip
+++ b/unirestore_amd/csrc/runtime.hip
@@ -75,7 +75,7 @@
 
 extern "C" {
 
-int ur_version(void) { return 101; }
+int ur_version(void) { return 102; }
 const char* ur_last_error(void) { return ur::g_err.c_str(); }
 
 int ur_profile_enable(int on) {
diff --git a/unirestore_amd/modules/nn.py b/unirestore_amd/modules/nn.py
--- a/unirestore_amd/modules/nn.py
+++ b/unirestore_amd/modules/nn.py
@@ -19,7 +19,7 @@
 
 
 class Conv2d(_NoEager, nn.Conv2d):
-    def packed(self, pair=False, scale: Optional[torch.Tensor] = None) -> ops.PackedConv:
+    def packed(self, pair=False, scale: Optional[torch.Tensor] = None, fold=False) -> ops.PackedConv:
         key = ("pk", pair, ops.act_dtype())
         if key not in self.__dict__:
             w, b = self.weight, self.bias
@@ -27,7 +27,7 @@
                 s = scale.detach().reshape(-1)
                 w = w * s[:, None, None, None]
                 b = None if b is None else b * s
-            self.__dict__[key] = ops.pack_conv(w, b, DEV, pair=pair, groups=self.groups)
+            self.__dict__[key] = ops.pack_conv(w, b, DEV, pair=pair, groups=self.groups, fold=fold)
         return self.__dict__[key]
 
 
@@ -177,7 +177,7 @@
         self.conv = Conv2d(c, c, 3, padding=1)
 
     def run(self, x):
-        return ops.conv(x, self.conv.packed(), upsample=True, gn=True)
+        return ops.conv(x, self.conv.packed(fold=True), upsample=True, gn=True)
 
 
 class _ToOut(nn.ModuleList):
diff --git a/unirestore_amd/ops.py b/unirestore_amd/ops.py
--- a/unirestore_amd/ops.py
+++ b/unirestore_amd/ops.py
@@ -87,6 +87,8 @@
     ln_eps: float = 0.0
     kcm: bool = False
     w_frag: Optional[torch.Tensor] = None
+    w_fold: Optional[torch.Tensor] = None
+    fold_src: Optional[torch.Tensor] = None
 
     def frag(self) -> torch.Tensor:
         if self.w_frag is None:
@@ -95,13 +97,51 @@
             self.w_frag = w.permute(0, 3, 4, 5, 1, 6, 2, 7).contiguous()
         return self.w_frag
 
+    def fold(self) -> torch.Tensor:
+        if self.w_fold is None:
+            if self.fold_src is None:
+                raise ValueError("PackedConv.fold: the weights were not packed with pack_conv(fold=True) (the fold needs the fp32 master)")
+            w = self.fold_src.detach().to(self.w.device, torch.float32)
+            w4 = torch.zeros(self.cout, self.cin, 3, 3, dtype=torch.float32, device=self.w.device)
+            w4[:w.shape[0], :w.shape[1]] = w
+            self.w_fold = pack_fold(fold_upsample_weight(w4)).to(self.w.dtype)
+        return self.w_fold
+
+
+_FOLD_TAPS = (((0,), (1, 2)), ((0, 1), (2,)))
+
+
+def fold_upsample_weight(w: torch.Tensor) -> torch.Tensor:
+    cout, cin = w.shape[:2]
+    out = w.new_zeros(2, 2, cout, cin, 2, 2)
+    for py in range(2):
+        for px in range(2):
+            for a in range(2):
+                for b in range(2):
+                    for kh in _FOLD_TAPS[py][a]:
+                        for kw in _FOLD_TAPS[px][b]:
+                            out[py, px, :, :, a, b] += w[:, :, kh, kw]
+    return out
+
+
+def pack_fold(wf: torch.Tensor) -> torch.Tensor:
+    _, _, cout, cin, _, _ = wf.shape
+    w = wf.reshape(4, cout, cin // 64, 64, 4)
+    return w.permute(1, 0, 2, 4, 3).reshape(cout, 16 * cin).contiguous()
+
+
+def wants_fold(pc: "PackedConv", h, w_, c2, stride, upsample, groups) -> bool:
+    return ((pc.w_fold is not None or pc.fold_src is not None) and pc.k == 3 and pc.kcm and upsample and stride == 1 and groups == 1 and c2 == 0 and not pc.pair
+            and h % 8 == 0 and w_ % 32 == 0)
+
 
 def wants_frag(pc: "PackedConv", n, h, w_, c1, c2, stride, upsample, groups) -> bool:
     return (pc.k == 3 and pc.kcm and groups == 1 and stride == 1 and not upsample and h == 8 and w_ == 8 and n <= 16 and not pc.pair
             and pc.cout % 128 == 0 and (c1 + c2) % 256 == 0 and (c1 + c2) >= 512 and (c2 == 0 or c1 % 64 == 0))
 
 
-def pack_conv(weight: torch.Tensor, bias: Optional[torch.Tensor], dev, *, pair=False, groups=1, cin_pad=None, c1=None, group_halo=False) -> PackedConv:
+def pack_conv(weight: torch.Tensor, bias: Optional[torch.Tensor], dev, *, pair=False, groups=1, cin_pad=None, c1=None, group_halo=False,
+              fold=False) -> PackedConv:
     w = weight.detach().to(dev, torch.float32)
     if w.dim() == 2:
         w = w[:, :, None, None]
@@ -132,8 +172,11 @@
     kcm = kh == 3 and (groups == 1 or (group_halo and cout_p == cout)) and cin_p % 64 == 0 and (c1 is None or c1 % 64 == 0)
     if kcm:
         wp = wp.reshape(cout_p, kh * kw, cin_p // 64, 64).permute(0, 2, 1, 3)
-    return PackedConv(wp.reshape(cout_p, kh * kw * cin_p).to(_act).contiguous(),
-                      None if b is None else b.contiguous(), cin_p, cout_p, cout_out, kh, groups, pair, kcm=kcm)
+    pc = PackedConv(wp.reshape(cout_p, kh * kw * cin_p).to(_act).contiguous(),
+                    None if b is None else b.contiguous(), cin_p, cout_p, cout_out, kh, groups, pair, kcm=kcm)
+    if fold and kcm and groups == 1 and not pair:
+        pc.fold_src = weight
+    return pc
 
 
 def _conv_desc(x, pc: PackedConv, x2, stride, pad, upsample, out_hw, plan_only) -> ConvDesc:
@@ -163,6 +206,8 @@
     d.k_chunk_major = int(pc.kcm and (c2 == 0 or c1 % 64 == 0))
     if wants_frag(pc, n, h, w_, c1, c2, stride, upsample, g) and pad == (1, 1):
         d.w_frag = 16 if plan_only else pc.frag().data_ptr()
+    if wants_fold(pc, h, w_, c2, stride, upsample, g) and pad == (1, 1):
+        d.w_fold = 16 if plan_only else pc.fold().data_ptr()
     d.nbatch = g
     if g > 1:
         d.bs_x, d.bs_w, d.bs_bias, d.bs_y, d.bs_r = c1 // g, (pc.cout // g) * pc.w.shape[1], pc.cout // g, pc.cout_out // g, pc.cout_out // g
```

Result: no change. 30.34 images/s (median of 6 runs) (+0.7%).
